# milos-agathon/vulkan-forge

Measured on AMD Instinct MI355X. Metric: Mpix/s terrain shade (grid=4096, 4096x4096), higher is better.
Workload: dtype f32

## Files before the change

include/vf_hip.h:

```cpp
#ifndef VF_HIP_H
#define VF_HIP_H

#include <stddef.h>
#include <stdint.h>

#ifdef __cplusplus
extern "C" {
#endif

#define VF_OK 0
#define VF_ERR_NO_DEVICE (-1)
#define VF_ERR_HIP (-2)
#define VF_ERR_INVALID (-3)
#define VF_ERR_NOMEM (-4)

typedef struct vf_ctx vf_ctx;
typedef struct vf_terrain vf_terrain;

typedef struct vf_device_info {
    char name[256];
    char arch[64];
    int32_t device_ordinal;
    int32_t compute_units;
    int32_t wavefront_size;
// ... 25 lines not shown
int vf_ctx_stream(const vf_ctx *ctx, void **stream);

int vf_terrain_create(vf_ctx *ctx, uint32_t width, uint32_t height, uint32_t grid,
                      const uint8_t lut_rgba8[1024], int lut_is_srgb, vf_terrain **out);
void vf_terrain_destroy(vf_terrain *t);

int vf_terrain_set_uniforms(vf_terrain *t, const float uniforms[44]);

int vf_terrain_set_height(vf_terrain *t, const float *host_height, uint32_t tw, uint32_t th);
int vf_terrain_set_height_device(vf_terrain *t, const float *dev_height, uint32_t tw, uint32_t th);

#define VF_SHADE_REFERENCE 0
#define VF_SHADE_SPEC_T32 1
int vf_terrain_set_shade_mode(vf_terrain *t, int mode);
#define VF_PRECISION_EXACT 0
#define VF_PRECISION_FAST 1
int vf_terrain_set_shade_precision(vf_terrain *t, int precision);
int vf_terrain_set_raster_groups(vf_terrain *t, int mode);
int vf_terrain_raster_groups(const vf_terrain *t, int *in_use, float ms[2]);

int vf_terrain_set_shard(vf_terrain *t, uint32_t rank, uint32_t nranks, uint32_t band_h);
int vf_terrain_local_rows(const vf_terrain *t, uint32_t *rows);

#define VF_TILE_LAYOUT(skew, stripe_log2) ((uint32_t)(skew) | ((uint32_t)(stripe_log2) << 16))
int vf_terrain_set_tile_shard(vf_terrain *t, uint32_t rank, uint32_t nranks, uint32_t layout);
int vf_terrain_tile_times(vf_terrain *t, float *ms, uint32_t capacity, uint32_t *count);
int vf_balance_stripes(const float *stripe_ms, uint32_t nstripes, uint32_t nranks, uint8_t *stripe_owner);
int vf_tile_layout_register_map(const uint8_t *stripe_owner, uint32_t nstripes, uint32_t stripe_log2, uint32_t nranks, uint32_t *layout);
int vf_terrain_local_tiles(const vf_terrain *t, uint32_t *tiles);
int vf_terrain_read_tiles(vf_terrain *t, uint8_t *dst, uint32_t first, uint32_t count);
int vf_tile_layout(uint32_t width, uint32_t height, uint32_t rank, uint32_t nranks, uint32_t layout, uint32_t *tiles,
                   uint32_t capacity, uint32_t *count);

int vf_terrain_set_output_device(vf_terrain *t, void *dev_rgba);
int vf_terrain_rgba_device(const vf_terrain *t, void **dev_rgba);

int vf_terrain_render(vf_terrain *t, void *stream);
int vf_terrain_render_batch(vf_terrain *t, const float *uniforms, uint32_t n, void *const *dev_rgba, void *stream);
int vf_terrain_render_batch_host(vf_terrain *t, const float *uniforms, uint32_t n, uint8_t *const *host_rgba);
int vf_terrain_sync(vf_terrain *t);

#define VF_SHAPE_CIRCLE 0
#define VF_SHAPE_SQUARE 1
#define VF_CAP_BUTT 0
#define VF_CAP_SQUARE 1
#define VF_CAP_ROUND 2
int vf_terrain_add_points(vf_terrain *t, const float *xyz, uint32_t n, const float *size_px, const uint8_t *rgba, float default_size,
                          const uint8_t default_rgba[4], int shape, int drape, uint32_t *layer_id);
int vf_terrain_add_lines(vf_terrain *t, const float *xyz, const uint32_t *path_offsets, uint32_t npaths, float width_px,
                         const uint8_t rgba[4], int cap, int drape, uint32_t *layer_id);
int vf_terrain_clear_overlays(vf_terrain *t);
int vf_terrain_add_polygons(vf_terrain *t, const float *xyz, const uint32_t *ring_offsets, uint32_t nrings, const uint32_t *feature_offsets,
                            uint32_t nfeatures, const uint8_t *fill_rgba, const uint8_t default_fill[4], const uint8_t line_rgba[4],
                            float line_width_px, int drape, uint32_t *layer_id);
#define VF_OCCLUSION_DEPTH_BIAS 1e-2f
int vf_terrain_set_layer_occlusion(vf_terrain *t, uint32_t layer_id, int occlude, float depth_bias);
#define VF_JOIN_ROUND 0
#define VF_JOIN_NONE 1
int vf_terrain_add_contours(vf_terrain *t, const float *levels, uint32_t nlevels, float width_px, const uint8_t rgba[4], float lift, int join,
                            int occlude, float depth_bias, uint32_t *layer_id, uint32_t *nsegments);
int vf_terrain_height_bounds(vf_terrain *t, float *lo, float *hi);
int vf_terrain_layer_primitive_count(vf_terrain *t, uint32_t layer_id, uint32_t *count);

int vf_terrain_read_rgba(vf_terrain *t, uint8_t *dst, uint32_t y0, uint32_t rows);
int vf_host_alloc(size_t bytes, void **host);
void vf_host_free(void *host);
int vf_terrain_read_png_scanlines(vf_terrain *t, const uint8_t **host_scanlines, size_t *nbytes);
int vf_terrain_read_visibility(vf_terrain *t, uint32_t *dst);

int vf_terrain_enable_timing(vf_terrain *t, int enable);
int vf_terrain_timings(vf_terrain *t, vf_timings *out);
int vf_terrain_frame_times(vf_terrain *t, float *tile_ms, float *period_ms, uint32_t max_frames, uint32_t *count);
int vf_terrain_debug_item_stats(vf_terrain *t, uint32_t *dst, uint32_t max_items, uint32_t *count);
#define VF_BAND_SLOTS 8u
int vf_terrain_debug_band_masks(vf_terrain *t, uint32_t *recs, uint64_t *masks, int32_t *xy, uint32_t max_blocks, uint32_t *count);
int vf_terrain_debug_set_plan_feedback(vf_terrain *t, const uint32_t *tile_ticks, const uint8_t *strips_log2, const uint32_t *piece_ticks,
                                       uint32_t ntiles);
#define VF_PLAN_FIRST        1u
#define VF_PLAN_FRESH        2u
#define VF_PLAN_MOTION_MAP   4u
#define VF_PLAN_DILATE       8u
#define VF_PLAN_QUEUED_AHEAD 16u
#define VF_PLAN_GEOMETRY_REUSED 32u
int vf_terrain_debug_plan_mode(const vf_terrain *t, uint32_t *mode);
int vf_terrain_debug_phase_cycles(vf_terrain *t, uint64_t *dst, uint32_t n);

int vf_grid_generate(vf_ctx *ctx, uint32_t nx, uint32_t nz, float dx, float dy,
                     float *xy, float *uv, uint32_t *idx);
int vf_grid_generate_device(vf_ctx *ctx, uint32_t nx, uint32_t nz, float dx, float dy,
                            float *dev_xy, float *dev_uv, uint32_t *dev_idx, void *stream);

int vf_triangle_render(vf_ctx *ctx, uint32_t width, uint32_t height, uint8_t *rgba_host);

typedef struct vf_dem vf_dem;
int vf_dem_create(vf_ctx *ctx, vf_dem **out);
void vf_dem_destroy(vf_dem *d);
int vf_dem_set_heights_f32(vf_dem *d, const float *host, uint32_t w, uint32_t h, float exaggeration);
int vf_dem_set_heights_f64(vf_dem *d, const double *host, uint32_t w, uint32_t h, float exaggeration);
int vf_dem_stats(vf_dem *d, float out[4]);
int vf_dem_percentile_range(vf_dem *d, float *p1, float *p99);
int vf_dem_normalize(vf_dem *d, int mode, float lo, float hi, float eps);
int vf_dem_upload_height(vf_dem *d);
int vf_dem_texture_size(const vf_dem *d, uint32_t *w, uint32_t *h);
int vf_dem_read_patch(vf_dem *d, uint32_t x, uint32_t y, uint32_t w, uint32_t h, float *dst);

int vf_stitch_bands_device(vf_ctx *ctx, const void *dev_gathered, void *dev_image, uint32_t width,
                           uint32_t height, uint32_t nranks, uint32_t band_h, void *stream);
int vf_stitch_tiles_device(vf_ctx *ctx, const void *dev_gathered, void *dev_image, uint32_t width, uint32_t height,
                           uint32_t nranks, uint32_t layout, uint32_t stride_tiles, void *stream);

#define VF_DIST_UNIQUE_ID_BYTES 128
int vf_dist_available(void);
int vf_dist_version(int *version);
int vf_dist_unique_id(uint8_t id[VF_DIST_UNIQUE_ID_BYTES]);
int vf_dist_comm_init(vf_ctx *ctx, const uint8_t id[VF_DIST_UNIQUE_ID_BYTES], int rank, int nranks, void **comm);
void vf_dist_comm_destroy(void *comm);
int vf_dist_gather_tiles(vf_terrain *t, void *rccl_comm, int root, void *dev_gathered, uint32_t stride_tiles, void *stream);
int vf_dist_gather_bands(vf_terrain *t, void *rccl_comm, int root, void *dev_image, void *stream);
int vf_dist_exchange_bands(vf_terrain *t, void *rccl_comm, int root, void *dev_image, void *stream);

typedef struct vf_fragment_timing {
    float resolve_ms;
    uint32_t covered_pixels;
    uint32_t repeats;
    uint32_t equal_to_frame;
} vf_fragment_timing;
int vf_terrain_debug_fragment_stage(vf_terrain *t, uint32_t repeats, vf_fragment_timing *out);

int vf_terrain_gbuffer_device(vf_terrain *t, float *dev_depth, float *dev_position, float *dev_normal, uint32_t *dev_primitive, void *stream);
int vf_terrain_read_gbuffer(vf_terrain *t, float *depth, float *position, float *normal, uint32_t *primitive);
int vf_terrain_pick(vf_terrain *t, const int32_t *pixels_xy, uint32_t n, float *out8);
#define VF_GBUFFER_DEPTH 1u
#define VF_GBUFFER_POSITION 2u
#define VF_GBUFFER_NORMAL 4u
#define VF_GBUFFER_PRIMITIVE 8u
int vf_terrain_debug_gbuffer_stage(vf_terrain *t, uint32_t planes, uint32_t repeats, float *ms);

#define VF_SHADOW_STRENGTH 0.7f
#define VF_SHADOW_SOFTNESS 0.02f
#define VF_SHADOW_BIAS 0.002f
int vf_terrain_set_shadows(vf_terrain *t, int enable, float strength, float softness, float bias);
int vf_terrain_read_shadow_field(vf_terrain *t, float *lit);
int vf_terrain_shadow_field_device(vf_terrain *t, float *dev_lit, void *stream);
int vf_terrain_debug_shadow_stage(vf_terrain *t, uint32_t repeats, float ms[2]);
int vf_terrain_debug_shadow_scans(vf_terrain *t, uint32_t *count);

#define VF_AMBIENT_STRENGTH 0.6f
#define VF_AMBIENT_REACH 64.0f
#define VF_AMBIENT_DIRECTIONS 16
#define VF_AMBIENT_REACH_MAX 1024
#define VF_AMBIENT_DIRECTIONS_MAX 64
int vf_terrain_set_ambient(vf_terrain *t, int enable, float strength, float reach, uint32_t ndirs, const float *dirs_xz);
int vf_terrain_read_sky_view_field(vf_terrain *t, float *sky);
int vf_terrain_sky_view_field_device(vf_terrain *t, float *dev_sky, void *stream);
int vf_terrain_debug_ambient_stage(vf_terrain *t, uint32_t repeats, float ms[2]);
int vf_terrain_debug_ambient_scans(vf_terrain *t, uint32_t *count);

#define VF_DRAPE_SIZE_MAX 16384
#define VF_DRAPE_NEAREST 0
#define VF_DRAPE_LINEAR 1
int vf_terrain_set_drape(vf_terrain *t, const uint8_t *rgba, uint32_t iw, uint32_t ih, uint32_t channels ,
                         const float extent[4], float opacity, int filter);
int vf_terrain_set_drape_device(vf_terrain *t, const void *dev_rgba , uint32_t iw, uint32_t ih,
                                const float extent[4], float opacity, int filter, void *stream);
int vf_terrain_clear_drape(vf_terrain *t);
int vf_terrain_drape_info(const vf_terrain *t, uint32_t *iw, uint32_t *ih, float extent[4], float *opacity, int *filter);
int vf_terrain_debug_drape_stage(vf_terrain *t, uint32_t repeats, float *ms);
// ... 56 lines not shown
```

vulkan_forge_amd/cabi.py:

```python
from __future__ import annotations

import ctypes as C
import os

import numpy as np

_HERE = os.path.dirname(os.path.abspath(__file__))
DEFAULT_LIB = os.environ.get("VF_HIP_LIB") or os.path.join(_HERE, "libvf_hip.so")

VF_OK, VF_ERR_NO_DEVICE, VF_ERR_HIP, VF_ERR_INVALID, VF_ERR_NOMEM = 0, -1, -2, -3, -4
VF_DRAPE_SIZE_MAX, VF_DRAPE_NEAREST, VF_DRAPE_LINEAR = 16384, 0, 1
VF_DRAPE_MIP_BIAS_MAX, VF_DRAPE_MIP_LEVELS_MAX = 16.0, 15
VF_PLAN_FIRST, VF_PLAN_FRESH, VF_PLAN_MOTION_MAP, VF_PLAN_DILATE, VF_PLAN_QUEUED_AHEAD = 1, 2, 4, 8, 16
VF_PLAN_GEOMETRY_REUSED = 32

SYMBOLS = [
    "vf_last_error", "vf_device_count", "vf_device_query", "vf_ctx_create", "vf_ctx_destroy", "vf_ctx_device_info", "vf_ctx_stream",
    "vf_terrain_create", "vf_terrain_destroy", "vf_terrain_set_uniforms", "vf_terrain_set_height",
    "vf_terrain_set_height_device", "vf_terrain_set_shade_mode", "vf_terrain_set_shade_precision", "vf_terrain_set_raster_groups", "vf_terrain_raster_groups", "vf_terrain_set_shard", "vf_terrain_local_rows", "vf_terrain_set_tile_shard",
    "vf_terrain_local_tiles", "vf_terrain_read_tiles", "vf_tile_layout", "vf_terrain_tile_times", "vf_balance_stripes", "vf_tile_layout_register_map", "vf_terrain_set_output_device",
    "vf_terrain_rgba_device", "vf_terrain_render", "vf_terrain_render_batch", "vf_terrain_render_batch_host", "vf_terrain_sync",
    "vf_terrain_add_points", "vf_terrain_add_lines", "vf_terrain_add_polygons", "vf_terrain_set_layer_occlusion", "vf_terrain_add_contours", "vf_terrain_height_bounds", "vf_terrain_layer_primitive_count", "vf_terrain_clear_overlays", "vf_terrain_read_rgba", "vf_terrain_read_png_scanlines", "vf_terrain_read_visibility",
    "vf_terrain_enable_timing", "vf_terrain_timings", "vf_terrain_frame_times", "vf_terrain_debug_item_stats", "vf_terrain_debug_band_masks", "vf_terrain_debug_set_plan_feedback", "vf_terrain_debug_plan_mode", "vf_terrain_debug_phase_cycles", "vf_grid_generate", "vf_grid_generate_device", "vf_triangle_render",
    "vf_stitch_bands_device", "vf_stitch_tiles_device",
    "vf_dist_available", "vf_dist_version", "vf_dist_unique_id", "vf_dist_comm_init", "vf_dist_comm_destroy", "vf_dist_gather_tiles", "vf_dist_gather_bands", "vf_dist_exchange_bands",
    "vf_terrain_debug_fragment_stage", "vf_host_alloc", "vf_host_free",
    "vf_terrain_gbuffer_device", "vf_terrain_read_gbuffer", "vf_terrain_pick", "vf_terrain_debug_gbuffer_stage",
    "vf_terrain_set_shadows", "vf_terrain_read_shadow_field", "vf_terrain_shadow_field_device", "vf_terrain_debug_shadow_stage",
    "vf_terrain_debug_shadow_scans",
    "vf_terrain_set_ambient", "vf_terrain_read_sky_view_field", "vf_terrain_sky_view_field_device", "vf_terrain_debug_ambient_stage",
    "vf_terrain_debug_ambient_scans",
    "vf_terrain_set_drape", "vf_terrain_set_drape_device", "vf_terrain_clear_drape", "vf_terrain_drape_info", "vf_terrain_debug_drape_stage",
    "vf_terrain_set_drape_mips", "vf_terrain_drape_mip_info", "vf_terrain_read_drape_level", "vf_terrain_debug_drape_mip_build",
    "vf_terrain_set_viewshed", "vf_terrain_read_viewshed_field", "vf_terrain_viewshed_field_device", "vf_terrain_viewshed_info",
    "vf_terrain_debug_viewshed_stage", "vf_terrain_debug_viewshed_scans",
    "vf_terrain_set_cumulative_viewshed", "vf_terrain_read_cumulative_viewshed_field", "vf_terrain_cumulative_viewshed_field_device",
    "vf_terrain_cumulative_viewshed_info", "vf_terrain_read_cumulative_viewshed_vertices", "vf_terrain_debug_cumulative_viewshed_batch",
    "vf_terrain_debug_cumulative_viewshed_scans", "vf_terrain_debug_cumulative_viewshed_stage",
    "vf_dem_create", "vf_dem_destroy", "vf_dem_set_heights_f32", "vf_dem_set_heights_f64", "vf_dem_stats",
    "vf_dem_percentile_range", "vf_dem_normalize", "vf_dem_upload_height", "vf_dem_texture_size", "vf_dem_read_patch",
]


class DeviceInfo(C.Structure):
    _fields_ = [("name", C.c_char * 256), ("arch", C.c_char * 64), ("device_ordinal", C.c_int32), ("compute_units", C.c_int32),
                ("wavefront_size", C.c_int32), ("clock_khz", C.c_int32), ("total_mem_bytes", C.c_uint64),
                ("lds_bytes_per_cu", C.c_uint64), ("pci_bus_id", C.c_int32), ("pci_device_id", C.c_int32)]


class Timings(C.Structure):
    _fields_ = [("ranges_ms", C.c_float), ("plan_ms", C.c_float), ("tile_ms", C.c_float), ("total_ms", C.c_float),
                ("blocks_rasterised", C.c_uint32), ("tiles", C.c_uint32), ("frames", C.c_uint32), ("blocks_distinct", C.c_uint32)]


class FragmentTiming(C.Structure):
    _fields_ = [("resolve_ms", C.c_float), ("covered_pixels", C.c_uint32), ("repeats", C.c_uint32), ("equal_to_frame", C.c_uint32)]


class ViewshedInfo(C.Structure):
    _fields_ = [("enabled", C.c_int32), ("has_observer", C.c_int32), ("vertex", C.c_uint32 * 2), ("observer_xyz", C.c_float * 3), ("eye_y", C.c_float),
                ("eye_height", C.c_float), ("target_height", C.c_float), ("radius", C.c_float), ("softness", C.c_float), ("bias", C.c_float),
                ("visible_rgba", C.c_uint8 * 4), ("hidden_rgba", C.c_uint8 * 4)]


class CumulativeViewshedInfo(C.Structure):
    _fields_ = [("enabled", C.c_int32), ("count", C.c_uint32), ("batch", C.c_uint32), ("eye_height", C.c_float), ("target_height", C.c_float),
                ("radius", C.c_float), ("softness", C.c_float), ("bias", C.c_float), ("high_rgba", C.c_uint8 * 4), ("low_rgba", C.c_uint8 * 4)]


DIST_UNIQUE_ID_BYTES = 128
_vp, _u32, _f, _i = C.c_void_p, C.c_uint32, C.c_float, C.c_int
_PROTOS = {
    "vf_last_error": (C.c_char_p, []),
    "vf_device_count": (_i, [C.POINTER(_i)]),
    "vf_device_query": (_i, [_i, C.POINTER(DeviceInfo)]),
    "vf_ctx_create": (_i, [_i, C.POINTER(_vp)]),
    "vf_ctx_destroy": (None, [_vp]),
    "vf_ctx_device_info": (_i, [_vp, C.POINTER(DeviceInfo)]),
    "vf_ctx_stream": (_i, [_vp, C.POINTER(_vp)]),
    "vf_terrain_create": (_i, [_vp, _u32, _u32, _u32, _vp, _i, C.POINTER(_vp)]),
    "vf_terrain_destroy": (None, [_vp]),
    "vf_terrain_set_uniforms": (_i, [_vp, _vp]),
    "vf_terrain_set_height": (_i, [_vp, _vp, _u32, _u32]),
    "vf_terrain_set_height_device": (_i, [_vp, _vp, _u32, _u32]),
    "vf_terrain_set_shade_mode": (_i, [_vp, _i]),
    "vf_terrain_set_shade_precision": (_i, [_vp, _i]),
    "vf_terrain_set_raster_groups": (_i, [_vp, _i]),
    "vf_terrain_raster_groups": (_i, [_vp, C.POINTER(_i), _vp]),
    "vf_terrain_set_shard": (_i, [_vp, _u32, _u32, _u32]),
    "vf_terrain_local_rows": (_i, [_vp, C.POINTER(_u32)]),
    "vf_terrain_set_tile_shard": (_i, [_vp, _u32, _u32, _u32]),
    "vf_terrain_add_points": (_i, [_vp, _vp, _u32, _vp, _vp, _f, _vp, _i, _i, C.POINTER(_u32)]),
    "vf_terrain_add_lines": (_i, [_vp, _vp, _vp, _u32, _f, _vp, _i, _i, C.POINTER(_u32)]),
    "vf_terrain_add_polygons": (_i, [_vp, _vp, _vp, _u32, _vp, _u32, _vp, _vp, _vp, _f, _i, C.POINTER(_u32)]),
    "vf_terrain_set_layer_occlusion": (_i, [_vp, _u32, _i, _f]),
    "vf_terrain_add_contours": (_i, [_vp, _vp, _u32, _f, _vp, _f, _i, _i, _f, C.POINTER(_u32), C.POINTER(_u32)]),
    "vf_terrain_height_bounds": (_i, [_vp, C.POINTER(_f), C.POINTER(_f)]),
    "vf_terrain_layer_primitive_count": (_i, [_vp, _u32, C.POINTER(_u32)]),
    "vf_terrain_clear_overlays": (_i, [_vp]),
    "vf_terrain_local_tiles": (_i, [_vp, C.POINTER(_u32)]),
    "vf_terrain_read_tiles": (_i, [_vp, _vp, _u32, _u32]),
    "vf_tile_layout": (_i, [_u32, _u32, _u32, _u32, _u32, _vp, _u32, C.POINTER(_u32)]),
    "vf_terrain_set_output_device": (_i, [_vp, _vp]),
    "vf_terrain_rgba_device": (_i, [_vp, C.POINTER(_vp)]),
    "vf_terrain_render": (_i, [_vp, _vp]),
    "vf_terrain_render_batch": (_i, [_vp, _vp, _u32, _vp, _vp]),
    "vf_terrain_render_batch_host": (_i, [_vp, _vp, _u32, _vp]),
    "vf_terrain_sync": (_i, [_vp]),
    "vf_terrain_read_rgba": (_i, [_vp, _vp, _u32, _u32]),
    "vf_terrain_read_png_scanlines": (_i, [_vp, C.POINTER(_vp), C.POINTER(C.c_size_t)]),
    "vf_terrain_read_visibility": (_i, [_vp, _vp]),
    "vf_terrain_enable_timing": (_i, [_vp, _i]),
    "vf_terrain_timings": (_i, [_vp, C.POINTER(Timings)]),
    "vf_terrain_frame_times": (_i, [_vp, _vp, _vp, _u32, C.POINTER(_u32)]),
    "vf_terrain_debug_item_stats": (_i, [_vp, _vp, _u32, C.POINTER(_u32)]),
    "vf_terrain_debug_band_masks": (_i, [_vp, _vp, _vp, _vp, _u32, C.POINTER(_u32)]),
    "vf_terrain_debug_set_plan_feedback": (_i, [_vp, _vp, _vp, _vp, _u32]),
    "vf_terrain_debug_plan_mode": (_i, [_vp, C.POINTER(_u32)]),
    "vf_terrain_debug_phase_cycles": (_i, [_vp, _vp, _u32]),
    "vf_terrain_tile_times": (_i, [_vp, _vp, _u32, C.POINTER(_u32)]),
    "vf_balance_stripes": (_i, [_vp, _u32, _u32, _vp]),
    "vf_tile_layout_register_map": (_i, [_vp, _u32, _u32, _u32, C.POINTER(_u32)]),
    "vf_host_alloc": (_i, [C.c_size_t, C.POINTER(_vp)]),
    "vf_host_free": (None, [_vp]),
    "vf_grid_generate": (_i, [_vp, _u32, _u32, _f, _f, _vp, _vp, _vp]),
    "vf_grid_generate_device": (_i, [_vp, _u32, _u32, _f, _f, _vp, _vp, _vp, _vp]),
    "vf_triangle_render": (_i, [_vp, _u32, _u32, _vp]),
    "vf_stitch_bands_device": (_i, [_vp, _vp, _vp, _u32, _u32, _u32, _u32, _vp]),
    "vf_stitch_tiles_device": (_i, [_vp, _vp, _vp, _u32, _u32, _u32, _u32, _u32, _vp]),
    "vf_dist_available": (_i, []),
    "vf_dist_version": (_i, [C.POINTER(_i)]),
    "vf_dist_unique_id": (_i, [_vp]),
    "vf_dist_comm_init": (_i, [_vp, _vp, _i, _i, C.POINTER(_vp)]),
    "vf_dist_comm_destroy": (None, [_vp]),
    "vf_dist_gather_tiles": (_i, [_vp, _vp, _i, _vp, _u32, _vp]),
    "vf_dist_gather_bands": (_i, [_vp, _vp, _i, _vp, _vp]),
    "vf_dist_exchange_bands": (_i, [_vp, _vp, _i, _vp, _vp]),
    "vf_terrain_debug_fragment_stage": (_i, [_vp, _u32, C.POINTER(FragmentTiming)]),
    "vf_terrain_gbuffer_device": (_i, [_vp, _vp, _vp, _vp, _vp, _vp]),
    "vf_terrain_read_gbuffer": (_i, [_vp, _vp, _vp, _vp, _vp]),
    "vf_terrain_pick": (_i, [_vp, _vp, _u32, _vp]),
    "vf_terrain_debug_gbuffer_stage": (_i, [_vp, _u32, _u32, C.POINTER(_f)]),
    "vf_terrain_set_shadows": (_i, [_vp, _i, _f, _f, _f]),
    "vf_terrain_read_shadow_field": (_i, [_vp, _vp]),
    "vf_terrain_shadow_field_device": (_i, [_vp, _vp, _vp]),
    "vf_terrain_debug_shadow_stage": (_i, [_vp, _u32, C.POINTER(_f)]),
    "vf_terrain_debug_shadow_scans": (_i, [_vp, C.POINTER(_u32)]),
    "vf_terrain_set_ambient": (_i, [_vp, _i, _f, _f, _u32, _vp]),
    "vf_terrain_read_sky_view_field": (_i, [_vp, _vp]),
    "vf_terrain_sky_view_field_device": (_i, [_vp, _vp, _vp]),
    "vf_terrain_debug_ambient_stage": (_i, [_vp, _u32, C.POINTER(_f)]),
    "vf_terrain_debug_ambient_scans": (_i, [_vp, C.POINTER(_u32)]),
    "vf_terrain_set_drape": (_i, [_vp, _vp, _u32, _u32, _u32, C.POINTER(_f), _f, _i]),
    "vf_terrain_set_drape_device": (_i, [_vp, _vp, _u32, _u32, C.POINTER(_f), _f, _i, _vp]),
    "vf_terrain_clear_drape": (_i, [_vp]),
    "vf_terrain_drape_info": (_i, [_vp, C.POINTER(_u32), C.POINTER(_u32), C.POINTER(_f), C.POINTER(_f), C.POINTER(_i)]),
    "vf_terrain_debug_drape_stage": (_i, [_vp, _u32, C.POINTER(_f)]),
    "vf_terrain_set_drape_mips": (_i, [_vp, _i, _f]),
    "vf_terrain_drape_mip_info": (_i, [_vp, C.POINTER(_i), C.POINTER(_u32), C.POINTER(_f), C.POINTER(C.c_uint64), C.POINTER(_u32)]),
    "vf_terrain_read_drape_level": (_i, [_vp, _u32, _vp, C.POINTER(_u32), C.POINTER(_u32)]),
    "vf_terrain_debug_drape_mip_build": (_i, [_vp, _u32, C.POINTER(_f)]),
    "vf_terrain_set_viewshed": (_i, [_vp, _i, C.POINTER(_f), _f, _f, _f, C.POINTER(C.c_uint8), C.POINTER(C.c_uint8), _f, _f]),
    "vf_terrain_read_viewshed_field": (_i, [_vp, _vp]),
    "vf_terrain_viewshed_field_device": (_i, [_vp, _vp, _vp]),
    "vf_terrain_viewshed_info": (_i, [_vp, C.POINTER(ViewshedInfo)]),
    "vf_terrain_debug_viewshed_stage": (_i, [_vp, _u32, C.POINTER(_f)]),
    "vf_terrain_debug_viewshed_scans": (_i, [_vp, C.POINTER(_u32)]),
    "vf_terrain_set_cumulative_viewshed": (_i, [_vp, _i, _vp, _u32, _f, _f, _f, C.POINTER(C.c_uint8), C.POINTER(C.c_uint8), _f, _f]),
    "vf_terrain_read_cumulative_viewshed_field": (_i, [_vp, _vp]),
    "vf_terrain_cumulative_viewshed_field_device": (_i, [_vp, _vp, _vp]),
    "vf_terrain_cumulative_viewshed_info": (_i, [_vp, C.POINTER(CumulativeViewshedInfo)]),
    "vf_terrain_read_cumulative_viewshed_vertices": (_i, [_vp, _vp]),
    "vf_terrain_debug_cumulative_viewshed_batch": (_i, [_vp, _u32]),
    "vf_terrain_debug_cumulative_viewshed_scans": (_i, [_vp, C.POINTER(_u32)]),
    "vf_terrain_debug_cumulative_viewshed_stage": (_i, [_vp, _u32, C.POINTER(_f)]),
    "vf_dem_create": (_i, [_vp, C.POINTER(_vp)]),
    "vf_dem_destroy": (None, [_vp]),
    "vf_dem_set_heights_f32": (_i, [_vp, _vp, _u32, _u32, _f]),
    "vf_dem_set_heights_f64": (_i, [_vp, _vp, _u32, _u32, _f]),
    "vf_dem_stats": (_i, [_vp, _vp]),
    "vf_dem_percentile_range": (_i, [_vp, C.POINTER(_f), C.POINTER(_f)]),
    "vf_dem_normalize": (_i, [_vp, _i, _f, _f, _f]),
    "vf_dem_upload_height": (_i, [_vp]),
    "vf_dem_texture_size": (_i, [_vp, C.POINTER(_u32), C.POINTER(_u32)]),
    "vf_dem_read_patch": (_i, [_vp, _u32, _u32, _u32, _u32, _vp]),
}


def load(path: str = DEFAULT_LIB) -> C.CDLL:
    lib = C.CDLL(path)
    for name, (res, args) in _PROTOS.items():
        fn = getattr(lib, name)
        fn.restype, fn.argtypes = res, args
    return lib


class VfError(RuntimeError):
    pass


def tile_layout(width, height, rank, nranks, skew=3, lib=None):
# ... 422 lines not shown
        from ._drape import drape_args
        img, iw, ih, ch, ext, opacity, code = drape_args(image, extent, opacity, filter)
        self._check(self.lib.vf_terrain_set_drape(self.t, img.ctypes.data, iw, ih, ch, ext.ctypes.data_as(C.POINTER(_f)), opacity, code))

    def set_drape_device(self, dev_rgba, width, height, *, extent=None, opacity=1.0, filter="linear", stream=None):
        from ._drape import drape_params, drape_size
        iw, ih = drape_size(width, height)
        ext, opacity, code = drape_params(extent, opacity, filter)
        self._check(self.lib.vf_terrain_set_drape_device(self.t, dev_rgba, iw, ih, ext.ctypes.data_as(C.POINTER(_f)), opacity, code, stream))

    def clear_drape(self):
        self._check(self.lib.vf_terrain_clear_drape(self.t))

    def drape_info(self):
        from ._drape import drape_info
        iw, ih, op, code, ext = _u32(), _u32(), _f(), _i(), (_f * 4)()
        self._check(self.lib.vf_terrain_drape_info(self.t, C.byref(iw), C.byref(ih), ext, C.byref(op), C.byref(code)))
        return drape_info(iw.value, ih.value, tuple(ext), op.value, code.value)

    def drape_stage(self, repeats=20):
        ms = _f()
        self._check(self.lib.vf_terrain_debug_drape_stage(self.t, int(repeats), C.byref(ms)))
        return ms.value

    def set_drape_mipmaps(self, enabled=True, *, bias=0.0):
        from ._drape import mip_params
        on, bias = mip_params(enabled, bias)
        self._check(self.lib.vf_terrain_set_drape_mips(self.t, on, bias))

    def drape_mip_info(self):
        from ._drape import mip_info
        on, levels, bias, nbytes, builds, iw, ih = _i(), _u32(), _f(), C.c_uint64(), _u32(), _u32(), _u32()
        self._check(self.lib.vf_terrain_drape_mip_info(self.t, C.byref(on), C.byref(levels), C.byref(bias), C.byref(nbytes), C.byref(builds)))
        self._check(self.lib.vf_terrain_drape_info(self.t, C.byref(iw), C.byref(ih), None, None, None))
        return mip_info(on.value != 0, levels.value, bias.value, nbytes.value, builds.value, iw.value, ih.value)

    def read_drape_level(self, level):
        from ._drape import mip_level
        levels, w, h = _u32(), _u32(), _u32()
        self._check(self.lib.vf_terrain_drape_mip_info(self.t, None, C.byref(levels), None, None, None))
        k = mip_level(level, levels.value)
        self._check(self.lib.vf_terrain_read_drape_level(self.t, k, None, C.byref(w), C.byref(h)))
        out = np.empty((h.value, w.value, 4), np.float16)
        self._check(self.lib.vf_terrain_read_drape_level(self.t, k, out.ctypes.data, None, None))
        return out

    def drape_mip_build_stage(self, repeats=20):
        ms = _f()
        self._check(self.lib.vf_terrain_debug_drape_mip_build(self.t, int(repeats), C.byref(ms)))
        return ms.value

    def enable_timing(self, on=True, stats=True, sampled=False):
        self._check(self.lib.vf_terrain_enable_timing(self.t, (1 if stats else (3 if sampled else 2)) if on else 0))

    def item_stats(self):
        cap = self.timings()["tiles"] + 2048
        out = np.zeros((cap, 4), np.uint32)
        n = _u32()
        self._check(self.lib.vf_terrain_debug_item_stats(self.t, out.ctypes.data, cap, C.byref(n)))
        return out[:n.value]

    def band_masks(self):
        nb = (self.grid - 1 + 7) // 8
        n = nb * nb
        recs, masks, xy = np.zeros((n, 8), np.uint32), np.zeros((n, 8, 2), np.uint64), np.zeros((n, 81, 2), np.int32)
        got = _u32()
        self._check(self.lib.vf_terrain_debug_band_masks(self.t, recs.ctypes.data, masks.ctypes.data, xy.ctypes.data, n, C.byref(got)))
        assert got.value == n
        wide = recs[:, 4:8].copy().view(np.uint64)
        return dict(box=recs[:, 0:2].copy().view(np.int16), flags=recs[:, 2].copy(), count=recs[:, 3].copy(),
                    alive_even=wide[:, 0].copy(), alive_odd=wide[:, 1].copy(), masks=masks, xy=xy)

    def set_plan_feedback(self, tile_ticks, strips_log2=None, piece_ticks=None):
        ticks = np.ascontiguousarray(tile_ticks, dtype=np.uint32).reshape(-1)
        n = len(ticks)
        lg = np.zeros(n, np.uint8) if strips_log2 is None else np.ascontiguousarray(strips_log2, dtype=np.uint8).reshape(n)
        pieces = None if piece_ticks is None else np.ascontiguousarray(piece_ticks, dtype=np.uint32).reshape(n, 64)
        self._check(self.lib.vf_terrain_debug_set_plan_feedback(self.t, ticks.ctypes.data, lg.ctypes.data,
                                                                None if pieces is None else pieces.ctypes.data, n))

    def plan_mode(self, geometry=False):
        m = _u32()
        self._check(self.lib.vf_terrain_debug_plan_mode(self.t, C.byref(m)))
        return m.value if geometry else m.value & ~VF_PLAN_GEOMETRY_REUSED

    def geometry_reused(self):
        return bool(self.plan_mode(geometry=True) & VF_PLAN_GEOMETRY_REUSED)

    def tile_stats(self):
        it = self.item_stats()
        out = np.zeros((self.timings()["tiles"], 3), np.uint32)
        tile = it[:, 0] & 0xFFFFF
        np.add.at(out[:, 0], tile, it[:, 1])
        np.maximum.at(out[:, 1], tile, it[:, 2])
        np.maximum.at(out[:, 2], tile, it[:, 3])
        return out

    def phase_cycles(self):
        out = np.zeros(40, np.uint64)
        self._check(self.lib.vf_terrain_debug_phase_cycles(self.t, out.ctypes.data, 40))
        return out

    def frame_times(self):
        tile, period, n = np.zeros(64, np.float32), np.zeros(64, np.float32), _u32(0)
        self._check(self.lib.vf_terrain_frame_times(self.t, tile.ctypes.data, period.ctypes.data, 64, C.byref(n)))
        return tile[:n.value].copy(), period[:n.value].copy()

    def timings(self):
        tm = Timings()
        self._check(self.lib.vf_terrain_timings(self.t, C.byref(tm)))
        return {k: getattr(tm, k) for k, _ in Timings._fields_}


class Dem:

    def __init__(self, device=0, lib=None):
        self.lib = lib or load()
        self.ctx, self.d = _vp(), _vp()
        self._check(self.lib.vf_ctx_create(int(device), C.byref(self.ctx)))
        self._check(self.lib.vf_dem_create(self.ctx, C.byref(self.d)))

    def _check(self, rc):
        if rc != VF_OK:
            msg = self.lib.vf_last_error().decode()
            raise VfError("No suitable GPU adapter" if rc == VF_ERR_NO_DEVICE else msg)

    def close(self):
        if self.d:
            self.lib.vf_dem_destroy(self.d)
            self.d = _vp()
        if self.ctx:
            self.lib.vf_ctx_destroy(self.ctx)
            self.ctx = _vp()

    def __del__(self):
        try:
            self.close()
        except Exception:
            pass

    def set_heights(self, heights, exaggeration=1.0):
        a = np.asarray(heights)
        if a.ndim != 2 or a.dtype not in (np.float32, np.float64) or not a.flags.c_contiguous:
            raise TypeError("heights must be a C-contiguous 2-D array of float32 or float64")
        fn = self.lib.vf_dem_set_heights_f32 if a.dtype == np.float32 else self.lib.vf_dem_set_heights_f64
        self._check(fn(self.d, a.ctypes.data, a.shape[1], a.shape[0], float(exaggeration)))

    def stats(self):
        out = np.zeros(4, np.float32)
        self._check(self.lib.vf_dem_stats(self.d, out.ctypes.data))
        return tuple(out)

    def percentile_range(self):
        p1, p99 = _f(), _f()
        self._check(self.lib.vf_dem_percentile_range(self.d, C.byref(p1), C.byref(p99)))
        return np.float32(p1.value), np.float32(p99.value)

    def normalize(self, mode, lo=0.0, hi=1.0, eps=1e-8):
        self._check(self.lib.vf_dem_normalize(self.d, {"minmax": 0, "zscore": 1}[mode], float(lo), float(hi), float(eps)))

    def upload(self):
        self._check(self.lib.vf_dem_upload_height(self.d))

    def texture_size(self):
        w, h = _u32(), _u32()
        self._check(self.lib.vf_dem_texture_size(self.d, C.byref(w), C.byref(h)))
        return w.value, h.value
# ... 11 lines not shown
```

vulkan_forge_amd/csrc/vf_hip.hip:

```cpp
#include "../../include/vf_hip.h"
#include "vf_kernels.h"
#include "vf_overlay.h"
#include "vf_gbuffer.h"
#include "vf_shadow.h"
#include "vf_ambient.h"
#include "vf_drape.h"
#include "vf_relight.h"
#include "vf_viewshed.h"
#include "vf_cumulative_viewshed.h"
#include "vf_line_loop.h"

#include <algorithm>
#include <cmath>
#include <vector>
#include <cstddef>
#include <cstdio>
#include <cstring>
#include <cstdlib>
#include <functional>
#include <new>
#include <string>
#include <atomic>
#include <memory>
#include <mutex>
// ... 79 lines not shown
    while ((1u << s) < v) ++s;
    return s;
}

}

struct PinnedRegistry {
    std::mutex mu;
    std::vector<void *> registered;
    static PinnedRegistry &get() { static PinnedRegistry *r = new PinnedRegistry; return *r; }
};
static hipError_t pinned_alloc(void **out, size_t n)
{
    constexpr size_t kHuge = (size_t)2 << 20;
    *out = nullptr;
    if (n >= 2 * kHuge) {
        void *p = nullptr;
        const size_t r = (n + kHuge - 1) & ~(kHuge - 1);
        if (posix_memalign(&p, kHuge, r) == 0) {
            (void)madvise(p, r, MADV_HUGEPAGE);
            if (hipHostRegister(p, r, hipHostRegisterDefault) == hipSuccess) {
                std::lock_guard<std::mutex> lk(PinnedRegistry::get().mu);
                PinnedRegistry::get().registered.push_back(p);
                *out = p;
                return hipSuccess;
            }
            (void)hipGetLastError();
            std::free(p);
        }
    }
    return hipHostMalloc(out, n, hipHostMallocDefault);
}
static void pinned_free(void *p)
{
    if (!p) return;
    bool ours = false;
    {
        PinnedRegistry &R = PinnedRegistry::get();
        std::lock_guard<std::mutex> lk(R.mu);
        auto it = std::find(R.registered.begin(), R.registered.end(), p);
        if (it != R.registered.end()) { R.registered.erase(it); ours = true; }
    }
    if (ours) { (void)hipHostUnregister(p); std::free(p); }
    else (void)hipHostFree(p);
}

struct vf_ctx {
    int device = 0;
    hipStream_t stream = nullptr;
    hipDeviceProp_t prop;
    float *d_decode = nullptr;
    float *d_thresh = nullptr;
    hipStream_t side = nullptr, side2 = nullptr, copy = nullptr;
    uint8_t *d_maps = nullptr;
    uint64_t maps_uploaded = 0;
    std::mutex lazy_mu;
};

static hipError_t ctx_side_streams(vf_ctx *c, hipStream_t *side, hipStream_t *side2)
{
    std::lock_guard<std::mutex> lk(c->lazy_mu);
    hipError_t e = hipSuccess;
    if (!c->side) e = hipStreamCreateWithFlags(&c->side, hipStreamNonBlocking);
    if (e == hipSuccess && !c->side2) e = hipStreamCreateWithFlags(&c->side2, hipStreamNonBlocking);
    *side = c->side; *side2 = c->side2;
    return e;
}
static hipError_t ctx_copy_stream(vf_ctx *c, hipStream_t *copy)
{
    std::lock_guard<std::mutex> lk(c->lazy_mu);
    hipError_t e = hipSuccess;
    if (!c->copy) e = hipStreamCreateWithFlags(&c->copy, hipStreamNonBlocking);
    *copy = c->copy;
    return e;
}

struct FramePlan {
    FrameParams P;
    uint32_t set = 0, ntiles = 0;
    uint32_t mode = 0;
    bool motion_starts = false;
    bool sampled = true;
    uint32_t *rc_lo = nullptr, *rc_hi = nullptr, *seg_count = nullptr;
};

template <typename T> struct DevBuf {
    T *p = nullptr;
    size_t cap = 0;
    hipError_t reserve(size_t need, size_t new_cap, size_t keep = 0, bool zero = false)
    {
        if (need <= cap) return hipSuccess;
        T *q = nullptr;
        hipError_t e = hipMalloc(&q, new_cap * sizeof(T));
        if (e == hipSuccess && zero) e = hipMemset(q, 0, new_cap * sizeof(T));
        if (e == hipSuccess && keep) e = hipMemcpy(q, p, keep * sizeof(T), hipMemcpyDeviceToDevice);
        if (e != hipSuccess) {
            if (q) (void)hipFree(q);
            return e;
        }
        release();
        p = q; cap = new_cap;
        return hipSuccess;
    }
    void release()
    {
        if (p) (void)hipFree(p);
        p = nullptr; cap = 0;
    }
};

struct VertexField {
    DevBuf<float> d;
    bool valid = false;
    uint64_t height_gen = 0;
    std::vector<uint32_t> key;
    uint32_t scans = 0;
    int prepare(const vf_terrain *t, const std::vector<uint32_t> &k, bool force, const char *nomem, bool *current);
    void computed(const vf_terrain *t, std::vector<uint32_t> &k);
    void release() { d.release(); valid = false; }
};
static uint32_t key_bits(float f) { uint32_t w; std::memcpy(&w, &f, sizeof w); return w; }
static std::vector<uint32_t> key_of(std::initializer_list<float> fs)
{
    std::vector<uint32_t> k;
    for (float f : fs) k.push_back(key_bits(f));
    return k;
}

template <typename F> static hipError_t time_launches(hipStream_t s, uint32_t repeats, float &ms, F &&launch)
{
    hipEvent_t e0 = nullptr, e1 = nullptr;
    hipError_t err = hipEventCreate(&e0);
    if (err == hipSuccess) err = hipEventCreate(&e1);
    if (err == hipSuccess) err = launch(true);
    if (err == hipSuccess) err = hipEventRecord(e0, s);
    for (uint32_t k = 0; k < repeats && err == hipSuccess; ++k) err = launch(false);
    if (err == hipSuccess) err = hipEventRecord(e1, s);
    if (err == hipSuccess) err = hipEventSynchronize(e1);
    float total = 0.0f;
    if (err == hipSuccess) err = hipEventElapsedTime(&total, e0, e1);
    if (e0) (void)hipEventDestroy(e0);
    if (e1) (void)hipEventDestroy(e1);
    ms = total / (float)repeats;
    return err;
}

struct PlanCursor {
    uint32_t cur_set = 0;
    uint32_t frame_no = 0;
    uint32_t frames_since_reset = 0;
    bool have_drawn = false, camera_moving = false, was_moving = false;
    float u_drawn[32] = {};
};

struct FrameInputs {
    float u[44] = {};
    uint32_t shade_mode = 0;
    uint32_t precision = VF_PRECISION_FAST;
};

struct LineLoop {
    int mode = -1;
    struct Probe { hipEvent_t a = nullptr, b = nullptr; int variant = 0; uint32_t epoch = 0; bool pending = false; } probes[16];
    uint32_t head = 0, epoch_id = 0;
    float ms[2] = { 0.0f, 0.0f };
    uint32_t n[2] = { 0u, 0u };
// ... 86 lines not shown
        DevBuf<float> d_cmax;
    } sh;
    struct Ambient {
        bool enabled = false;
        float strength = VF_AMBIENT_STRENGTH, reach = VF_AMBIENT_REACH;
        uint32_t ndirs = VF_AMBIENT_DIRECTIONS;
        bool default_dirs = true;
        std::vector<float> dirs;
        VertexField sky;
    } am;
    struct Drape {
        uint32_t iw = 0, ih = 0;
        float extent[4] = { -1.5f, -1.5f, 1.5f, 1.5f }, opacity = 1.0f;
        int filter = VF_DRAPE_LINEAR;
        DevBuf<uint32_t> d_img;
        hipEvent_t copied = nullptr;
    } dr;
    struct DrapeMipState {
        bool enabled = false;
        float bias = 0.0f;
        DevBuf<uint2> d_pyr;
        bool stale = true;
        uint32_t builds = 0;
    } dm;
    struct Viewshed {
        bool enabled = false, have_observer = false;
        float ox = 0.0f, oz = 0.0f;
        float eye_height = VF_VIEWSHED_EYE_HEIGHT, target_height = VF_VIEWSHED_TARGET_HEIGHT, radius = 0.0f;
        float softness = VF_VIEWSHED_SOFTNESS, bias = VF_VIEWSHED_BIAS;
        uint32_t visible_rgba = VF_VIEWSHED_VISIBLE_RGBA, hidden_rgba = VF_VIEWSHED_HIDDEN_RGBA;
        bool tinted = false;
        VertexField seen;
        DevBuf<float> d_cmax;
    } vs;
    struct CumulativeViewshed {
        bool enabled = false;
        std::vector<float> xz;
        float eye_height = VF_VIEWSHED_EYE_HEIGHT, target_height = VF_VIEWSHED_TARGET_HEIGHT, radius = 0.0f;
        float softness = VF_VIEWSHED_SOFTNESS, bias = VF_VIEWSHED_BIAS;
        uint32_t high_rgba = VF_CUMULATIVE_VIEWSHED_HIGH_RGBA, low_rgba = VF_CUMULATIVE_VIEWSHED_LOW_RGBA;
        uint32_t forced_batch = 0;
        DevBuf<uint32_t> d_sum;
        VertexField count;
        DevBuf<float> d_frac;
        DevBuf<float> d_cmax;
        DevBuf<ViewshedPlan> d_plans;
        std::vector<ViewshedPlan> plans;
        uint32_t batch = 0;
    } cv;
    uint64_t height_gen = 1;
    static constexpr uint32_t kBatchRing = 3;
    uint32_t *d_batch[kBatchRing] = { nullptr, nullptr, nullptr };
    hipEvent_t batch_drawn[kBatchRing] = { nullptr, nullptr, nullptr }, batch_copied[kBatchRing] = { nullptr, nullptr, nullptr };
    hipStream_t copy_stream = nullptr;
    uint8_t *d_png = nullptr, *h_png = nullptr;
    uint8_t *h_stage = nullptr;
    hipEvent_t stage_ev[4] = { nullptr, nullptr, nullptr, nullptr };
    static constexpr uint32_t kPlanStates = 2;
    struct PlanState {
        PixelBox *ranges = nullptr;
        VertexRec *vtx = nullptr;
        BlockRec *recs = nullptr;
        ulonglong2 *gen = nullptr;
        ulonglong2 *band = nullptr;
        uint32_t *seg_list = nullptr;
        PixelBox *row_ranges = nullptr;
        float4 *cap_seg = nullptr;
        float *cap_rad = nullptr;
        uint32_t *rc = nullptr;
        uint2 *work = nullptr;
        uint2 *work_sorted = nullptr;
        uint32_t *work_count = nullptr;
        uint32_t *redo = nullptr;
        uint32_t *background = nullptr;
        uint32_t *flags_new = nullptr;
        uint32_t *feedback = nullptr;
        hipEvent_t planned = nullptr, drawn = nullptr, boxed = nullptr, set_up = nullptr;
        hipEvent_t pev[3] = { nullptr, nullptr, nullptr };
        bool pev_valid = false;
        uint8_t *slab = nullptr;
        float u_used[32] = {};
        bool have_u_used = false;
        uint64_t geom_stamp = 0, height_stamp = 0;
    } ps[kPlanStates];
    PlanCursor cursor;
    uint32_t last_set = 0;
    uint32_t last_plan_mode = 0;
    hipStream_t side = nullptr;
    hipStream_t side2 = nullptr;
    hipEvent_t entry = nullptr;
    hipEvent_t cached = nullptr;
    hipStream_t cached_on = nullptr;
    hipStream_t last_stream = nullptr;
    bool rendered = false;
    uint64_t inputs_gen = 1;
    uint64_t geom_gen = 1;
    struct PrePlan {
        bool valid = false;
        FramePlan K;
        uint64_t gen = 0, geom = 0;
        PlanCursor before;
    } pre;
    uint64_t last_drawn_geom = 0;
    bool replan_fresh = false;
    bool preplan_pending = false;
    uint32_t tight_calls = 0;
    bool want_plan_streams = false;
    hipEvent_t copied = nullptr;
    static constexpr int kTimingRing = 64;
    bool timing = false;
    bool stats_on = false;
    uint32_t timing_every = 1;
    struct FrameEvents { hipEvent_t begin = nullptr, end = nullptr; } ev[kTimingRing];
    uint32_t timed_frames = 0;
    LineLoop loop;
    uint8_t *d_xrecv = nullptr, *d_xband = nullptr;
    size_t xrecv_bytes = 0, xband_bytes = 0;
    struct Overlays {
        uint32_t nprims = 0, features = 0;
        DevBuf<OvIn> in;
        DevBuf<OvPrim> prim;
        DevBuf<uint2> box;
        uint32_t *d_cnt = nullptr;
        uint32_t *d_start = nullptr;
        DevBuf<uint32_t> list;
        uint32_t *h_total = nullptr;
        hipEvent_t counted = nullptr;
        uint32_t nfill = 0;
        uint32_t pg_lo = 0, pg_hi = 0;
        DevBuf<uint32_t> pg_hdr;
        DevBuf<uint4> pg_fbox;
        DevBuf<uint4> pg_fbin;
        DevBuf<unsigned long long> pg_total;
        DevBuf<uint32_t> mask;
        struct Layer { uint32_t lo, hi; bool polygon, occlude; };
        std::vector<Layer> layer;
        uint32_t occluding = 0;
        DevBuf<float4> dep;
    } ov;
    struct Contours {
        DevBuf<float> levels;
        DevBuf<uint32_t> count;
        DevBuf<unsigned long long> total;
        DevBuf<float2> bounds;
    } ct;
};

struct StatsLayout { size_t phases, block_bits, words; };
static StatsLayout stats_layout(const vf_terrain *t)
{
    const size_t phases = 4 + 4 * ((size_t)t->ntx * t->nty + kSplitBudget), block_bits = phases + 2 * kPhaseSlots;
    return { phases, block_bits, block_bits + (t->nblocks + 31) / 32 };
}
static size_t feedback_words(const vf_terrain *t) { return (size_t)t->ntx * t->nty * 65 + 1; }
static uint32_t grid_segments(const vf_terrain *t) { return t->nb * ((t->nb + kSegBlocks - 1) / kSegBlocks); }
static float grid_step(const vf_terrain *t) { return (2.0f * 1.5f) / ((float)t->n - 1.0f); }
static float spacing_of(const float *u) { return std::fmax(u[36], 1e-8f); }

int VertexField::prepare(const vf_terrain *t, const std::vector<uint32_t> &k, bool force, const char *nomem, bool *current)
{
    if (!d.p) {
        const size_t nv = (size_t)t->n * t->n;
        if (d.reserve(nv, nv) != hipSuccess) { (void)hipGetLastError(); return fail(VF_ERR_NOMEM, nomem); }
        valid = false;
    }
    *current = !force && valid && height_gen == t->height_gen && key == k;
    if (!*current) valid = false;
// ... 112 lines not shown
}

static AxisTables axis(const vf_terrain *t)
{
    AxisTables A;
    A.xs = t->d_xs; A.sinx = t->d_sinx; A.cosz = t->d_cosz; A.txi = t->d_txi; A.tyj = t->d_tyj;
    return A;
}

namespace {
struct Carver {
    struct Item { void **p; size_t bytes; };
    std::vector<Item> zeroed, plain;
    void add(void **p, size_t bytes, bool zero = false) { (zero ? zeroed : plain).push_back({ p, (bytes + 255u) & ~(size_t)255u }); }
    hipError_t commit(uint8_t **base, hipStream_t s)
    {
        size_t zero_bytes = 0, total = 0;
        for (const Item &i : zeroed) zero_bytes += i.bytes;
        total = zero_bytes;
        for (const Item &i : plain) total += i.bytes;
        hipError_t e = hipMalloc((void **)base, total);
        if (e != hipSuccess) return e;
        size_t off = 0;
        for (const Item &i : zeroed) { *i.p = *base + off; off += i.bytes; }
        for (const Item &i : plain) { *i.p = *base + off; off += i.bytes; }
        return zero_bytes ? hipMemsetAsync(*base, 0, zero_bytes, s) : hipSuccess;
    }
};
}

static hipError_t sync_sides(const vf_terrain *t)
{
    hipError_t e = t->side ? hipStreamSynchronize(t->side) : hipSuccess;
    if (e == hipSuccess && t->side2) e = hipStreamSynchronize(t->side2);
    return e;
}

static hipError_t wait_frame(const vf_terrain *t)
{
    const hipError_t e = hipSetDevice(t->ctx->device);
    return e != hipSuccess ? e : hipStreamSynchronize(t->last_stream ? t->last_stream : t->ctx->stream);
}

static hipError_t drop_preplan(vf_terrain *t, hipStream_t next_plan_on = nullptr)
{
    t->preplan_pending = false;
    if (!t->pre.valid) return hipSuccess;
    const vf_terrain::PrePlan &R = t->pre;
    t->pre.valid = false;
    t->cursor = R.before;
    t->replan_fresh = true;
    hipStream_t on = t->side ? t->side : (next_plan_on ? next_plan_on : (t->last_stream ? t->last_stream : t->ctx->stream));
    hipError_t e = hipStreamWaitEvent(on, t->ps[R.K.set].set_up, 0);
    if (e == hipSuccess) e = hipStreamWaitEvent(on, t->ps[R.K.set].planned, 0);
    if (e == hipSuccess) e = hipMemsetAsync(R.K.seg_count, 0, sizeof(uint32_t), on);
    return e;
}

static hipError_t ensure_plan_state(vf_terrain *t, uint32_t k, hipStream_t zero_on)
{
    vf_terrain::PlanState &S = t->ps[k];
    if (S.slab) return hipSuccess;
    const size_t all_tiles = (size_t)t->ntx * t->nty;
    Carver C;
    C.add((void **)&S.seg_list, ((size_t)grid_segments(t) + 1) * sizeof(uint32_t), true);
    C.add((void **)&S.feedback, feedback_words(t) * sizeof(uint32_t), true);
    C.add((void **)&S.background, all_tiles * sizeof(uint32_t), true);
    C.add((void **)&S.ranges, t->nblocks * sizeof(PixelBox));
    C.add((void **)&S.vtx, (size_t)t->nblocks * kBlockStride * sizeof(VertexRec));
    C.add((void **)&S.recs, (size_t)t->nblocks * sizeof(BlockRec));
    C.add((void **)&S.band, (size_t)t->nblocks * kBandSlots * sizeof(ulonglong2));
    C.add((void **)&S.gen, (size_t)t->nblocks * sizeof(ulonglong2));
    C.add((void **)&S.row_ranges, t->nb * sizeof(PixelBox));
    C.add((void **)&S.cap_seg, t->nblocks * sizeof(float4));
    C.add((void **)&S.cap_rad, t->nblocks * sizeof(float));
    C.add((void **)&S.rc, 2 * (size_t)t->nb * t->ntx * sizeof(uint32_t));
    C.add((void **)&S.work, 2 * (all_tiles + kSplitBudget + 16) * sizeof(uint2));
    C.add((void **)&S.work_count, 4 * sizeof(uint32_t));
    C.add((void **)&S.redo, (all_tiles + kSplitBudget) * sizeof(uint32_t));
    C.add((void **)&S.flags_new, all_tiles * sizeof(uint32_t));
    hipError_t err = C.commit(&S.slab, zero_on);
    if (err != hipSuccess) { S.slab = nullptr; return err; }
    S.geom_stamp = S.height_stamp = 0;
    S.work_sorted = S.work + (all_tiles + kSplitBudget + 16);
    if (err == hipSuccess) err = hipEventCreateWithFlags(&S.planned, hipEventDisableTiming);
    if (err == hipSuccess) err = hipEventCreateWithFlags(&S.drawn, hipEventDisableTiming);
    if (err == hipSuccess) err = hipEventCreateWithFlags(&S.boxed, hipEventDisableTiming);
    if (err == hipSuccess) err = hipEventCreateWithFlags(&S.set_up, hipEventDisableTiming);
    return err;
}

static int refresh_tables(vf_terrain *t, hipStream_t s)
{
    hipLaunchKernelGGL(k_axis_tables, dim3((t->n + 255) / 256), dim3(256), 0, s, t->n, t->tw, t->th, t->d_xs, t->d_sinx,
                       t->d_cosz, t->d_txi, t->d_tyj);
    VF_HIP_TRY(hipGetLastError());
    t->bounds_dirty = true;
    return VF_OK;
}

static void ov_release(vf_terrain *t)
{
    vf_terrain::Overlays &O = t->ov;
    void *ptrs[] = { O.d_cnt, O.d_start };
    for (void *p : ptrs) if (p) (void)hipFree(p);
    O.in.release(); O.prim.release(); O.box.release(); O.list.release(); O.dep.release();
    O.pg_hdr.release(); O.pg_fbox.release(); O.pg_fbin.release(); O.pg_total.release(); O.mask.release();
    if (O.h_total) (void)hipHostFree(O.h_total);
    if (O.counted) (void)hipEventDestroy(O.counted);
    O = vf_terrain::Overlays();
    t->ct.levels.release(); t->ct.count.release(); t->ct.total.release(); t->ct.bounds.release();
}

static void drape_release(vf_terrain *t)
{
    vf_terrain::Drape &D = t->dr;
    D.d_img.release();
    if (D.copied) (void)hipEventDestroy(D.copied);
    D = vf_terrain::Drape();
    t->dm.d_pyr.release(); t->dm.stale = true;
}

static void shadow_release(vf_terrain *t) { t->sh.lit.release(); t->sh.d_cmax.release(); }
static void ambient_release(vf_terrain *t) { t->am.sky.release(); }

static void viewshed_release(vf_terrain *t)
{
    vf_terrain::Viewshed &H = t->vs;
    H.seen.release(); H.d_cmax.release();
    const uint32_t scans = H.seen.scans;
    H = vf_terrain::Viewshed();
    H.seen.scans = scans;
}

static void cumulative_release(vf_terrain *t)
{
    vf_terrain::CumulativeViewshed &H = t->cv;
    H.d_sum.release(); H.count.release(); H.d_frac.release(); H.d_cmax.release(); H.d_plans.release();
    const uint32_t scans = H.count.scans, forced = H.forced_batch;
    H = vf_terrain::CumulativeViewshed();
    H.count.scans = scans; H.forced_batch = forced;
}

int vf_terrain_create(vf_ctx *ctx, uint32_t width, uint32_t height, uint32_t grid, const uint8_t lut_rgba8[1024],
                      int lut_is_srgb, vf_terrain **out)
{
    if (!ctx || !out || !lut_rgba8) return fail(VF_ERR_INVALID, "NULL argument");
    *out = nullptr;
    if (width == 0 || height == 0 || width > 16384 || height > 16384) return fail(VF_ERR_INVALID, "width/height must be in 1..16384");
    uint32_t n = grid < 2 ? 2 : grid;
    if (n > 8192) return fail(VF_ERR_INVALID, "grid must be <= 8192");
    VF_HIP_TRY(hipSetDevice(ctx->device));
    vf_terrain *t = new (std::nothrow) vf_terrain;
    if (!t) return fail(VF_ERR_NOMEM, "out of host memory");
    t->ctx = ctx; t->W = width; t->H = height; t->n = n;
    t->nb = (n - 1 + kBlockCells - 1) / kBlockCells;
    t->nblocks = t->nb * t->nb;
    t->ntx = (width + kTileW - 1) / kTileW;
    t->nty = (height + kTileH - 1) / kTileH;
    t->local_rows = height;
    t->local_tiles = t->ntx * t->nty;

    float lut[kLutFloats];
    for (int i = 0; i <= 256; ++i) {
        const int k = i < 256 ? i : 255;
        for (int ch = 0; ch < 3; ++ch)
            lut[kLutStride * i + ch] = lut_is_srgb ? tables().decode[lut_rgba8[4 * k + ch]] : (float)lut_rgba8[4 * k + ch] / 255.0f;
        lut[kLutStride * i + 3] = 0.0f;
    }
    hipError_t err = hipSuccess;
    const size_t all_tiles = (size_t)t->ntx * t->nty;
    Carver C;
    C.add((void **)&t->d_height_dummy, sizeof(float), true);
    C.add((void **)&t->d_stats, stats_layout(t).words * sizeof(uint32_t), true);
    C.add((void **)&t->d_xs, n * sizeof(float));
    C.add((void **)&t->d_sinx, n * sizeof(float));
    C.add((void **)&t->d_cosz, n * sizeof(float));
    C.add((void **)&t->d_txi, n * sizeof(int32_t));
    C.add((void **)&t->d_tyj, n * sizeof(int32_t));
    C.add((void **)&t->d_bounds, t->nblocks * sizeof(float2));
    C.add((void **)&t->d_hblk, (size_t)t->nblocks * kBlockStride * sizeof(float));
    C.add((void **)&t->d_lut, sizeof lut);
    C.add((void **)&t->d_rgba_own, all_tiles * kTileW * kTileH * sizeof(uint32_t));
    C.add((void **)&t->d_tile_map, all_tiles * sizeof(uint32_t));
    C.add((void **)&t->d_stripe_owner, kMaxStripes);
    err = C.commit(&t->slab, ctx->stream);
    if (err == hipSuccess) err = hipMemcpyAsync(t->d_lut, lut, sizeof lut, hipMemcpyHostToDevice, ctx->stream);
    if (err == hipSuccess) err = hipEventCreateWithFlags(&t->entry, hipEventDisableTiming);
    if (err == hipSuccess) err = hipEventCreateWithFlags(&t->cached, hipEventDisableTiming);
    for (uint32_t k = 0; k < vf_terrain::kPlanStates && err == hipSuccess; ++k) err = ensure_plan_state(t, k, ctx->stream);
    if (err != hipSuccess) {
        std::string m = std::string("terrain allocation failed: ") + hipGetErrorString(err);
        vf_terrain_destroy(t);
        return fail(err == hipErrorOutOfMemory ? VF_ERR_NOMEM : VF_ERR_HIP, m);
    }
    t->d_rgba = t->d_rgba_own;
    t->d_height = t->d_height_dummy; t->tw = 1; t->th = 1;
    int rc = refresh_tables(t, ctx->stream);
    if (rc == VF_OK && hipStreamSynchronize(ctx->stream) != hipSuccess) rc = fail(VF_ERR_HIP, "table setup failed");
    if (rc != VF_OK) { std::string keep = g_err; vf_terrain_destroy(t); g_err = keep; return rc; }
    *out = t;
    return VF_OK;
}

void vf_terrain_destroy(vf_terrain *t)
{
    if (!t) return;
    (void)hipSetDevice(t->ctx->device);
    (void)hipDeviceSynchronize();
    void *ptrs[] = { t->slab, t->d_height_own, t->d_vis, t->d_rgba_scratch, t->d_diag, t->d_xrecv, t->d_xband, t->d_batch[0], t->d_batch[1], t->d_batch[2] };
    for (void *p : ptrs) if (p) (void)hipFree(p);
    t->d_gb.release(); t->d_pick.release();
    shadow_release(t); ambient_release(t); viewshed_release(t); cumulative_release(t);
    drape_release(t);
    for (auto &e : t->batch_drawn) if (e) (void)hipEventDestroy(e);
    for (auto &e : t->batch_copied) if (e) (void)hipEventDestroy(e);

    for (auto &S : t->ps) {
        if (S.slab) (void)hipFree(S.slab);
        if (S.planned) (void)hipEventDestroy(S.planned);
        if (S.drawn) (void)hipEventDestroy(S.drawn);
        if (S.boxed) (void)hipEventDestroy(S.boxed);
        if (S.set_up) (void)hipEventDestroy(S.set_up);
        for (auto &e : S.pev) if (e) (void)hipEventDestroy(e);
    }
    pinned_free(t->h_stage);
    for (auto &e : t->stage_ev) if (e) (void)hipEventDestroy(e);
    if (t->d_png) (void)hipFree(t->d_png);
    pinned_free(t->h_png);
    for (auto &f : t->ev) { if (f.begin) (void)hipEventDestroy(f.begin); if (f.end) (void)hipEventDestroy(f.end); }
    if (t->entry) (void)hipEventDestroy(t->entry);
    if (t->cached) (void)hipEventDestroy(t->cached);
    if (t->copied) (void)hipEventDestroy(t->copied);
    for (auto &g : t->loop.probes) { if (g.a) (void)hipEventDestroy(g.a); if (g.b) (void)hipEventDestroy(g.b); }
    ov_release(t);
    delete t;
}

static bool same_geometry(const float *a, const float *b)
{
    return std::memcmp(a, b, 32 * sizeof(float)) == 0 && std::memcmp(a + 36, b + 36, sizeof(float)) == 0 && std::memcmp(a + 38, b + 38, sizeof(float)) == 0;
}

static void take_uniforms(vf_terrain *t, const float *uniforms)
{
    if (!t->have_uniforms || std::memcmp(t->inputs.u, uniforms, sizeof t->inputs.u) != 0) t->inputs_gen++;
    if (!t->have_uniforms || !same_geometry(t->inputs.u, uniforms)) t->geom_gen++;
    std::memcpy(t->inputs.u, uniforms, sizeof t->inputs.u);
    t->have_uniforms = true;
}

int vf_terrain_set_uniforms(vf_terrain *t, const float uniforms[44])
{
    if (!t || !uniforms) return fail(VF_ERR_INVALID, "NULL argument");
    take_uniforms(t, uniforms);
    return VF_OK;
}

static int set_height_common(vf_terrain *t, uint32_t tw, uint32_t th)
{
    t->inputs_gen++;
    t->geom_gen++;
    t->height_gen++;
    VF_HIP_TRY(drop_preplan(t));
    t->loop.reset();
    bool resized = tw != t->tw || th != t->th;
    t->tw = tw; t->th = th;
    if (resized) return refresh_tables(t, t->ctx->stream);
    t->bounds_dirty = true;
    return VF_OK;
}

int vf_terrain_set_height(vf_terrain *t, const float *host_height, uint32_t tw, uint32_t th)
{
    if (!t || !host_height) return fail(VF_ERR_INVALID, "NULL argument");
    if (tw == 0 || th == 0 || tw > 32768 || th > 32768) return fail(VF_ERR_INVALID, "height texture size must be in 1..32768");
    VF_HIP_TRY(wait_frame(t));
    VF_HIP_TRY(sync_sides(t));
    size_t bytes = (size_t)tw * th * sizeof(float);
    if ((size_t)t->tw * t->th != (size_t)tw * th || t->d_height != t->d_height_own) {
        float *fresh = nullptr;
        hipError_t e = hipMalloc(&fresh, bytes);
        if (e != hipSuccess) return fail(e == hipErrorOutOfMemory ? VF_ERR_NOMEM : VF_ERR_HIP, std::string("height texture allocation failed: ") + hipGetErrorString(e));
        if (t->d_height_own) (void)hipFree(t->d_height_own);
        t->d_height_own = fresh;
    }
    t->d_height = t->d_height_own;
    VF_HIP_TRY(hipMemcpyAsync(t->d_height_own, host_height, bytes, hipMemcpyHostToDevice, t->ctx->stream));
    int rc = set_height_common(t, tw, th);
    if (rc == VF_OK) {
        hipLaunchKernelGGL(k_height_blocks, dim3(t->nblocks), dim3(64), 0, t->ctx->stream, t->n, t->nb, t->tw, axis(t), t->d_height, t->d_hblk, t->d_bounds);
        const hipError_t le = hipGetLastError();
        if (le != hipSuccess) rc = fail(VF_ERR_HIP, std::string("k_height_blocks: ") + hipGetErrorString(le));
        else t->bounds_dirty = false;
    }
    VF_HIP_TRY(hipStreamSynchronize(t->ctx->stream));
    return rc;
}

int vf_terrain_set_height_device(vf_terrain *t, const float *dev_height, uint32_t tw, uint32_t th)
{
    if (!t || !dev_height) return fail(VF_ERR_INVALID, "NULL argument");
    if (tw == 0 || th == 0 || tw > 32768 || th > 32768) return fail(VF_ERR_INVALID, "height texture size must be in 1..32768");
    VF_HIP_TRY(wait_frame(t));
    VF_HIP_TRY(sync_sides(t));
    t->d_height = dev_height;
    int rc = set_height_common(t, tw, th);
    if (rc != VF_OK) return rc;
    VF_HIP_TRY(hipStreamSynchronize(t->ctx->stream));
    return VF_OK;
}

int vf_terrain_set_shade_mode(vf_terrain *t, int mode)
{
    if (!t) return fail(VF_ERR_INVALID, "NULL argument");
    if (mode != VF_SHADE_REFERENCE && mode != VF_SHADE_SPEC_T32) return fail(VF_ERR_INVALID, "unknown shade mode");
    if (t->inputs.shade_mode != (uint32_t)mode) t->inputs_gen++;
    t->inputs.shade_mode = (uint32_t)mode;
    return VF_OK;
}

int vf_terrain_set_shade_precision(vf_terrain *t, int precision)
{
    if (!t) return fail(VF_ERR_INVALID, "NULL argument");
    if (precision != VF_PRECISION_EXACT && precision != VF_PRECISION_FAST) return fail(VF_ERR_INVALID, "unknown shade precision");
    if (t->inputs.precision != (uint32_t)precision) t->inputs_gen++;
    t->inputs.precision = (uint32_t)precision;
    return VF_OK;
}

int vf_terrain_set_raster_groups(vf_terrain *t, int mode)
{
    if (!t) return fail(VF_ERR_INVALID, "NULL argument");
    if (mode < -1 || mode > 1) return fail(VF_ERR_INVALID, "mode must be -1 (measure and choose), 0 or 1");
    t->loop.mode = mode;
    t->loop.reset();
    return VF_OK;
}

int vf_terrain_raster_groups(const vf_terrain *t, int *in_use, float ms[2])
{
    if (!t || !in_use) return fail(VF_ERR_INVALID, "NULL argument");
    *in_use = t->loop.now;
    if (ms) { ms[0] = t->loop.n[0] ? t->loop.ms[0] : 0.0f; ms[1] = t->loop.n[1] ? t->loop.ms[1] : 0.0f; }
    return VF_OK;
}

static int reset_layout_feedback(vf_terrain *t)
{
    t->rendered = false; t->have_frame = false;
    t->cursor.frames_since_reset = 0;
    VF_HIP_TRY(sync_sides(t));
    for (auto &S : t->ps) {
        if (!S.slab) continue;
        VF_HIP_TRY(hipMemset(S.feedback, 0, feedback_words(t) * sizeof(uint32_t)));
        VF_HIP_TRY(hipMemset(S.background, 0, (size_t)t->ntx * t->nty * sizeof(uint32_t)));
        S.have_u_used = false;
    }
    for (auto &S : t->ps) S.geom_stamp = S.height_stamp = 0;
    return VF_OK;
}

int vf_terrain_set_shard(vf_terrain *t, uint32_t rank, uint32_t nranks, uint32_t band_h)
{
    if (!t) return fail(VF_ERR_INVALID, "NULL argument");
    if (nranks == 0 || rank >= nranks) return fail(VF_ERR_INVALID, "rank must be < nranks");
    if (!is_pow2(band_h) || band_h < (uint32_t)kTileH) return fail(VF_ERR_INVALID, "band_h must be a power of two >= 64 (the tile height)");
    if (!t->ov.layer.empty()) return fail(VF_ERR_INVALID, "the handle has overlays: sharded compositing is not supported (vf_terrain_clear_overlays first)");
    if (t->sh.enabled && nranks != 1) return fail(VF_ERR_INVALID, "the handle has shadows enabled: shadows need a whole-frame handle");
    if (t->am.enabled && nranks != 1) return fail(VF_ERR_INVALID, "the handle has ambient occlusion enabled: it needs a whole-frame handle");
    if (t->dr.iw && nranks != 1) return fail(VF_ERR_INVALID, "the handle holds a draped image: it needs a whole-frame handle");
    if (t->vs.enabled && nranks != 1) return fail(VF_ERR_INVALID, "the handle has a viewshed enabled: it needs a whole-frame handle");
    if (t->cv.enabled && nranks != 1) return fail(VF_ERR_INVALID, "the handle has a cumulative viewshed enabled: it needs a whole-frame handle");
    VF_HIP_TRY(wait_frame(t));
    t->inputs_gen++;
    t->geom_gen++;
    VF_HIP_TRY(drop_preplan(t));
    t->rank = rank; t->nranks = nranks; t->band_h = band_h;
    t->shard_tiles = false; t->use_map = false;
    t->local_rows = compute_local_rows(t->H, rank, nranks, band_h);
    t->local_tiles = t->ntx * ((t->local_rows + kTileH - 1) / kTileH);
    return reset_layout_feedback(t);
}

int vf_tile_layout(uint32_t width, uint32_t height, uint32_t rank, uint32_t nranks, uint32_t skew, uint32_t *tiles, uint32_t capacity,
                   uint32_t *count)
{
    if (!count) return fail(VF_ERR_INVALID, "NULL argument");
    if (width == 0 || height == 0 || nranks == 0 || rank >= nranks) return fail(VF_ERR_INVALID, "empty frame or rank >= nranks");
    if (!layout_valid(skew)) return fail(VF_ERR_INVALID, "layout word is neither VF_TILE_LAYOUT(skew < 65536, stripe_log2 <= 15) nor a registered stripe map");
    const uint32_t ntx = (width + kTileW - 1) / kTileW, nty = (height + kTileH - 1) / kTileH;
    if (ntx > 0xFFFFu || nty > 0xFFFFu) return fail(VF_ERR_INVALID, "frame too large");
    const StripeMap *m = layout_map(skew);
    if (m && (m->nranks != nranks || ((ntx - 1u) >> m->shift) >= m->owner.size()))
        return fail(VF_ERR_INVALID, "the registered stripe map was made for another number of ranks or a narrower frame");
    uint32_t n = 0;
    for (uint32_t ty = 0; ty < nty; ++ty)
        for (uint32_t tx = 0; tx < ntx; ++tx)
            if (layout_owner(skew, m, tx, ty, nranks) == rank) {
                if (tiles && n < capacity) tiles[n] = tx | (ty << 16);
                ++n;
            }
    *count = n;
    return VF_OK;
}

int vf_tile_layout_register_map(const uint8_t *stripe_owner, uint32_t nstripes, uint32_t stripe_log2, uint32_t nranks, uint32_t *layout)
{
    if (!stripe_owner || !layout) return fail(VF_ERR_INVALID, "NULL argument");
    if (nstripes == 0 || nstripes > kMaxStripes || stripe_log2 > 15u || nranks == 0 || nranks > 255u) return fail(VF_ERR_INVALID, "1..256 stripes, stripe_log2 <= 15, 1..255 ranks");
    for (uint32_t k = 0; k < nstripes; ++k) if (stripe_owner[k] >= nranks) return fail(VF_ERR_INVALID, "a stripe's owner is not a rank");
    std::lock_guard<std::mutex> lk(g_maps_mu);
    g_maps.reserve(kMaxStripeMaps);
    for (uint32_t id = 0; id < g_maps.size(); ++id)
        if (g_maps[id].shift == stripe_log2 && g_maps[id].nranks == nranks && g_maps[id].owner.size() == nstripes &&
            std::memcmp(g_maps[id].owner.data(), stripe_owner, nstripes) == 0) { *layout = kLayoutMapBit | (id << 21) | (stripe_log2 << 16); return VF_OK; }
    if (g_maps.size() >= kMaxStripeMaps) return fail(VF_ERR_INVALID, "too many registered stripe maps (64 per process)");
    StripeMap m;
    m.owner.assign(stripe_owner, stripe_owner + nstripes); m.shift = stripe_log2; m.nranks = nranks;
    g_maps.push_back(std::move(m));
    *layout = kLayoutMapBit | ((uint32_t)(g_maps.size() - 1u) << 21) | (stripe_log2 << 16);
    return VF_OK;
}

int vf_balance_stripes(const float *stripe_ms, uint32_t nstripes, uint32_t nranks, uint8_t *stripe_owner)
{
    if (!stripe_ms || !stripe_owner) return fail(VF_ERR_INVALID, "NULL argument");
    if (nranks == 0 || nranks > 255u || nstripes == 0 || nstripes > kMaxStripes || nstripes % nranks) return fail(VF_ERR_INVALID, "the stripes must divide evenly among 1..255 ranks");
    std::vector<uint32_t> order(nstripes);
    for (uint32_t k = 0; k < nstripes; ++k) order[k] = k;
    auto cost = [&](uint32_t k) { const float v = stripe_ms[k]; return std::isfinite(v) && v > 0.0f ? (double)v : 0.0; };
    std::stable_sort(order.begin(), order.end(), [&](uint32_t a, uint32_t b) { return cost(a) > cost(b); });
    std::vector<double> load(nranks, 0.0);
    std::vector<uint32_t> have(nranks, 0u);
    std::vector<uint8_t> own(nstripes, 0);
    const uint32_t room = nstripes / nranks;
    for (uint32_t k : order) {
        uint32_t best = nranks;
        for (uint32_t r = 0; r < nranks; ++r)
            if (have[r] < room && (best == nranks || load[r] < load[best])) best = r;
        own[k] = (uint8_t)best; load[best] += cost(k); have[best]++;
    }
// ... 128 lines not shown
    P.hw = 0.5f * (float)t->W; P.hh = 0.5f * (float)t->H;
    P.step = grid_step(t);
    P.n = t->n; P.nm1 = t->n - 1; P.nb = t->nb;
    P.W = t->W; P.H = t->H; P.ntx = t->ntx; P.nty = t->nty; P.tw = t->tw; P.th = t->th;
    P.rank = t->rank; P.nranks = t->nranks; P.band_h = t->band_h; P.band_shift = ilog2(t->band_h);
    P.local_rows = t->local_rows;
    P.shard_tiles = t->shard_tiles ? 1u : 0u; P.tile_map = t->d_tile_map; P.skew = layout_skew(t->skew); P.stripe_shift = layout_shift(t->skew);
    P.stripe_owner = t->shard_tiles && t->use_map ? t->d_stripe_owner : nullptr;
    P.shade_mode = in.shade_mode; P.tex = t->d_height;
    P.inv2hr = 1.0f / (2.0f * P.h_range);
    {
        const uint32_t d = P.nm1;
        if (d <= 1u) { P.div_m = 0u; P.div_s = 0u; }
        else {
            const uint32_t L = ilog2(d);
            P.div_s = L - 1u;
            P.div_m = (uint32_t)((((uint64_t)1 << (31u + L)) + d - 1u) / d);
        }
    }
    const SrgbTables &T = tables();
    P.clear_rgba = T.encode(0.02f) | (T.encode(0.02f) << 8) | (T.encode(0.03f) << 16) | 0xFF000000u;
}

static float camera_shift_px(const vf_terrain *t, const float *a, const float *b)
{
    const float ext = 1.5f * spacing_of(t->inputs.u);
    float worst = 0.0f;
    for (int c = 0; c < 4; ++c) {
        const float p[4] = { (c & 1) ? ext : -ext, 0.0f, (c & 2) ? ext : -ext, 1.0f };
        float xy[2][2];
        for (int k = 0; k < 2; ++k) {
            const float *u = k ? b : a;
            float v[4], q[4];
            for (int r = 0; r < 4; ++r) v[r] = u[r] * p[0] + u[4 + r] * p[1] + u[8 + r] * p[2] + u[12 + r] * p[3];
            for (int r = 0; r < 4; ++r) q[r] = u[16 + r] * v[0] + u[20 + r] * v[1] + u[24 + r] * v[2] + u[28 + r] * v[3];
            if (!(q[3] > 1e-6f)) return 1e9f;
            xy[k][0] = q[0] / q[3] * 0.5f * (float)t->W; xy[k][1] = q[1] / q[3] * 0.5f * (float)t->H;
        }
        worst = std::fmax(worst, std::fmax(std::fabs(xy[0][0] - xy[1][0]), std::fabs(xy[0][1] - xy[1][1])));
    }
    return worst;
}
static bool motion_map(const vf_terrain *t, const float *then, const float *now, MotionMap &M)
{
    const double hw = 0.5 * t->W, hh = 0.5 * t->H;
    auto plane = [&](const float *u, double g[9]) {
        double vp[16];
        for (int c = 0; c < 4; ++c)
            for (int r = 0; r < 4; ++r) {
                double a = 0.0;
                for (int k = 0; k < 4; ++k) a += (double)u[16 + 4 * k + r] * (double)u[4 * c + k];
                vp[4 * c + r] = a;
            }
        const int cols[3] = { 0, 2, 3 };
        for (int j = 0; j < 3; ++j) {
            const double cx = vp[4 * cols[j] + 0], cy = vp[4 * cols[j] + 1], cw = vp[4 * cols[j] + 3];
            g[0 + j] = hw * cx + hw * cw; g[3 + j] = -hh * cy + hh * cw; g[6 + j] = cw;
        }
    };
    double a[9], b[9];
    plane(then, a); plane(now, b);
    const double det = b[0] * (b[4] * b[8] - b[5] * b[7]) - b[1] * (b[3] * b[8] - b[5] * b[6]) + b[2] * (b[3] * b[7] - b[4] * b[6]);
    double scale = 0.0;
    for (double v : b) scale = std::fmax(scale, std::fabs(v));
    if (!(std::fabs(det) > 1e-12 * scale * scale * scale)) return false;
    const double inv[9] = { (b[4] * b[8] - b[5] * b[7]) / det, (b[2] * b[7] - b[1] * b[8]) / det, (b[1] * b[5] - b[2] * b[4]) / det,
                            (b[5] * b[6] - b[3] * b[8]) / det, (b[0] * b[8] - b[2] * b[6]) / det, (b[2] * b[3] - b[0] * b[5]) / det,
                            (b[3] * b[7] - b[4] * b[6]) / det, (b[1] * b[6] - b[0] * b[7]) / det, (b[0] * b[4] - b[1] * b[3]) / det };
    double m[9], big = 0.0;
    for (int r = 0; r < 3; ++r)
        for (int c = 0; c < 3; ++c) { m[3 * r + c] = a[3 * r] * inv[c] + a[3 * r + 1] * inv[3 + c] + a[3 * r + 2] * inv[6 + c]; big = std::fmax(big, std::fabs(m[3 * r + c])); }
    if (!(big > 0.0) || !std::isfinite(big)) return false;
    for (int k = 0; k < 9; ++k) M.m[k] = (float)(m[k] / big);
    M.on = 1u;
    return true;
}
constexpr float kFreshFeedbackPx = 24.0f;

#ifndef VF_GROUPS_MAX_RANKS
#define VF_GROUPS_MAX_RANKS 8
#endif
static bool fast_shading(const FrameInputs &in) { return in.precision == VF_PRECISION_FAST && in.shade_mode == VF_SHADE_REFERENCE; }

static int plan_frame(vf_terrain *t, hipStream_t s, FramePlan &K, bool streaming = false)
{
    FrameParams &P = K.P;
    PlanCursor &C = t->cursor;
    const float *u = t->inputs.u;
    build_params(t, t->inputs, P);
    AxisTables A = axis(t);
    const uint32_t ntiles = t->local_tiles;
    const uint32_t set = C.cur_set;
    C.cur_set = (set + 1u) % vf_terrain::kPlanStates;
    C.frame_no++;
    if (!t->side && C.frame_no > 1u) {
        bool have = false;
        { std::lock_guard<std::mutex> lk(t->ctx->lazy_mu); have = t->ctx->side && t->ctx->side2; }
        if (have || streaming || t->want_plan_streams) VF_HIP_TRY(ctx_side_streams(t->ctx, &t->side, &t->side2));
    }
    const bool solo = !t->side;
    VF_HIP_TRY(ensure_plan_state(t, set, solo ? s : t->side));
    vf_terrain::PlanState &S = t->ps[set], &O = t->ps[t->last_set];
    float shift = 0.0f;
    if (C.have_drawn) {
        shift = camera_shift_px(t, C.u_drawn, u);
        if (shift > kFreshFeedbackPx) C.camera_moving = true;
        else if (shift < 0.5f * kFreshFeedbackPx) C.camera_moving = false;
    }
    const bool young = C.frames_since_reset >= 1 && C.frames_since_reset < vf_terrain::kPlanStates;
    MotionMap M;
    std::memset(&M, 0, sizeof M);
    if ((C.camera_moving || C.was_moving) && !young && C.frames_since_reset >= vf_terrain::kPlanStates && S.have_u_used && t->nranks == 1u && !t->shard_tiles &&
        camera_shift_px(t, S.u_used, u) < 0.4f * (float)std::max(t->W, t->H))
        (void)motion_map(t, S.u_used, u, M);
    const bool after_drop = t->replan_fresh && C.frames_since_reset >= vf_terrain::kPlanStates;
    t->replan_fresh = false;
    if (after_drop) M.on = 0u;
    const bool fresh = young || after_drop || ((C.camera_moving || C.was_moving) && !M.on);
    const bool first = C.frames_since_reset == 0;
    C.frames_since_reset++;
    const bool motion_starts = C.camera_moving && !C.was_moving;
    C.was_moving = C.camera_moving;
    const bool dilate = fresh || shift > 0.5f * kFreshFeedbackPx;
    std::memcpy(C.u_drawn, u, sizeof C.u_drawn);
    C.have_drawn = true;
    hipStream_t side = solo ? s : t->side, side2 = solo ? s : t->side2;
    K.sampled = t->timing_every <= 1u || C.frame_no % t->timing_every == 0u;
    const bool timed = t->timing && t->timing_every <= 1u && S.pev[0] != nullptr;
    hipEvent_t *ev = S.pev;
    S.pev_valid = timed;
    VF_HIP_TRY(hipStreamWaitEvent(side, S.drawn, 0));
    if (t->bounds_dirty) {
        VF_HIP_TRY(hipEventRecord(t->entry, s));
        VF_HIP_TRY(hipStreamWaitEvent(side, t->entry, 0));
        hipLaunchKernelGGL(k_height_blocks, dim3(t->nblocks), dim3(64), 0, side, t->n, t->nb, t->tw, A, t->d_height, t->d_hblk, t->d_bounds);
        VF_HIP_TRY(hipGetLastError());
        VF_HIP_TRY(hipEventRecord(t->cached, side));
        t->cached_on = side;
        t->bounds_dirty = false;
        for (auto &X : t->ps) X.geom_stamp = X.height_stamp = 0;
    }
    if (t->cached_on && t->cached_on != side) {
        VF_HIP_TRY(hipStreamWaitEvent(side, t->cached, 0));
        t->cached_on = side;
    }
    const bool reuse = S.geom_stamp != 0 && S.geom_stamp == t->geom_gen && S.height_stamp == t->height_gen;
    if (timed) VF_HIP_TRY(hipEventRecord(ev[0], side));
    const size_t rc_n = (size_t)t->nb * t->ntx;
    uint32_t *rc_lo = S.rc, *rc_hi = S.rc + rc_n;
    uint32_t *quantum = S.feedback + (size_t)t->ntx * t->nty;
    const uint32_t nsegs_all = grid_segments(t);
    uint32_t *seg_count = S.seg_list + nsegs_all;
    const uint32_t *const quantum_from = fresh || first ? (const uint32_t *)nullptr : S.feedback;
    if (reuse) {
        hipLaunchKernelGGL(k_plan_begin, dim3(1), dim3(512), 0, side, quantum_from, t->ntx * t->nty, quantum, S.work_count);
    } else {
        S.geom_stamp = S.height_stamp = 0;
        hipLaunchKernelGGL(k_block_boxes, dim3(t->nb + 1), dim3(t->nb > 256 ? 512 : 256), 0, side, P, t->d_bounds, S.ranges, S.row_ranges, S.cap_seg, S.cap_rad, rc_lo, rc_hi,
                           quantum_from, t->ntx * t->nty, quantum, S.work_count, S.recs, S.seg_list, seg_count);
        VF_HIP_TRY(hipEventRecord(S.boxed, side));
        VF_HIP_TRY(hipStreamWaitEvent(side2, S.boxed, 0));
        hipLaunchKernelGGL(k_block_setup, dim3(nsegs_all), dim3(kSetupThreads), 0, side2,
                           P, t->d_hblk, S.ranges, S.vtx, S.recs, S.gen, S.seg_list, seg_count, S.band);
        VF_HIP_TRY(hipEventRecord(S.set_up, side2));
        VF_HIP_TRY(hipGetLastError());
        S.geom_stamp = t->geom_gen; S.height_stamp = t->height_gen;
    }
    if (timed) VF_HIP_TRY(hipEventRecord(ev[1], side));
    if (ntiles) {
        if (fresh) {
            VF_HIP_TRY(hipStreamWaitEvent(side, O.drawn, 0));
            hipLaunchKernelGGL(k_quantum, dim3(1), dim3(512), 0, side, O.feedback, t->ntx * t->nty, quantum);
        } else if (first) {
            VF_HIP_TRY(hipStreamWaitEvent(side, S.set_up, 0));
            hipLaunchKernelGGL(k_plan_estimate, dim3(ntiles), dim3(256), 0, side, P, S.row_ranges, S.recs, S.cap_seg, S.cap_rad, rc_lo, rc_hi, S.feedback);
            hipLaunchKernelGGL(k_quantum, dim3(1), dim3(512), 0, side, S.feedback, t->ntx * t->nty, quantum);
        }
        const vf_terrain::PlanState &F = fresh ? O : S;
        hipLaunchKernelGGL(k_plan, dim3(ntiles), dim3(256), 0, side, P, S.row_ranges, S.flags_new, S.work, S.work_count,
                           F.feedback, quantum, S.work_count + 1, rc_lo, rc_hi, dilate ? 1u : 0u, F.background, M);
        hipLaunchKernelGGL(k_plan_sort, dim3(1), dim3(256), 0, side, S.work, S.work_sorted, S.work_count, S.feedback, t->ntx * t->nty,
                           S.flags_new, S.background, ntiles);
    }
    VF_HIP_TRY(hipGetLastError());
    if (timed) VF_HIP_TRY(hipEventRecord(ev[2], side));
    VF_HIP_TRY(hipEventRecord(S.planned, side));
    K.mode = (first ? VF_PLAN_FIRST : 0u) | (fresh ? VF_PLAN_FRESH : 0u) | (M.on ? VF_PLAN_MOTION_MAP : 0u) | (dilate ? VF_PLAN_DILATE : 0u) |
             (reuse ? VF_PLAN_GEOMETRY_REUSED : 0u);
    K.set = set; K.ntiles = ntiles; K.motion_starts = motion_starts; K.rc_lo = rc_lo; K.rc_hi = rc_hi; K.seg_count = seg_count;
    return VF_OK;
}

static int overlay_pass(vf_terrain *t, hipStream_t s, const FrameParams &P, const SetupView &V)
{
    vf_terrain::Overlays &O = t->ov;
    const uint32_t nbx = (t->W + kOvBin - 1u) / kOvBin, nby = (t->H + kOvBin - 1u) / kOvBin, nbins = nbx * nby;
    const dim3 per_prim((O.nprims + 255u) / 256u), threads(256);
    const bool occlude = O.occluding != 0u;
    hipLaunchKernelGGL(k_ov_setup, per_prim, threads, 0, s, P, axis(t), O.nprims, O.in.p, O.prim.p, O.box.p, O.d_cnt, nbx,
                       occlude ? O.dep.p : nullptr);
    const dim3 per_slot((O.pg_hi - O.pg_lo + 255u) / 256u);
    if (O.nfill) {
        hipLaunchKernelGGL(k_pg_setup, per_slot, threads, 0, s, P, axis(t), O.pg_lo, O.pg_hi, O.in.p, O.prim.p, O.box.p, O.d_cnt, nbx, O.pg_fbox.p);
        hipLaunchKernelGGL(k_pg_header, dim3((O.nfill + 255u) / 256u), threads, 0, s, P, O.nfill, O.pg_hdr.p, O.in.p, O.pg_fbox.p, O.pg_fbin.p,
                           O.prim.p, O.box.p, O.d_cnt, nbx, O.pg_total.p);
    }
    hipLaunchKernelGGL(k_ov_scan, dim3(1), dim3(1024), 0, s, nbins, O.d_cnt, O.d_start);
    VF_HIP_TRY(hipGetLastError());
    VF_HIP_TRY(hipMemcpyAsync(O.h_total, O.d_start + nbins, sizeof(uint32_t), hipMemcpyDeviceToHost, s));
    if (O.nfill) {
        VF_HIP_TRY(hipMemcpyAsync(O.h_total + 2, O.pg_total.p, sizeof(unsigned long long), hipMemcpyDeviceToHost, s));
        VF_HIP_TRY(hipMemsetAsync(O.pg_total.p, 0, sizeof(unsigned long long), s));
    }
    VF_HIP_TRY(hipEventRecord(O.counted, s));
    VF_HIP_TRY(hipEventSynchronize(O.counted));
    const uint32_t total = *O.h_total;
    unsigned long long words = 0;
    if (O.nfill) std::memcpy(&words, O.h_total + 2, sizeof words);
    if (total == 0u) return VF_OK;
    if (total == 0xFFFFFFFFu) return fail(VF_ERR_NOMEM, "overlays: more than 2^32 - 2 (primitive, screen bin) pairs in one frame");
    if (words > 0xFFFFFFFFull) return fail(VF_ERR_NOMEM, "overlays: polygon fills reach more than 2^32 - 1 (feature, screen bin) pairs in one frame");
    hipError_t e = O.mask.reserve(words, words + words / 2u + 4096u);
    if (e != hipSuccess) return fail(VF_ERR_NOMEM, std::string("polygon mask allocation failed: ") + hipGetErrorString(e));
    if (words) {
        VF_HIP_TRY(hipMemsetAsync(O.mask.p, 0, (size_t)words * sizeof(uint32_t), s));
        hipLaunchKernelGGL(k_pg_backdrop, per_slot, threads, 0, s, t->H, O.pg_lo, O.pg_hi, O.in.p, O.prim.p, O.pg_fbin.p, O.mask.p);
        hipLaunchKernelGGL(k_pg_prefix, dim3((O.nfill + 3u) / 4u), threads, 0, s, O.nfill, O.pg_fbin.p, O.mask.p);
    }
    e = O.list.reserve(total, (size_t)total + total / 2u + 4096u);
    if (e != hipSuccess) return fail(VF_ERR_NOMEM, std::string("overlay pair list allocation failed: ") + hipGetErrorString(e));
    hipLaunchKernelGGL(k_ov_scatter, per_prim, threads, 0, s, O.nprims, O.box.p, nbx, O.d_start, O.d_cnt, O.list.p);
    if (occlude)
        hipLaunchKernelGGL(k_ov_composite_occlude, dim3(nbins), threads, 0, s, t->W, t->H, nbx, O.prim.p, O.d_cnt, O.d_start, O.list.p, t->ctx->d_decode,
                           t->ctx->d_thresh, O.mask.p, t->d_rgba, P, V, t->d_vis, O.dep.p);
    else
        hipLaunchKernelGGL(k_ov_composite, dim3(nbins), threads, 0, s, t->W, t->H, nbx, O.prim.p, O.d_cnt, O.d_start, O.list.p, t->ctx->d_decode,
                           t->ctx->d_thresh, O.mask.p, t->d_rgba);
    VF_HIP_TRY(hipGetLastError());
    return VF_OK;
}

static int relight_pass(vf_terrain *t, hipStream_t s, const FrameParams &P, const SetupView &V, const uint32_t *redo, uint32_t *rgba, Relight pass,
                        bool shadows, bool ambient);

static int viewshed_pass(vf_terrain *t, hipStream_t s, const FrameParams &P, const SetupView &V, const uint32_t *redo, uint32_t *rgba);
static int cumulative_pass(vf_terrain *t, hipStream_t s, const FrameParams &P, const SetupView &V, const uint32_t *redo, uint32_t *rgba);

static int draw_frame(vf_terrain *t, hipStream_t s, const FramePlan &K, bool diag)
{
    const FrameParams &P = K.P;
    const bool shadows = t->sh.enabled && !diag;
    const bool ambient = t->am.enabled && !diag;
    const bool drape = t->dr.iw != 0u && !diag;
    const Relight drape_pass = t->dm.enabled ? kDrapeMip : kDrape;
    const bool viewshed = t->vs.enabled && !diag;
    const bool cumulative = t->cv.enabled && !diag;
    const bool write_vis = diag || (t->ov.occluding && t->ov.nprims) || shadows || ambient || drape || viewshed || cumulative;
    vf_terrain::PlanState &S = t->ps[K.set];
    const uint32_t ntiles = K.ntiles, set = K.set;
    uint32_t *const rc_lo = K.rc_lo, *const rc_hi = K.rc_hi, *const seg_count = K.seg_count;
    vf_terrain::FrameEvents &ev = t->ev[t->timed_frames % (uint32_t)vf_terrain::kTimingRing];
    const bool timing_now = t->timing && K.sampled;
    const SetupView V = { S.vtx, t->d_hblk, S.recs, S.gen };
    uint32_t *stats = t->timing && t->stats_on ? t->d_stats : nullptr;
    const uint32_t nstats = (uint32_t)stats_layout(t).words;
    VF_HIP_TRY(hipStreamWaitEvent(s, S.planned, 0));
    VF_HIP_TRY(hipStreamWaitEvent(s, S.set_up, 0));
    if (t->last_stream && t->last_stream != s && t->rendered)
        VF_HIP_TRY(hipStreamWaitEvent(s, t->ps[t->last_set].drawn, 0));
    if (timing_now) VF_HIP_TRY(hipEventRecord(ev.begin, s));
    const int guess = t->nranks < (uint32_t)VF_GROUPS_MAX_RANKS ? 1 : 0;
    const LoopPick pick = t->loop.choose(guess, t->cursor.frames_since_reset <= 1 || K.motion_starts, ntiles != 0u);
    const bool groups = pick.variant != 0;
    LineLoop::Probe *gp = pick.probe ? t->loop.arm(s) : nullptr;
    if (ntiles) {
        uint32_t *vis = write_vis ? t->d_vis : nullptr;
        hipLaunchKernelGGL(k_clear, dim3(ntiles), dim3(256), 0, s, P, S.background, t->d_rgba, vis, stats, nstats, seg_count);
        const dim3 per_cu(std::min<uint32_t>((uint32_t)std::max(1, t->ctx->prop.multiProcessorCount) * (1024u / (uint32_t)kTileThreads), ntiles + kSplitBudget)),
                   few(std::min<uint32_t>(64u, ntiles + kSplitBudget)), threads(kTileThreads);
#define VF_TILE_ARGS P, V, S.row_ranges, S.cap_seg, S.cap_rad, t->d_lut, t->ctx->d_thresh, S.work_sorted, S.work_count, \
                     rc_lo, rc_hi, t->d_rgba, vis, stats, S.feedback, S.redo, S.band
        const bool fast = fast_shading(t->inputs);
#define VF_TILE_LAUNCH(WV, FS)                                                                                         \
        do {                                                                                                           \
            if (groups) hipLaunchKernelGGL((k_tile<WV, false, FS, true>), per_cu, threads, 0, s, VF_TILE_ARGS);        \
            else hipLaunchKernelGGL((k_tile<WV, false, FS, false>), per_cu, threads, 0, s, VF_TILE_ARGS);              \
            hipLaunchKernelGGL((k_tile<WV, true, FS, false>), few, threads, 0, s, VF_TILE_ARGS);                       \
        } while (0)
        if (write_vis && fast) VF_TILE_LAUNCH(true, true);
        else if (write_vis) VF_TILE_LAUNCH(true, false);
        else if (fast) VF_TILE_LAUNCH(false, true);
        else VF_TILE_LAUNCH(false, false);
#undef VF_TILE_LAUNCH
#undef VF_TILE_ARGS
        if (gp) t->loop.close(gp, s);
    }
    else VF_HIP_TRY(hipMemsetAsync(seg_count, 0, sizeof(uint32_t), s));
    if (timing_now) { VF_HIP_TRY(hipEventRecord(ev.end, s)); t->timed_frames++; }
    if ((shadows || ambient) && ntiles) {
        const int src = relight_pass(t, s, P, V, S.work_count + 3, t->d_rgba, ambient ? kAmbient : kShadow, shadows, ambient);
        if (src != VF_OK) return src;
    }
    if (drape && ntiles) {
        const int drc = relight_pass(t, s, P, V, S.work_count + 3, t->d_rgba, drape_pass, shadows, ambient);
        if (drc != VF_OK) return drc;
    }
    if (cumulative && ntiles) {
        const int crc = cumulative_pass(t, s, P, V, S.work_count + 3, t->d_rgba);
        if (crc != VF_OK) return crc;
    }
    if (viewshed && ntiles) {
        const int vrc = viewshed_pass(t, s, P, V, S.work_count + 3, t->d_rgba);
        if (vrc != VF_OK) return vrc;
    }
    if (t->ov.nprims && !diag) {
        const int orc = overlay_pass(t, s, P, V);
        if (orc != VF_OK) return orc;
    }
    VF_HIP_TRY(hipEventRecord(S.drawn, s));
    VF_HIP_TRY(hipGetLastError());
    std::memcpy(S.u_used, t->inputs.u, sizeof S.u_used);
    S.have_u_used = true;
    t->last_stream = s;
    t->last_set = set;
    t->rendered = true;
    return VF_OK;
}

static void plan_ahead(vf_terrain *t, hipStream_t s)
{
    vf_terrain::PrePlan &R = t->pre;
    R.before = t->cursor;
    if (plan_frame(t, s, R.K) == VF_OK) { R.valid = true; R.gen = t->inputs_gen; R.geom = t->geom_gen; }
    else {
        t->cursor = R.before;
        (void)hipGetLastError();
    }
}

static void flush_preplan(vf_terrain *t, hipStream_t s)
{
    if (!t->preplan_pending) return;
    t->preplan_pending = false;
    if (t->pre.valid || t->side || t->last_drawn_geom != t->geom_gen || t->bounds_dirty || s != t->last_stream) return;
    plan_ahead(t, s);
}

static hipError_t finish_readback(vf_terrain *t, hipStream_t s)
{
    if (!t->preplan_pending) return hipStreamSynchronize(s);
    hipError_t e = t->copied ? hipSuccess : hipEventCreateWithFlags(&t->copied, hipEventDisableTiming);
    if (e != hipSuccess) { t->preplan_pending = false; return hipStreamSynchronize(s); }
    e = hipEventRecord(t->copied, s);
    if (e != hipSuccess) return e;
    flush_preplan(t, s);
    return hipEventSynchronize(t->copied);
}

static int render_impl(vf_terrain *t, hipStream_t s, bool write_vis)
{
    FramePlan K;
    bool planned = false;
    const bool idle_at_entry = t->rendered && hipEventQuery(t->ps[t->last_set].drawn) == hipSuccess;
    (void)hipGetLastError();
    const bool streaming = t->rendered && !idle_at_entry;
    t->preplan_pending = false;
    if (t->pre.valid) {
        t->pre.valid = false;
        if (t->pre.geom == t->geom_gen && !write_vis) {
            K = t->pre.K; planned = true;
            if (t->pre.gen != t->inputs_gen) build_params(t, t->inputs, K.P);
            if (!t->side) {
                const bool ready = hipEventQuery(t->ps[K.set].planned) == hipSuccess;
                (void)hipGetLastError();
                t->tight_calls = ready ? 0u : t->tight_calls + 1u;
                if (t->tight_calls >= 3u) t->want_plan_streams = true;
            }
        }
        else { t->pre.valid = true; VF_HIP_TRY(drop_preplan(t, s)); }
    }
    if (!planned) { const int rc = plan_frame(t, s, K, streaming); if (rc != VF_OK) return rc; }
    const bool again = t->last_drawn_geom == t->geom_gen;
    const int rc = draw_frame(t, s, K, write_vis);
    if (rc != VF_OK) return rc;
    t->last_plan_mode = K.mode | (planned ? VF_PLAN_QUEUED_AHEAD : 0u);
    t->last_drawn_geom = t->geom_gen;
    if (again && (idle_at_entry || t->side) && !write_vis && !t->bounds_dirty && !t->cursor.camera_moving && !t->cursor.was_moving && t->cursor.frames_since_reset > vf_terrain::kPlanStates && !(t->timing && t->stats_on)) {
        if (t->side) plan_ahead(t, s);
        else t->preplan_pending = true;
    }
    return VF_OK;
}

static int render_recorded(vf_terrain *t, hipStream_t s)
{
    t->drawn_inputs = t->inputs;
    t->have_frame = true;
    return render_impl(t, s, false);
}

int vf_terrain_render(vf_terrain *t, void *stream)
{
    if (!t) return fail(VF_ERR_INVALID, "NULL argument");
    if (!t->have_uniforms) return fail(VF_ERR_INVALID, "uniforms not set");
    VF_HIP_TRY(hipSetDevice(t->ctx->device));
    return render_recorded(t, stream ? (hipStream_t)stream : t->ctx->stream);
}

int vf_terrain_render_batch(vf_terrain *t, const float *uniforms, uint32_t n, void *const *dev_rgba, void *stream)
{
    if (!t || (!uniforms && n)) return fail(VF_ERR_INVALID, "NULL argument");
    if (t->sh.enabled) return fail(VF_ERR_INVALID, "render_batch on a handle with shadows enabled is not supported: a sun per pose would need a shadow field per pose");
    if (t->am.enabled) return fail(VF_ERR_INVALID, "render_batch on a handle with ambient occlusion enabled is not supported");
    if (t->dr.iw) return fail(VF_ERR_INVALID, "render_batch on a handle that holds a draped image is not supported");
    if (t->vs.enabled) return fail(VF_ERR_INVALID, "render_batch on a handle with a viewshed enabled is not supported");
    if (t->cv.enabled) return fail(VF_ERR_INVALID, "render_batch on a handle with a cumulative viewshed enabled is not supported");
    VF_HIP_TRY(hipSetDevice(t->ctx->device));
    hipStream_t s = stream ? (hipStream_t)stream : t->ctx->stream;
    for (uint32_t k = 0; k < n; ++k) {
        if (dev_rgba && !dev_rgba[k]) return fail(VF_ERR_INVALID, "dev_rgba holds a NULL output buffer");
        take_uniforms(t, uniforms + 44u * k);
        if (dev_rgba) t->d_rgba = (uint32_t *)dev_rgba[k];
        const int rc = render_recorded(t, s);
        if (rc != VF_OK) return rc;
    }
    return VF_OK;
}

int vf_terrain_render_batch_host(vf_terrain *t, const float *uniforms, uint32_t n, uint8_t *const *host_rgba)
{
    if (!t || !uniforms || !host_rgba) return fail(VF_ERR_INVALID, "NULL argument");
    if (t->shard_tiles || t->local_rows != t->H) return fail(VF_ERR_INVALID, "batch read-back needs the whole frame on one handle (pose-parallel ranks are replicas)");
    if (t->sh.enabled) return fail(VF_ERR_INVALID, "render_batch on a handle with shadows enabled is not supported: a sun per pose would need a shadow field per pose");
    if (t->am.enabled) return fail(VF_ERR_INVALID, "render_batch on a handle with ambient occlusion enabled is not supported");
    if (t->dr.iw) return fail(VF_ERR_INVALID, "render_batch on a handle that holds a draped image is not supported");
    if (t->vs.enabled) return fail(VF_ERR_INVALID, "render_batch on a handle with a viewshed enabled is not supported");
    if (t->cv.enabled) return fail(VF_ERR_INVALID, "render_batch on a handle with a cumulative viewshed enabled is not supported");
    for (uint32_t k = 0; k < n; ++k) if (!host_rgba[k]) return fail(VF_ERR_INVALID, "host_rgba holds a NULL destination");
    VF_HIP_TRY(hipSetDevice(t->ctx->device));
    constexpr uint32_t R = vf_terrain::kBatchRing;
    const size_t frame_bytes = (size_t)t->W * t->H * 4, slot_bytes = (size_t)t->ntx * t->nty * kTileW * kTileH * 4;
    VF_HIP_TRY(ctx_copy_stream(t->ctx, &t->copy_stream));
    for (uint32_t r = 0; r < R && r < n; ++r) {
        if (!t->d_batch[r]) VF_HIP_TRY(hipMalloc(&t->d_batch[r], slot_bytes));
        if (!t->batch_drawn[r]) VF_HIP_TRY(hipEventCreateWithFlags(&t->batch_drawn[r], hipEventDisableTiming));
        if (!t->batch_copied[r]) VF_HIP_TRY(hipEventCreateWithFlags(&t->batch_copied[r], hipEventDisableTiming));
    }
    hipStream_t s = t->ctx->stream;
    uint32_t *const out_before = t->d_rgba;
    int rc = VF_OK;
    hipError_t err = hipSuccess;
    for (uint32_t k = 0; k < n && rc == VF_OK && err == hipSuccess; ++k) {
        const uint32_t r = k % R;
        if (k >= R) err = hipStreamWaitEvent(s, t->batch_copied[r], 0);
        if (err != hipSuccess) break;
        rc = vf_terrain_render_batch(t, uniforms + 44u * k, 1, (void *const *)&t->d_batch[r], s);
        if (rc != VF_OK) break;
        err = hipEventRecord(t->batch_drawn[r], s);
        if (err == hipSuccess) err = hipStreamWaitEvent(t->copy_stream, t->batch_drawn[r], 0);
        if (err == hipSuccess) err = hipMemcpyAsync(host_rgba[k], t->d_batch[r], frame_bytes, hipMemcpyDeviceToHost, t->copy_stream);
        if (err == hipSuccess) err = hipEventRecord(t->batch_copied[r], t->copy_stream);
    }
    const hipError_t e2 = hipStreamSynchronize(t->copy_stream);
    const hipError_t e3 = hipStreamSynchronize(s);
    t->d_rgba = out_before;
    t->rendered = false;
    if (rc != VF_OK) return rc;
    if (err != hipSuccess) return fail(VF_ERR_HIP, std::string("batch read-back: ") + hipGetErrorString(err));
    if (e2 != hipSuccess || e3 != hipSuccess) return fail(VF_ERR_HIP, std::string("batch read-back: ") + hipGetErrorString(e2 != hipSuccess ? e2 : e3));
// ... 369 lines not shown
        VF_HIP_TRY(hipGetLastError());
        VF_HIP_TRY(hipStreamSynchronize(s));
        return VF_OK;
    }, {}, 0, false, t->ov.features + 1u, layer_id, occlude != 0);
    if (rc == VF_OK && nsegments) *nsegments = (uint32_t)nseg;
    return rc;
}

int vf_terrain_clear_overlays(vf_terrain *t)
{
    if (!t) return fail(VF_ERR_INVALID, "NULL argument");
    VF_HIP_TRY(wait_frame(t));
    ov_release(t);
    return VF_OK;
}

constexpr size_t kStageChunk = 8u << 20;
constexpr size_t kStageSlots = 4;
static unsigned copy_threads()
{
    if (const char *e = std::getenv("VF_COPY_THREADS")) { const int v = std::atoi(e); if (v >= 1) return (unsigned)std::min(v, 16); }
    const unsigned hw = std::thread::hardware_concurrency();
    return std::max(1u, std::min(4u, hw > 1 ? hw - 1 : 1u));
}
static bool is_pinned_host(const void *p)
{
    hipPointerAttribute_t a;
    if (hipPointerGetAttributes(&a, p) != hipSuccess) { (void)hipGetLastError(); return false; }
    return a.type == hipMemoryTypeHost;
}
static hipError_t copy_to_pinned(void *host, const void *dev, size_t n, hipStream_t s)
{
    void *view = nullptr;
    if (n >= 4096 && hipHostGetDevicePointer(&view, host, 0) == hipSuccess && view && (((uintptr_t)view | (uintptr_t)dev) & 15u) == 0) {
        const size_t n16 = n / 16;
        const unsigned grid = (unsigned)std::min<size_t>(1024, (n16 + 255) / 256);
        hipLaunchKernelGGL(k_copy_to_host, dim3(grid), dim3(256), 0, s, (const uint4 *)dev, (uint4 *)view, n16, n);
        return hipGetLastError();
    }
    (void)hipGetLastError();
    return hipMemcpyAsync(host, dev, n, hipMemcpyDeviceToHost, s);
}
static int copy_to_host_staged(vf_terrain *t, uint8_t *dst, const uint8_t *src, size_t n, hipStream_t s)
{
    if (is_pinned_host(dst)) { VF_HIP_TRY(copy_to_pinned(dst, src, n, s)); VF_HIP_TRY(finish_readback(t, s)); return VF_OK; }
    if (n < kStageChunk) { VF_HIP_TRY(hipMemcpyAsync(dst, src, n, hipMemcpyDeviceToHost, s)); VF_HIP_TRY(finish_readback(t, s)); return VF_OK; }
    if (!t->h_stage) VF_HIP_TRY(pinned_alloc((void **)&t->h_stage, kStageSlots * kStageChunk));
    for (auto &e : t->stage_ev) if (!e) VF_HIP_TRY(hipEventCreateWithFlags(&e, hipEventDisableTiming));
    const size_t nchunks = (n + kStageChunk - 1) / kStageChunk;
    const unsigned nthreads = copy_threads();
    auto chunk_len = [&](size_t k) { return k + 1 == nchunks ? n - k * kStageChunk : kStageChunk; };
    std::atomic<size_t> enqueued{0};
    std::unique_ptr<std::atomic<uint32_t>[]> done(new std::atomic<uint32_t>[nchunks]);
    for (size_t k = 0; k < nchunks; ++k) done[k].store(0, std::memory_order_relaxed);
    std::atomic<int> failed{0};
    const int device = t->ctx->device;
    auto worker = [&](unsigned w) {
        (void)hipSetDevice(device);
        for (size_t k = 0; k < nchunks; ++k) {
            while (enqueued.load(std::memory_order_acquire) <= k) {
                if (failed.load(std::memory_order_relaxed)) return;
                std::this_thread::yield();
            }
            if (hipEventSynchronize(t->stage_ev[k % kStageSlots]) != hipSuccess) failed.store(1);
            else {
                const size_t len = chunk_len(k);
                const size_t lo = (len * w / nthreads) & ~(size_t)4095, hi = w + 1 == nthreads ? len : (len * (w + 1) / nthreads) & ~(size_t)4095;
                if (hi > lo) std::memcpy(dst + k * kStageChunk + lo, t->h_stage + (k % kStageSlots) * kStageChunk + lo, hi - lo);
            }
            done[k].fetch_add(1, std::memory_order_release);
        }
    };
    std::vector<std::thread> pool;
    pool.reserve(nthreads);
    for (unsigned w = 0; w < nthreads; ++w) pool.emplace_back(worker, w);
    hipError_t err = hipSuccess;
    for (size_t i = 0; i < nchunks && err == hipSuccess && !failed.load(); ++i) {
        if (i >= kStageSlots)
            while (done[i - kStageSlots].load(std::memory_order_acquire) < nthreads) std::this_thread::yield();
        err = copy_to_pinned(t->h_stage + (i % kStageSlots) * kStageChunk, src + i * kStageChunk, chunk_len(i), s);
        if (err == hipSuccess) err = hipEventRecord(t->stage_ev[i % kStageSlots], s);
        if (err == hipSuccess) enqueued.store(i + 1, std::memory_order_release);
    }
    if (err == hipSuccess) flush_preplan(t, s);
    if (err != hipSuccess) failed.store(1);
    for (auto &th : pool) th.join();
    if (err != hipSuccess) return fail(VF_ERR_HIP, hipGetErrorString(err));
    if (failed.load()) return fail(VF_ERR_HIP, "device -> host copy failed");
    return VF_OK;
}

int vf_terrain_read_rgba(vf_terrain *t, uint8_t *dst, uint32_t y0, uint32_t rows)
{
    if (!t || !dst) return fail(VF_ERR_INVALID, "NULL argument");
    if (!t->rendered) return fail(VF_ERR_INVALID, "nothing rendered yet");
    if (t->shard_tiles) return fail(VF_ERR_INVALID, "tile-sharded handle: read with vf_terrain_read_tiles");
    if ((uint64_t)y0 + rows > t->local_rows) return fail(VF_ERR_INVALID, "row range outside the local rows");
    int rc = vf_terrain_sync(t);
    if (rc != VF_OK) return rc;
    return copy_to_host_staged(t, dst, (const uint8_t *)(t->d_rgba + (size_t)y0 * t->W), (size_t)rows * t->W * 4,
                               t->last_stream ? t->last_stream : t->ctx->stream);
}

int vf_host_alloc(size_t bytes, void **host)
{
    if (!host || bytes == 0) return fail(VF_ERR_INVALID, "NULL argument or zero size");
    *host = nullptr;
    hipError_t e = pinned_alloc(host, bytes);
    if (e != hipSuccess) { *host = nullptr; return fail(e == hipErrorOutOfMemory ? VF_ERR_NOMEM : VF_ERR_HIP, std::string("page-locked allocation: ") + hipGetErrorString(e)); }
    return VF_OK;
}
void vf_host_free(void *host) { pinned_free(host); }

int vf_terrain_read_png_scanlines(vf_terrain *t, const uint8_t **host_scanlines, size_t *nbytes)
{
    if (!t || !host_scanlines || !nbytes) return fail(VF_ERR_INVALID, "NULL argument");
    if (!t->rendered) return fail(VF_ERR_INVALID, "nothing rendered yet");
    if (t->shard_tiles || t->local_rows != t->H) return fail(VF_ERR_INVALID, "PNG read-back needs the whole frame on one handle");
    VF_HIP_TRY(hipSetDevice(t->ctx->device));
    const size_t n = ((size_t)t->W * 4 + 1) * t->H;
    if (!t->d_png) VF_HIP_TRY(hipMalloc(&t->d_png, n));
    hipStream_t s = t->last_stream ? t->last_stream : t->ctx->stream;
    hipLaunchKernelGGL(k_png_filter, dim3(t->H), dim3(256), 0, s, (const uint32_t *)t->d_rgba, t->W, t->d_png);
    VF_HIP_TRY(hipGetLastError());
    if (!t->h_png) VF_HIP_TRY(pinned_alloc((void **)&t->h_png, n));
    uint8_t *host = t->h_png;
    VF_HIP_TRY(copy_to_pinned(host, t->d_png, n, s));
    VF_HIP_TRY(finish_readback(t, s));
    *host_scanlines = host;
    *nbytes = n;
    return VF_OK;
}

int vf_terrain_read_visibility(vf_terrain *t, uint32_t *dst)
{
    if (!t || !dst) return fail(VF_ERR_INVALID, "NULL argument");
    if (!t->have_uniforms) return fail(VF_ERR_INVALID, "uniforms not set");
    if (t->shard_tiles) return fail(VF_ERR_INVALID, "visibility read-back needs a row-oriented handle (vf_terrain_set_shard)");
    VF_HIP_TRY(hipSetDevice(t->ctx->device));
    int rc = render_visibility(t);
    if (rc != VF_OK) return rc;
    VF_HIP_TRY(hipMemcpy(dst, t->d_vis, (size_t)t->local_rows * t->W * sizeof(uint32_t), hipMemcpyDeviceToHost));
    return VF_OK;
}

static dim3 region_grid(const vf_terrain *t, uint32_t regions, const char *env, uint32_t per_cu)
{
    if (const char *v = std::getenv(env)) per_cu = (uint32_t)std::max(1, std::atoi(v));
    const uint32_t cus = (uint32_t)std::max(8, t->ctx->prop.multiProcessorCount) / 8u * 8u;
    return dim3(std::min<uint32_t>((regions + 7u) / 8u * 8u, cus * per_cu));
}

int vf_terrain_debug_fragment_stage(vf_terrain *t, uint32_t repeats, vf_fragment_timing *out)
{
    if (!t || !out) return fail(VF_ERR_INVALID, "NULL argument");
    if (!t->have_uniforms) return fail(VF_ERR_INVALID, "uniforms not set");
    if (t->shard_tiles || t->nranks != 1) return fail(VF_ERR_INVALID, "fragment-stage diagnostics need a whole-frame handle");
    if (repeats == 0) repeats = 1;
    VF_HIP_TRY(hipSetDevice(t->ctx->device));
    int rc = render_visibility(t);
    if (rc != VF_OK) return rc;
    const size_t npx = (size_t)t->W * t->H;
    uint32_t *d_out = nullptr;
    VF_HIP_TRY(hipMalloc(&d_out, npx * sizeof(uint32_t)));
    if (!t->d_diag) { hipError_t e = hipMalloc(&t->d_diag, 4 * sizeof(uint32_t)); if (e != hipSuccess) { (void)hipFree(d_out); return fail(VF_ERR_NOMEM, "diagnostics allocation failed"); } }
    uint32_t redo = 0;
    hipError_t err = hipMemcpy(&redo, t->ps[t->last_set].work_count + 3, sizeof redo, hipMemcpyDeviceToHost);
// ... 1071 lines not shown
    held.hold(t);
    int rc = VF_OK;
    float a = 0.0f;
    const hipError_t err = time_launches(s, repeats, a, [&](bool) { rc = cumulative_field(t, t->inputs.u, s, true); return rc == VF_OK ? hipSuccess : hipErrorUnknown; });
    if (rc != VF_OK) return rc;
    if (err != hipSuccess) return fail(VF_ERR_HIP, std::string("cumulative viewshed diagnostics: ") + hipGetErrorString(err));
    *ms = a;
    return VF_OK;
}

int vf_terrain_debug_item_stats(vf_terrain *t, uint32_t *dst, uint32_t max_items, uint32_t *count)
{
    if (!t || !dst || !count) return fail(VF_ERR_INVALID, "NULL argument");
    if (!t->timing || !t->stats_on || !t->rendered) return fail(VF_ERR_INVALID, "statistics not enabled or nothing rendered");
    int rc = vf_terrain_sync(t);
    if (rc != VF_OK) return rc;
    uint32_t n = 0;
    VF_HIP_TRY(hipMemcpy(&n, t->ps[t->last_set].work_count, sizeof n, hipMemcpyDeviceToHost));
    if (n > max_items) n = max_items;
    if (n) VF_HIP_TRY(hipMemcpy(dst, t->d_stats + 4, 4 * (size_t)n * sizeof(uint32_t), hipMemcpyDeviceToHost));
    *count = n;
    return VF_OK;
}

int vf_terrain_debug_band_masks(vf_terrain *t, uint32_t *recs, uint64_t *masks, int32_t *xy, uint32_t max_blocks, uint32_t *count)
{
    static_assert(VF_BAND_SLOTS == (uint32_t)kBandSlots, "the header's slot count is the kernels'");
    if (!t || !count) return fail(VF_ERR_INVALID, "NULL argument");
    if (!t->rendered) return fail(VF_ERR_INVALID, "nothing rendered");
    if (max_blocks < t->nblocks) return fail(VF_ERR_INVALID, "max_blocks is smaller than the grid's blocks");
    const vf_terrain::PlanState &S = t->ps[t->last_set];
    if (!S.slab) return fail(VF_ERR_INVALID, "nothing rendered");
    VF_HIP_TRY(wait_frame(t));
    VF_HIP_TRY(sync_sides(t));
    const size_t nb = t->nblocks;
    if (recs) VF_HIP_TRY(hipMemcpy(recs, S.recs, nb * sizeof(BlockRec), hipMemcpyDeviceToHost));
    if (masks) VF_HIP_TRY(hipMemcpy(masks, S.band, nb * kBandSlots * sizeof(ulonglong2), hipMemcpyDeviceToHost));
    if (xy) {
        std::vector<VertexRec> v(nb * kBlockStride);
        VF_HIP_TRY(hipMemcpy(v.data(), S.vtx, v.size() * sizeof(VertexRec), hipMemcpyDeviceToHost));
        for (size_t k = 0; k < v.size(); ++k) { xy[2 * k] = v[k].X; xy[2 * k + 1] = v[k].Y; }
    }
    *count = (uint32_t)nb;
    return VF_OK;
}

int vf_terrain_debug_set_plan_feedback(vf_terrain *t, const uint32_t *tile_ticks, const uint8_t *strips_log2, const uint32_t *piece_ticks,
                                       uint32_t ntiles)
{
    if (!t || !tile_ticks || !strips_log2) return fail(VF_ERR_INVALID, "NULL argument");
    if (ntiles != t->local_tiles) return fail(VF_ERR_INVALID, "ntiles must be the handle's local tiles");
    for (uint32_t k = 0; k < ntiles; ++k) if (strips_log2[k] > 4u) return fail(VF_ERR_INVALID, "strips_log2 must be 0 .. 4");
    if (t->cursor.frames_since_reset < vf_terrain::kPlanStates)
        return fail(VF_ERR_INVALID, "the handle's first frames are planned from the static estimate: render two frames first");
    for (const auto &S : t->ps) if (!S.slab) return fail(VF_ERR_INVALID, "a plan state has not been used yet: render two frames first");
    VF_HIP_TRY(hipSetDevice(t->ctx->device));
    VF_HIP_TRY(wait_frame(t));
    VF_HIP_TRY(sync_sides(t));
    VF_HIP_TRY(drop_preplan(t));
    VF_HIP_TRY(wait_frame(t));
    VF_HIP_TRY(sync_sides(t));
    if (!ntiles) return VF_OK;
    const size_t all_tiles = (size_t)t->ntx * t->nty;
    std::vector<uint32_t> pieces((size_t)ntiles * 64u, 0u), flags(ntiles);
    if (piece_ticks) std::memcpy(pieces.data(), piece_ticks, pieces.size() * sizeof(uint32_t));
    for (auto &S : t->ps) {
        VF_HIP_TRY(hipMemcpy(S.feedback, tile_ticks, (size_t)ntiles * sizeof(uint32_t), hipMemcpyHostToDevice));
        VF_HIP_TRY(hipMemcpy(S.feedback + all_tiles + 1u, pieces.data(), pieces.size() * sizeof(uint32_t), hipMemcpyHostToDevice));
        VF_HIP_TRY(hipMemcpy(flags.data(), S.background, (size_t)ntiles * sizeof(uint32_t), hipMemcpyDeviceToHost));
        for (uint32_t k = 0; k < ntiles; ++k) flags[k] = (flags[k] & 0xFFu) | ((uint32_t)strips_log2[k] << 8);
        VF_HIP_TRY(hipMemcpy(S.background, flags.data(), (size_t)ntiles * sizeof(uint32_t), hipMemcpyHostToDevice));
    }
    return VF_OK;
}

int vf_terrain_debug_plan_mode(const vf_terrain *t, uint32_t *mode)
{
    if (!t || !mode) return fail(VF_ERR_INVALID, "NULL argument");
    if (!t->rendered) return fail(VF_ERR_INVALID, "nothing rendered yet");
    *mode = t->last_plan_mode;
    return VF_OK;
}

int vf_terrain_debug_phase_cycles(vf_terrain *t, uint64_t *dst, uint32_t n)
{
    if (!t || !dst) return fail(VF_ERR_INVALID, "NULL argument");
#ifndef VF_PHASE_PROF
    (void)n;
    return fail(VF_ERR_INVALID, "library built without -DVF_PHASE_PROF");
#else
    if (!t->timing || !t->stats_on || !t->rendered) return fail(VF_ERR_INVALID, "statistics not enabled or nothing rendered");
    int rc = vf_terrain_sync(t);
    if (rc != VF_OK) return rc;
    if (n > kPhaseSlots) n = kPhaseSlots;
    VF_HIP_TRY(hipMemcpy(dst, t->d_stats + stats_layout(t).phases, n * sizeof(uint64_t), hipMemcpyDeviceToHost));
    return VF_OK;
#endif
}

int vf_terrain_enable_timing(vf_terrain *t, int enable)
{
    if (!t) return fail(VF_ERR_INVALID, "NULL argument");
    if (enable != 0 && !t->ev[0].begin) {
        VF_HIP_TRY(hipSetDevice(t->ctx->device));
        for (auto &f : t->ev) { VF_HIP_TRY(hipEventCreate(&f.begin)); VF_HIP_TRY(hipEventCreate(&f.end)); }
    }
    if (enable != 0) for (auto &S : t->ps) for (auto &e : S.pev) if (!e) VF_HIP_TRY(hipEventCreate(&e));
    if (enable < 0 || enable > 3) return fail(VF_ERR_INVALID, "enable must be 0 .. 3");
    t->timing = enable != 0;
    t->stats_on = enable == 1;
    t->timing_every = enable == 3 ? 4u : 1u;
    t->timed_frames = 0;
    return VF_OK;
}

int vf_terrain_timings(vf_terrain *t, vf_timings *out)
{
    if (!t || !out) return fail(VF_ERR_INVALID, "NULL argument");
    if (!t->timing || !t->rendered || t->timed_frames == 0) return fail(VF_ERR_INVALID, "timing not enabled or nothing rendered");
    int rc = vf_terrain_sync(t);
    if (rc != VF_OK) return rc;
    const uint32_t nf = t->timed_frames < (uint32_t)vf_terrain::kTimingRing ? t->timed_frames : (uint32_t)vf_terrain::kTimingRing;
    double ranges = 0, plan = 0, tile = 0, total = 0;
    uint32_t nplan = 0;
    for (uint32_t f = 0; f < nf; ++f) {
        float c = 0;
        VF_HIP_TRY(hipEventSynchronize(t->ev[f].end));
        VF_HIP_TRY(hipEventElapsedTime(&c, t->ev[f].begin, t->ev[f].end));
        tile += c; total += c;
    }
    VF_HIP_TRY(sync_sides(t));
    for (auto &S : t->ps) {
        if (!S.pev_valid || !S.pev[2]) continue;
        float a = 0, b = 0;
        if (hipEventSynchronize(S.pev[2]) != hipSuccess || hipEventElapsedTime(&a, S.pev[0], S.pev[1]) != hipSuccess ||
            hipEventElapsedTime(&b, S.pev[1], S.pev[2]) != hipSuccess) { (void)hipGetLastError(); continue; }
        ranges += a; plan += b; ++nplan;
    }
    if (nf == 1u && t->ps[t->last_set].pev_valid) {
        float d = 0;
        if (hipEventElapsedTime(&d, t->ps[t->last_set].pev[0], t->ev[0].end) == hipSuccess && d > 0.0f) total = d;
        else (void)hipGetLastError();
    }
    out->ranges_ms = nplan ? (float)(ranges / nplan) : 0.0f; out->plan_ms = nplan ? (float)(plan / nplan) : 0.0f; out->tile_ms = (float)(tile / nf);
    out->total_ms = (float)(total / nf);
    if (nf >= 2 && t->timed_frames <= (uint32_t)vf_terrain::kTimingRing) {
        float span = 0;
        VF_HIP_TRY(hipEventElapsedTime(&span, t->ev[0].end, t->ev[nf - 1].end));
        out->total_ms = span / (float)((nf - 1) * t->timing_every);
    }
    out->frames = nf;
    out->blocks_rasterised = 0; out->blocks_distinct = 0;
    out->tiles = t->local_tiles;
    if (t->stats_on) {
        uint32_t c[4];
        VF_HIP_TRY(hipMemcpy(c, t->d_stats, sizeof c, hipMemcpyDeviceToHost));
        out->blocks_rasterised = c[0];
        std::vector<uint32_t> bits((t->nblocks + 31) / 32);
        VF_HIP_TRY(hipMemcpy(bits.data(), t->d_stats + stats_layout(t).block_bits, bits.size() * sizeof(uint32_t), hipMemcpyDeviceToHost));
        uint32_t n = 0;
        for (uint32_t w : bits) n += (uint32_t)__builtin_popcount(w);
        out->blocks_distinct = n;
    }
    return VF_OK;
}

// ... 615 lines not shown
```

vulkan_forge_amd/csrc/vf_kernels.h:

```cpp
#pragma once
#include "vf_device.h"
#include "vf_raster.h"

namespace vf {

__global__ void k_axis_tables(uint32_t n, uint32_t tw, uint32_t th, float *xs, float *sinx, float *cosz,
                              int32_t *txi, int32_t *tyj)
{
    uint32_t i = blockIdx.x * blockDim.x + threadIdx.x;
    if (i >= n) return;
    const float scale = 1.5f;
    const float nm1f = (float)n - 1.0f;
    const float step = (2.0f * scale) / nm1f;
    float x = -scale + (float)i * step;
    float uvc = (float)i / nm1f;
    xs[i] = x;
    sinx[i] = det_sin(x * 1.3f);
    cosz[i] = det_cos(x * 1.1f);
    int tx = (int)floorf(uvc * (float)tw), ty = (int)floorf(uvc * (float)th);
    txi[i] = min(max(tx, 0), (int)tw - 1);
    tyj[i] = min(max(ty, 0), (int)th - 1);
}

__global__ __launch_bounds__(64) void k_height_blocks(uint32_t n, uint32_t nb, uint32_t tw, AxisTables A,
// ... 918 lines not shown
__device__ __forceinline__ uint32_t work_tile(uint32_t code) { return code & 0xFFFFFu; }
__device__ __forceinline__ uint32_t work_part(uint32_t code) { return (code >> 20) & 15u; }
__device__ __forceinline__ uint32_t work_slice(uint32_t code) { return (code >> 27) & 3u; }
__device__ __forceinline__ uint32_t work_lg_slices(uint32_t code) { return (code >> 29) & 3u; }
__device__ __forceinline__ void work_strip(uint32_t code, int32_t &px_lo, int32_t &px_hi)
{
    const uint32_t lg = (code >> 24) & 7u, part = (code >> 20) & 15u;
    const int32_t w = kTileW >> lg;
    const int32_t lo = px_lo + (int32_t)part * w;
    px_hi = min(px_hi, lo + w - 1);
    px_lo = lo;
}


__device__ __forceinline__ uint32_t tile_reach(const FrameParams &P, const PixelBox *__restrict__ row_boxes, const uint32_t *__restrict__ rc_lo,
                                               const uint32_t *__restrict__ rc_hi, uint32_t tcol, int32_t py_lo, int32_t py_hi,
                                               uint32_t *s_hits, uint32_t *s_est)
{
    if (threadIdx.x == 0) { *s_hits = 0; *s_est = 0; }
    __syncthreads();
    uint32_t hits = 0, est = 0;
    for (uint32_t r = threadIdx.x; r < P.nb; r += 256) {
        const PixelBox rr = row_boxes[r];
        const uint32_t lo = rc_lo[tcol * P.nb + r], hi = rc_hi[tcol * P.nb + r];
        if (lo < hi && rr.x0 <= rr.x1 && rr.y1 >= py_lo && rr.y0 <= py_hi) { ++hits; est += hi - lo; }
    }
    for (int o = 32; o > 0; o >>= 1) { hits += __shfl_xor(hits, o); est += __shfl_xor(est, o); }
    if ((threadIdx.x & 63u) == 0 && hits) { atomicAdd(s_hits, hits); atomicAdd(s_est, est); }
    __syncthreads();
    return *s_hits;
}
__device__ __forceinline__ uint32_t static_ticks(uint32_t blocks) { return max(blocks * 25u, 1u); }

__device__ __forceinline__ bool capsule_hits_rect(const float4 &seg, float rad, int32_t px_lo, int32_t px_hi, int32_t py_lo, int32_t py_hi);
__global__ __launch_bounds__(256) void k_plan_estimate(FrameParams P, const PixelBox *__restrict__ row_boxes, const BlockRec *__restrict__ recs,
                                                       const float4 *__restrict__ cap_seg, const float *__restrict__ cap_rad,
                                                       const uint32_t *__restrict__ rc_lo, const uint32_t *__restrict__ rc_hi,
                                                       uint32_t *__restrict__ feedback)
{
    constexpr uint32_t kEstDepth = 24;
    __shared__ uint32_t s_est, s_top[8], s_stop;
    int32_t px_lo, px_hi, py_lo, py_hi;
    const TilePlace tp = tile_rect(P, blockIdx.x, px_lo, px_hi, py_lo, py_hi);
    if (threadIdx.x < 8u) s_top[threadIdx.x] = 0u;
    if (threadIdx.x == 0) { s_est = 0; s_stop = 0; }
    __syncthreads();
    const uint32_t sub = threadIdx.x & 7u, rsub = threadIdx.x >> 3;
    uint32_t est = 0;
    for (uint32_t base = 0; base < P.nb; base += 32u) {
        const uint32_t k = base + rsub;
        if (k < P.nb) {
            const uint32_t r = P.nb - 1u - k;
            const PixelBox rr = row_boxes[r];
            const uint32_t lo = rc_lo[tp.tx * P.nb + r], hi = rc_hi[tp.tx * P.nb + r];
            if (lo < hi && rr.x0 <= rr.x1 && rr.y1 >= py_lo && rr.y0 <= py_hi)
                for (uint32_t bx = lo + sub; bx < hi; bx += 8u) {
                    const uint4 rw = *reinterpret_cast<const uint4 *>(recs + r * P.nb + bx);
                    const PixelBox b = PixelBox{ (int16_t)(rw.x & 0xFFFFu), (int16_t)(rw.x >> 16), (int16_t)(rw.y & 0xFFFFu), (int16_t)(rw.y >> 16) };
                    if (!(b.x0 <= b.x1 && b.x1 >= px_lo && b.x0 <= px_hi && b.y1 >= py_lo && b.y0 <= py_hi)) continue;
                    if (!capsule_hits_rect(cap_seg[r * P.nb + bx], cap_rad[r * P.nb + bx], px_lo, px_hi, py_lo, py_hi)) continue;
                    const float ov = (float)((min((int32_t)b.x1, px_hi) - max((int32_t)b.x0, px_lo) + 1) * (min((int32_t)b.y1, py_hi) - max((int32_t)b.y0, py_lo) + 1));
                    const float area = (float)(((int32_t)b.x1 - (int32_t)b.x0 + 1) * ((int32_t)b.y1 - (int32_t)b.y0 + 1));
                    est += 32u + (uint32_t)(29.0f * (float)rw.w * ov / area);
                    if ((int32_t)b.y0 <= py_lo && (int32_t)b.y1 >= py_lo + 7)
                        for (int32_t c = max(((int32_t)b.x0 - px_lo + 7) >> 3, 0); c <= min(((int32_t)b.x1 - px_lo - 7) >> 3, 7); ++c) atomicAdd(&s_top[c], 1u);
                }
        }
        __syncthreads();
        if (threadIdx.x == 0) {
            uint32_t least = s_top[0];
            for (int c = 1; c < 8; ++c) least = min(least, s_top[c]);
            s_stop = least >= kEstDepth ? 1u : 0u;
        }
        __syncthreads();
        if (s_stop) break;
    }
    for (int o = 32; o > 0; o >>= 1) est += __shfl_xor(est, o);
    if ((threadIdx.x & 63u) == 0 && est) atomicAdd(&s_est, est);
    __syncthreads();
    if (threadIdx.x == 0) {
        const uint32_t ticks = max(s_est / 16u, 1u);
        feedback[blockIdx.x] = ticks;
        feedback[(size_t)P.ntx * P.nty + 1u + (size_t)blockIdx.x * 64u] = ticks;
    }
}

__global__ __launch_bounds__(256) void k_plan(FrameParams P, const PixelBox *__restrict__ row_boxes, uint32_t *__restrict__ flags_out,
                                              uint2 *__restrict__ work, uint32_t *__restrict__ work_count,
                                              const uint32_t *__restrict__ last_blocks, const uint32_t *__restrict__ last_mean,
                                              uint32_t *__restrict__ split_budget, const uint32_t *__restrict__ rc_lo,
                                              const uint32_t *__restrict__ rc_hi, uint32_t moving, const uint32_t *last_flags, MotionMap M)
{
    __shared__ uint32_t s_hits, s_est;
    int32_t px_lo, px_hi, py_lo, py_hi;
    const TilePlace tp = tile_rect(P, blockIdx.x, px_lo, px_hi, py_lo, py_hi);
    const uint32_t total = tile_reach(P, row_boxes, rc_lo, rc_hi, tp.tx, py_lo, py_hi, &s_hits, &s_est);
    if (total) {
        if (threadIdx.x == 0) {
            const bool as_one = P.nranks == 1u && !P.shard_tiles;
            auto tile_time = [&](uint32_t idx) -> uint32_t {
                uint32_t t = last_blocks[idx];
                const uint32_t f = last_flags[idx];
                const uint32_t lg = (f >> 8) & 15u;
                const uint32_t lgp = lg + ((f >> 12) & 3u);
                if (t && lgp && lgp <= 6u) {
                    const uint32_t *pc = last_blocks + (size_t)P.ntx * P.nty + 1u + (size_t)idx * 64u;
                    uint32_t pk = 0;
                    for (uint32_t p = 0; p < (1u << lgp); ++p) pk = max(pk, pc[p]);
                    t = max(t, (uint32_t)min((unsigned long long)pk << lgp, 0xFFFFFFFFull));
                }
                return as_one ? (uint32_t)(((unsigned long long)t * 4ull) / (4ull + lg + ((f >> 12) & 3u))) : t;
            };
            uint32_t seen = tile_time(blockIdx.x);
            const uint32_t mean = *last_mean;
            bool own_time = true;
            if (M.on && as_one) {
                const float cx = 0.5f * (float)(px_lo + px_hi + 1), cy = 0.5f * (float)(py_lo + py_hi + 1);
                const float ox = fmaf(M.m[0], cx, fmaf(M.m[1], cy, M.m[2])), oy = fmaf(M.m[3], cx, fmaf(M.m[4], cy, M.m[5])), ow = fmaf(M.m[6], cx, fmaf(M.m[7], cy, M.m[8]));
                seen = 0u; own_time = false;
                if (ow > 1e-6f) {
                    const float fx = ox / ow, fy = oy / ow;
                    if (fx > -64.0f && fy > -64.0f && fx < (float)P.W + 64.0f && fy < (float)P.H + 64.0f) {
                        const int32_t tx = (int32_t)floorf(fx * (1.0f / kTileW)), ty = (int32_t)floorf(fy * (1.0f / kTileH));
                        for (int32_t dy = -1; dy <= 1; ++dy)
                            for (int32_t dx = -1; dx <= 1; ++dx) {
                                const int32_t x = tx + dx, y = ty + dy;
                                if (x >= 0 && y >= 0 && x < (int32_t)P.ntx && y < (int32_t)P.nty) seen = max(seen, tile_time((uint32_t)y * P.ntx + (uint32_t)x));
                            }
                    }
                }
                {
                    const int32_t tx = (int32_t)tp.tx, ty = (int32_t)(blockIdx.x / P.ntx);
                    for (int32_t dy = -1; dy <= 1; ++dy)
                        for (int32_t dx = -2; dx <= 2; ++dx) {
                            const int32_t x = tx + dx, y = ty + dy;
                            if (x >= 0 && y >= 0 && x < (int32_t)P.ntx && y < (int32_t)P.nty) seen = max(seen, tile_time((uint32_t)y * P.ntx + (uint32_t)x));
                        }
                }
            }
            else if ((seen == 0u || moving) && mean && P.nranks == 1u && !P.shard_tiles) {
                const int32_t tx = (int32_t)tp.tx, ty = (int32_t)(blockIdx.x / P.ntx);
                const int32_t reach = seen ? 1 : 2;
                for (int32_t dy = -reach; dy <= reach; ++dy)
                    for (int32_t dx = -reach; dx <= reach; ++dx) {
                        const int32_t x = tx + dx, y = ty + dy;
                        if (x >= 0 && y >= 0 && x < (int32_t)P.ntx && y < (int32_t)P.nty) seen = max(seen, tile_time((uint32_t)y * P.ntx + (uint32_t)x));
                    }
            }
            const uint32_t weight = seen ? seen : static_ticks(s_est);
            uint32_t lg = 0, lgs = 0;
            if (mean && px_hi - px_lo + 1 == kTileW) {
                const uint32_t q = seen / mean;
                lg = q >= 16u ? 4u : q >= 8u ? 3u : q >= 4u ? 2u : q >= 2u ? 1u : 0u;
                while (lg + lgs && atomicAdd(split_budget, (1u << (lg + lgs)) - 1u) + (1u << (lg + lgs)) - 1u > kSplitBudget) {
                    atomicSub(split_budget, (1u << (lg + lgs)) - 1u);
                    if (lgs) --lgs; else --lg;
                }
            }
            const uint32_t cut = lg | (lgs << 4);
            const bool same_cut = own_time && seen == tile_time(blockIdx.x) && seen != 0u && ((last_flags[blockIdx.x] >> 8) & 0x3Fu) == cut;
            const uint32_t *piece_time = last_blocks + (size_t)P.ntx * P.nty + 1u + (size_t)blockIdx.x * 64u;
            flags_out[blockIdx.x] = cut << 8;
            const uint32_t parts = 1u << lg, slices = 1u << lgs;
            const uint32_t at = atomicAdd(work_count, parts * slices);
            for (uint32_t p = 0; p < parts; ++p)
                for (uint32_t sl = 0; sl < slices; ++sl)
// ... 12 lines not shown
    if (blockIdx.x == 0 && threadIdx.x == 0) *seg_count = 0u;
    if (stats) for (uint32_t k = blockIdx.x * 256u + threadIdx.x; k < nstats; k += gridDim.x * 256u) stats[k] = 0u;
    if ((background[blockIdx.x] & 1u) == 0u) return;
    int32_t px_lo, px_hi, py_lo, py_hi;
    const TilePlace tp = tile_rect(P, blockIdx.x, px_lo, px_hi, py_lo, py_hi);
    const int32_t w = px_hi - px_lo + 1, h = py_hi - py_lo + 1;
    if (w == kTileW && (tp.out_stride & 3u) == 0u && (tp.out_base & 3u) == 0u && (reinterpret_cast<uintptr_t>(rgba) & 15u) == 0u &&
        (!vis_out || (reinterpret_cast<uintptr_t>(vis_out) & 15u) == 0u)) {
        const uint4 c4 = make_uint4(P.clear_rgba, P.clear_rgba, P.clear_rgba, P.clear_rgba), z4 = make_uint4(0u, 0u, 0u, 0u);
        for (int32_t k = threadIdx.x; k < (kTileW / 4) * h; k += 256) {
            const int32_t ly = k / (kTileW / 4), q = k - ly * (kTileW / 4);
            const size_t o = tp.out_base + (size_t)ly * tp.out_stride + 4u * (uint32_t)q;
            *reinterpret_cast<uint4 *>(rgba + o) = c4;
            if (vis_out) *reinterpret_cast<uint4 *>(vis_out + o) = z4;
        }
        return;
    }
    for (int32_t k = threadIdx.x; k < w * h; k += 256) {
        const int32_t ly = k / w, lx = k - ly * w;
        const size_t o = tp.out_base + (size_t)ly * tp.out_stride + (uint32_t)lx;
        rgba[o] = P.clear_rgba;
        if (vis_out) vis_out[o] = 0u;
    }
}

__global__ __launch_bounds__(256) void k_plan_sort(const uint2 *__restrict__ work, uint2 *__restrict__ sorted, const uint32_t *__restrict__ work_count,
                                                   uint32_t *__restrict__ last_blocks, uint32_t ntiles,
                                                   const uint32_t *__restrict__ flags_new, uint32_t *__restrict__ background, uint32_t nlocal)
{
    constexpr uint32_t kKeys = 1024, kT = 256;
    __shared__ uint32_t s_hist[kKeys];
    __shared__ uint32_t s_kr[4096];
    __shared__ uint32_t s_wsum[kT / 64];
    const uint32_t n = *work_count, tid = threadIdx.x, lane = tid & 63u, wave = tid >> 6;
    for (uint32_t k = tid; k < ntiles; k += kT) last_blocks[k] = 0u;
    for (uint32_t k = tid; k < nlocal; k += kT) background[k] = flags_new[k];
    for (uint32_t base = 0; base < n; base += 4096) {
        const uint32_t m = min(4096u, n - base);
        for (uint32_t k = tid; k < kKeys; k += kT) s_hist[k] = 0u;
        __syncthreads();
#pragma unroll 1
        for (uint32_t k = tid; k < m; k += kT) {
            const uint32_t f = (__float_as_uint((float)max(work[base + k].y, 1u)) >> 18) - (127u << 5);
            const uint32_t key = (kKeys - 1u) - min(f, kKeys - 1u);
            s_kr[k] = key | (atomicAdd(&s_hist[key], 1u) << 10);
        }
        __syncthreads();
        const uint32_t a0 = s_hist[4u * tid], a1 = s_hist[4u * tid + 1u], a2 = s_hist[4u * tid + 2u], a3 = s_hist[4u * tid + 3u];
        const uint32_t mine = a0 + a1 + a2 + a3;
        const uint32_t inc = wave_scan_add(mine);
        if (lane == 63u) s_wsum[wave] = inc;
        __syncthreads();
        uint32_t before = 0;
#pragma unroll
        for (uint32_t w = 0; w < kT / 64; ++w) before += w < wave ? s_wsum[w] : 0u;
        const uint32_t first = before + inc - mine;
        s_hist[4u * tid] = first; s_hist[4u * tid + 1u] = first + a0; s_hist[4u * tid + 2u] = first + a0 + a1; s_hist[4u * tid + 3u] = first + a0 + a1 + a2;
        __syncthreads();
#pragma unroll 1
        for (uint32_t k = tid; k < m; k += kT) {
            const uint32_t kr = s_kr[k];
            sorted[base + s_hist[kr & (kKeys - 1u)] + (kr >> 10)] = work[base + k];
        }
        __syncthreads();
    }
}

#ifdef VF_PHASE_PROF
struct PhaseClock {
    uint64_t acc[20], last;
    __device__ __forceinline__ void start() { for (int k = 0; k < 20; ++k) acc[k] = 0; last = __builtin_readcyclecounter(); }
    __device__ __forceinline__ void tick(int p) { const uint64_t now = __builtin_readcyclecounter(); acc[p] += now - last; last = now; }
};
#define VF_PH_INIT PhaseClock PH; PH.start();
#define VF_PH(p) PH.tick(p);
#define VF_PH_ARG , PhaseClock &PH
#define VF_PH_PASS , PH
#else
#define VF_PH_INIT
#define VF_PH(p)
#define VF_PH_ARG
#define VF_PH_PASS
#endif
namespace tile {
constexpr int kWaves = kTileThreads / 64;
constexpr int kNV = kBlockVerts * kBlockVerts;
constexpr uint32_t kChunk = 4096;
constexpr int kMaxSteps = 128;
constexpr int kHitWords = 16;
constexpr int kRescanEvery = 1;
constexpr int kBlockPrims = 2 * kBlockCells * kBlockCells;
constexpr uint32_t kWideLines = 28, kBalGain = 2;
struct WaveLds {
    int2 xy[kWaves][kNV];
    uint32_t surv[kWaves][kBlockPrims];
};
constexpr size_t kHitBytes = sizeof(unsigned long long) * kMaxSteps * kHitWords;
constexpr size_t kOverlayBytes = sizeof(WaveLds) > kHitBytes ? sizeof(WaveLds) : kHitBytes;
struct Lds {
    uint32_t *vis;
    unsigned long long (*hit)[kHitWords];
    int2 (*xy)[kNV]; uint32_t (*surv)[kBlockPrims];
    uint32_t *list;
    uint32_t *cnt;
    uint16_t *words;
    uint32_t *pending;
    uint32_t *firstid;
    uint16_t *allrows;
    uint32_t *rc;
    uint32_t *colfin, *rowfin, *colfin4, *rowfin4;
    uint32_t *part;
    unsigned long long *rows;
    uint32_t *next, *lock, *done, *frontier, *published, *blocks, *redo;
    const uint32_t *per;
};
__device__ __forceinline__ uint32_t lds_peek(const uint32_t *p) { return __hip_atomic_load(p, __ATOMIC_RELAXED, __HIP_MEMORY_SCOPE_WORKGROUP); }

__device__ __forceinline__ uint32_t list_block_rows(const FrameParams &P, const Lds &L, const TileCtx &T, const PixelBox *__restrict__ row_boxes,
                                                    const uint32_t *__restrict__ rc_lo, const uint32_t *__restrict__ rc_hi, uint32_t tcol,
                                                    uint32_t tid, uint32_t lane, uint32_t wave VF_PH_ARG)
{
    for (uint32_t base = 0; base < P.nb; base += kTileThreads) {
        const uint32_t r = base + tid;
        bool hit = false;
        if (r < P.nb) {
            const PixelBox rr = row_boxes[r];
            const uint32_t lo = rc_lo[tcol * P.nb + r], hi = rc_hi[tcol * P.nb + r];
            L.rc[r] = lo < hi ? lo | (hi << 16) : 1u;
            hit = lo < hi && rr.x0 <= rr.x1 && rr.x1 >= T.px_lo && rr.x0 <= T.px_hi && rr.y1 >= T.py_lo && rr.y0 <= T.py_hi;
        }
        const unsigned long long m = __ballot(hit);
        if (lane == 0 && m) L.rows[r >> 6] = m;
    }
    __syncthreads();
    VF_PH(14)

    uint32_t nrows_total = 0;
    {
        uint32_t cnt[16];
#pragma unroll
        for (uint32_t w = 0; w < 16u; ++w) { cnt[w] = (uint32_t)__popcll(L.rows[w]); nrows_total += cnt[w]; }
        for (uint32_t word = 15u - wave; word < 16u; word -= (uint32_t)kWaves) {
            uint32_t above = 0;
#pragma unroll
            for (uint32_t w = 0; w < 16u; ++w) above += w > word ? cnt[w] : 0u;
            const unsigned long long m = L.rows[word];
            const uint32_t b = 63u - lane;
            if ((m >> b) & 1ull) L.allrows[above + (uint32_t)__popcll(b == 63u ? 0ull : m >> (b + 1u))] = (uint16_t)(word * 64u + b);
        }
    }
    __syncthreads();

    return nrows_total;
}

template <bool GROUPS>
__device__ __forceinline__ void test_candidates_pairs(const FrameParams &P, const SetupView &V, const Lds &L, const TileCtx &T, const float4 *__restrict__ cap_seg,
                                                      const float *__restrict__ cap_rad, uint32_t cursor, uint32_t nrowsteps, uint32_t lane, uint32_t wave)
{
    const uint32_t rsub = lane >> 3, bsub = lane & 7u;
    uint32_t *const hit32 = reinterpret_cast<uint32_t *>(&L.hit[0][0]);
    for (uint32_t kbase = 0; kbase < nrowsteps; kbase += 8u * kWaves) {
        const uint32_t k = kbase + wave + rsub * kWaves;
        const bool valid = k < nrowsteps;
        uint32_t by = 0, lo = 1, hi = 0;
        if (valid) { by = L.allrows[cursor + k]; const uint32_t range = L.rc[by]; lo = range & 0xFFFFu; hi = range >> 16; }
// ... 31 lines not shown
            const bool valid = k < nrowsteps;
            by[r] = valid ? (uint32_t)__builtin_amdgcn_readfirstlane((int)L.allrows[cursor + k]) : 0u;
            const uint32_t range = valid ? (uint32_t)__builtin_amdgcn_readfirstlane((int)L.rc[by[r]]) : 1u;
            bx_lo[r] = range & 0xFFFFu;
            bx_hi[r] = range >> 16;
            cnt[r] = 0u;
        }
        uint32_t g_first = hit_words, g_last = 0;
#pragma unroll
        for (int r = 0; r < kRowsAtOnce; ++r)
            if (bx_lo[r] < bx_hi[r]) { g_first = min(g_first, bx_lo[r] >> 6); g_last = max(g_last, ((bx_hi[r] - 1u) >> 6) + 1u); }
        for (uint32_t g = g_first; g < g_last; ++g) {
            const uint32_t bx = g * 64u + lane;
            PixelBox box[kRowsAtOnce];
            float4 seg[kRowsAtOnce];
            float rad[kRowsAtOnce];
            bool in[kRowsAtOnce];
#pragma unroll
            for (int r = 0; r < kRowsAtOnce; ++r) {
                in[r] = bx >= bx_lo[r] && bx < bx_hi[r];
                box[r] = PixelBox{ 1, 1, 0, 0 }; seg[r] = make_float4(0.f, 0.f, 0.f, 0.f); rad[r] = 0.0f;
                if (in[r]) {
                    const uint32_t bidx = by[r] * P.nb + bx;
                    box[r] = V.recs[bidx].box; seg[r] = cap_seg[bidx]; rad[r] = cap_rad[bidx];
                }
            }
#pragma unroll
            for (int r = 0; r < kRowsAtOnce; ++r) {
                const uint32_t k = k0 + (uint32_t)r * kWaves;
                if (k >= nrowsteps) continue;
                const unsigned long long m = __ballot(in[r] && block_is_candidate<GROUPS>(box[r], seg[r], rad[r], T));
                if (lane == 0) L.hit[k][g] = m;
                cnt[r] += (uint32_t)__popcll(m);
            }
        }
#pragma unroll
        for (int r = 0; r < kRowsAtOnce; ++r) {
            const uint32_t k = k0 + (uint32_t)r * kWaves;
            if (lane == 0 && k < nrowsteps) { L.cnt[k] = cnt[r]; L.words[k] = (uint16_t)(g_first < g_last ? g_first | (g_last << 8) : 0u); L.firstid[k] = 2u * (by[r] * kBlockCells * P.nm1) + 1u; }
        }
    }
}

__device__ __forceinline__ void fill_work_list(const Lds &L, uint32_t cursor, uint32_t nrowsteps, uint32_t lane, uint32_t wave, uint32_t &nsteps, uint32_t &nlist)
{
    constexpr int kParts = kMaxSteps / 64;
    static_assert(kMaxSteps % 64 == 0 && kParts >= 1 && kParts <= 4, "the offset scan below works on 64-row parts");
    uint32_t c[kParts], inc[kParts];
    unsigned long long fm[kParts];
    asm volatile("" : "+v"(lane));
#pragma unroll
    for (int p = 0; p < kParts; ++p) {
        c[p] = lane + 64u * p < nrowsteps ? L.cnt[lane + 64u * p] : 0u;
        inc[p] = wave_scan_add(c[p]);
        if (p) inc[p] += (uint32_t)__builtin_amdgcn_readlane((int)inc[p - 1], 63);
        fm[p] = __ballot(lane + 64u * p < nrowsteps && inc[p] <= kChunk);
    }
    nsteps = 64u * kParts;
#pragma unroll
    for (int p = kParts - 1; p >= 0; --p) if (fm[p] != ~0ull) nsteps = 64u * p + (uint32_t)__builtin_ctzll(~fm[p]);
    auto row_value = [&](const uint32_t (&v)[kParts], uint32_t k) -> uint32_t {
        uint32_t r = (uint32_t)__builtin_amdgcn_readlane((int)v[0], (int)(k & 63u));
#pragma unroll
        for (int p = 1; p < kParts; ++p) if ((k >> 6) == (uint32_t)p) r = (uint32_t)__builtin_amdgcn_readlane((int)v[p], (int)(k & 63u));
        return r;
    };
    nlist = row_value(inc, nsteps - 1u);
    for (uint32_t k = wave; k < nsteps; k += kWaves) {
        const uint32_t by = (uint32_t)__builtin_amdgcn_readfirstlane((int)L.allrows[cursor + k]);
        uint32_t pos = row_value(inc, k) - row_value(c, k);
        uint32_t cnt = 0;
        const uint32_t words = (uint32_t)__builtin_amdgcn_readfirstlane((int)L.words[k]);
        for (uint32_t g = words & 0xFFu; g < (words >> 8); ++g) {
            const unsigned long long m = L.hit[k][g];
            if ((m >> lane) & 1ull) L.list[pos + (uint32_t)__popcll(m & ((1ull << lane) - 1ull))] = (g * 64u + lane) | (by << 10) | (k << 20);
            const uint32_t c = (uint32_t)__popcll(m);
            pos += c; cnt += c;
        }
        if (lane == 0) L.pending[k] = cnt;
    }
}

template <bool GROUPS>
__device__ __forceinline__ uint32_t publish_chunk_masks(const Lds &L, uint32_t nsteps, uint32_t lane, uint32_t wave)
{
    {
        constexpr int kRowsPerWave = kTileH / kWaves;
        uint32_t lane_here = lane;
        asm volatile("" : "+v"(lane_here));
        const uint32_t nfinal = rescan_final(L.vis, L.colfin, L.rowfin, lane_here, L.firstid[nsteps - 1], (int32_t)wave * kRowsPerWave,
                                             (int32_t)(wave + 1) * kRowsPerWave);
        if (lane == 0) L.part[wave] = nfinal;
    }
    __syncthreads();
    if constexpr (GROUPS)
        if (wave == 0) refresh_fin4(L.colfin, L.rowfin, L.colfin4, L.rowfin4, lane);
    uint32_t all = 0;
#pragma unroll
    for (int w = 0; w < kWaves; ++w) all += L.part[w];
    return all;
}

template <bool WRITE_VIS, bool COMPLETE, bool FAST>
__device__ __forceinline__ void shade_item(const FrameParams &P, const SetupView &V, const ShadeTables &S, const Lds &L, const TileCtx &T, const TilePlace &tp, int32_t tile_x0,
                                           uint32_t *__restrict__ rgba, uint32_t *__restrict__ vis_out, uint32_t tid)
{
    const int32_t item_w = T.px_hi - T.px_lo + 1;
    if (item_w > 32 || (item_w & (item_w - 1)) != 0) {
        for (int k = tid; k < kTileW * kTileH; k += kTileThreads) {
            const int32_t lx = k & (kTileW - 1), ly = k / kTileW;
            const int32_t px = T.px_lo + lx, py = T.py_lo + ly;
            if (px > T.px_hi || py > T.py_hi) continue;
            const uint32_t id = L.vis[vis_index(lx, ly)];
            const size_t o = tp.out_base + (size_t)ly * tp.out_stride + (uint32_t)(px - tile_x0);
            rgba[o] = id ? shade_pixel<COMPLETE, FAST>(P, V, S, id - 1u, px, py) : P.clear_rgba;
            if (WRITE_VIS) vis_out[o] = id;
        }
    } else {
        const int32_t w_shift = 31 - __builtin_clz(item_w);
        for (int k = tid; k < ((T.py_hi - T.py_lo + 1) << w_shift); k += kTileThreads) {
            const int32_t ly = k >> w_shift, lx = k - (ly << w_shift);
            const int32_t px = T.px_lo + lx, py = T.py_lo + ly;
            const uint32_t id = L.vis[vis_index(lx, ly)];
            const size_t o = tp.out_base + (size_t)ly * tp.out_stride + (uint32_t)(px - tile_x0);
            rgba[o] = id ? shade_pixel<COMPLETE, FAST>(P, V, S, id - 1u, px, py) : P.clear_rgba;
            if (WRITE_VIS) vis_out[o] = id;
        }
    }
}
}

template <bool WRITE_VIS, bool COMPLETE, bool FAST, bool GROUPS>
__global__ __launch_bounds__(kTileThreads, VF_TILE_MIN_WAVES) void k_tile(FrameParams P, SetupView V, const PixelBox *__restrict__ row_boxes,
                                                       const float4 *__restrict__ cap_seg, const float *__restrict__ cap_rad,
                                                       const float *__restrict__ lut_linear, const float *__restrict__ thresh,
                                                       const uint2 *__restrict__ work, uint32_t *__restrict__ work_count,
                                                       const uint32_t *__restrict__ rc_lo, const uint32_t *__restrict__ rc_hi,
                                                       uint32_t *__restrict__ rgba, uint32_t *__restrict__ vis_out, uint32_t *stats,
                                                       uint32_t *__restrict__ last_blocks, uint32_t *__restrict__ redo,
                                                       const ulonglong2 *__restrict__ band)
{
    using namespace tile;
    uint32_t *const redo_count = work_count + 3;
    __shared__ uint32_t s_vis[kTileW * kTileH];
    __shared__ __attribute__((aligned(16))) unsigned char s_overlay[kOverlayBytes];
    __shared__ uint32_t s_list[kChunk];
    __shared__ uint32_t s_cnt[kMaxSteps];
    __shared__ uint16_t s_words[kMaxSteps];
    __shared__ uint32_t s_pending[kMaxSteps];
    __shared__ uint32_t s_firstid[kMaxSteps];
    __shared__ uint16_t s_allrows[1024];
    __shared__ uint32_t s_rc[1024];
    __shared__ uint32_t s_colfin[kTileW * 2];
    __shared__ uint32_t s_rowfin[kTileH * 2];
    __shared__ uint32_t s_colfin4[kTileW / 4 * 2], s_rowfin4[kTileH / 4 * 2];
    __shared__ uint32_t s_part[kWaves];
    __shared__ unsigned long long s_rows[16];
    __shared__ uint32_t s_next, s_lock, s_done, s_frontier, s_published, s_blocks, s_redo, s_item;
    __shared__ __attribute__((aligned(16))) float s_lut[kLutFloats];
    __shared__ float s_thr[256];
    __shared__ uint32_t s_per[65];
    WaveLds &s_wave = *reinterpret_cast<WaveLds *>(s_overlay);
    int2 (&sXY)[kWaves][kNV] = s_wave.xy;
    uint32_t (&sS)[kWaves][kBlockPrims] = s_wave.surv;
    Lds L;
    L.vis = s_vis; L.hit = reinterpret_cast<unsigned long long (*)[kHitWords]>(s_overlay);
    L.xy = s_wave.xy; L.surv = s_wave.surv;
    L.list = s_list; L.cnt = s_cnt; L.words = s_words; L.pending = s_pending; L.firstid = s_firstid; L.allrows = s_allrows; L.rc = s_rc;
    L.colfin = s_colfin; L.rowfin = s_rowfin; L.colfin4 = s_colfin4; L.rowfin4 = s_rowfin4; L.part = s_part; L.rows = s_rows;
    L.next = &s_next; L.lock = &s_lock; L.done = &s_done; L.frontier = &s_frontier; L.published = &s_published; L.blocks = &s_blocks; L.redo = &s_redo;
    L.per = s_per;

    const uint32_t tid = threadIdx.x, lane = tid & 63u;
    const uint32_t wave = (uint32_t)__builtin_amdgcn_readfirstlane((int)(tid >> 6));
    VF_PH_INIT
    VF_RC(RasterCounts RC = {};)
    uint32_t redo_at = blockIdx.x;
    if (COMPLETE && redo_at >= *redo_count) return;
    for (int k = tid; k < kLutFloats; k += kTileThreads) s_lut[k] = lut_linear[k];
    for (int k = tid; k < 256; k += kTileThreads) s_thr[k] = thresh[k];
    if (tid <= 64u) { const uint32_t per = tid ? 64u / tid : 64u; s_per[tid] = per | (((65536u + per - 1u) / per) << 7) | ((64u / per) << 24); }
    const ShadeTables S = { s_lut, s_thr };
    const uint32_t nwork = *work_count;
    uint32_t pulled = 0;
    if (!COMPLETE) {
        if (tid == 0) s_item = atomicAdd(work_count + 2, 1u);
        __syncthreads();
        pulled = (uint32_t)__builtin_amdgcn_readfirstlane((int)s_item);
        if (pulled >= nwork) return;
    }
    for (;;) {
    VF_PH(12)
    const uint32_t item_idx = COMPLETE ? redo[redo_at] : pulled;
    const uint64_t t_start = __builtin_amdgcn_s_memrealtime();
    const uint32_t item = work[item_idx].x;
    const uint32_t tile = work_tile(item);
    TileCtx T;
    T.vis = s_vis; T.colfin = s_colfin; T.rowfin = s_rowfin; T.colfin4 = s_colfin4; T.rowfin4 = s_rowfin4;
    const TilePlace tp = tile_rect(P, tile, T.px_lo, T.px_hi, T.py_lo, T.py_hi);
    const uint32_t tcol = tp.tx;
    static_assert(kTileH == 64, "the set-up pass folds rows of 64 pixels");
    const uint32_t band_slot = (uint32_t)__builtin_amdgcn_readfirstlane((int)(((uint32_t)T.py_lo >> 6) & ((uint32_t)kBandSlots - 1u)));
    const int32_t tile_x0 = T.px_lo;
    work_strip(item, T.px_lo, T.px_hi);
    const uint32_t tile_pixels = (uint32_t)(T.px_hi - T.px_lo + 1) * (uint32_t)(T.py_hi - T.py_lo + 1);
    const uint64_t row_full = ~0ull >> (63 - (T.px_hi - T.px_lo));

    for (int k = tid; k < kTileW * kTileH; k += kTileThreads) s_vis[k] = 0u;
    for (int k = tid; k < kTileW * 2; k += kTileThreads) s_colfin[k] = 0u;
    for (int k = tid; k < kTileH * 2; k += kTileThreads) s_rowfin[k] = 0u;
    if (tid < kTileW / 4 * 2) { s_colfin4[tid] = 0u; s_rowfin4[tid] = 0u; }
    if (tid < 16) s_rows[tid] = 0ull;
    if (tid == 0) { s_done = 0; s_blocks = 0; s_redo = 0; }
    __syncthreads();
    VF_PH(13)
    const uint32_t nrows_total = list_block_rows(P, L, T, row_boxes, rc_lo, rc_hi, tcol, tid, lane, wave VF_PH_PASS);
    VF_PH(8)
    uint32_t dbg_loop = 0;
    const uint32_t hit_words = (P.nb + 63u) / 64u;
    for (uint32_t cursor = 0; cursor < nrows_total;) {
        const uint32_t nrowsteps = min((uint32_t)kMaxSteps, nrows_total - cursor);
        if (tid == 0) { s_next = 0; s_lock = 0; s_frontier = 0; s_published = 0; }
        if (!GROUPS) test_candidates_pairs<GROUPS>(P, V, L, T, cap_seg, cap_rad, cursor, nrowsteps, lane, wave);
        else test_candidates_rows<GROUPS>(P, V, L, T, cap_seg, cap_rad, cursor, nrowsteps, hit_words, lane, wave);
        VF_PH(9)
        __syncthreads();
        VF_PH(10)
        uint32_t nsteps, nlist;
        fill_work_list(L, cursor, nrowsteps, lane, wave, nsteps, nlist);
        cursor += nsteps;
        VF_PH(11)
        __syncthreads();
        VF_PH(0)

        uint32_t my_blocks = 0;
        const uint64_t dbg_t0 = kDiagItem == 1 ? __builtin_amdgcn_s_memrealtime() : 0ull;
        for (;;) {
            uint32_t idx = 0;
            if (lane == 0) idx = atomicAdd(&s_next, 1u);
            idx = (uint32_t)__builtin_amdgcn_readfirstlane((int)idx);
            if (idx >= nlist) break;
            const uint32_t entry = (uint32_t)__builtin_amdgcn_readfirstlane((int)s_list[idx]);
            const uint32_t bx = entry & 0x3FFu, by = (entry >> 10) & 0x3FFu, stepidx = entry >> 20;
            if (GROUPS) {
                const uint32_t fr_now = lds_peek(&s_frontier);
                if (stepidx <= fr_now) __builtin_amdgcn_s_setprio(2); else if (stepidx == fr_now + 1u) __builtin_amdgcn_s_setprio(1); else __builtin_amdgcn_s_setprio(0);
            }
            const uint32_t bidx = by * P.nb + bx;
            typedef uint32_t __attribute__((ext_vector_type(4))) rec_words;
            const rec_words rw = *(const __attribute__((address_space(4))) rec_words *)(uintptr_t)(V.recs + bidx);
            const rec_words bw = *(const __attribute__((address_space(4))) rec_words *)(uintptr_t)(band + (size_t)bidx * kBandSlots + band_slot);
            const uint4 r_lo = make_uint4(rw[0], rw[1], rw[2], rw[3]), r_hi = make_uint4(bw[0], bw[1], bw[2], bw[3]);
            const uint4 *vsrc = reinterpret_cast<const uint4 *>(V.vtx + (size_t)bidx * kBlockStride);
            const uint4 va4 = vsrc[lane];
            uint4 vb4 = make_uint4(0u, 0u, 0u, 0u);
            if (lane < (uint32_t)(kNV - 64)) vb4 = vsrc[64u + lane];
            const int2 xa = make_int2((int32_t)va4.x, (int32_t)va4.y), xb = make_int2((int32_t)vb4.x, (int32_t)vb4.y);
            bool live;
            {
                const int32_t bx0 = (int32_t)(int16_t)(r_lo.x & 0xFFFFu), by0 = (int32_t)(int16_t)(r_lo.x >> 16);
                const int32_t bx1 = (int32_t)(int16_t)(r_lo.y & 0xFFFFu), by1 = (int32_t)(int16_t)(r_lo.y >> 16);
                const int32_t x0 = max(bx0, T.px_lo) - T.px_lo, x1 = min(bx1, T.px_hi) - T.px_lo;
                const int32_t y0 = max(by0, T.py_lo) - T.py_lo, y1 = min(by1, T.py_hi) - T.py_lo;
                const bool in = (int32_t)lane >= x0 && (int32_t)lane <= x1;
                const uint64_t open = in ? (~load_mask(s_colfin, (int32_t)lane) & bit_range(y0, y1)) : 0ull;
                live = __ballot(open != 0ull) != 0ull;
            }
            VF_PH(1)
            if (live) {
                ++my_blocks;
#ifndef VF_PHASE_PROF
                if (stats && lane == 0)
                    atomicOr(&stats[4u + 4u * (P.ntx * P.nty + kSplitBudget) + 2u * kPhaseSlots + (bidx >> 5)], 1u << (bidx & 31u));
#endif
                const uint32_t i0 = bx * kBlockCells, j0 = by * kBlockCells;
                const unsigned long long alive_e = (unsigned long long)(uint32_t)__builtin_amdgcn_readfirstlane((int)r_hi.x) | ((unsigned long long)(uint32_t)__builtin_amdgcn_readfirstlane((int)r_hi.y) << 32);
                const unsigned long long alive_o = (unsigned long long)(uint32_t)__builtin_amdgcn_readfirstlane((int)r_hi.z) | ((unsigned long long)(uint32_t)__builtin_amdgcn_readfirstlane((int)r_hi.w) << 32);
                const uint32_t rflags = (uint32_t)__builtin_amdgcn_readfirstlane((int)r_lo.z);
                VF_PH(16)
                VF_PH(17)
#ifdef VF_PHASE_PROF
                asm volatile("s_waitcnt vmcnt(0)" ::: "memory");
                VF_PH(18)
#endif
                sXY[wave][lane] = xa;
                if (lane < (uint32_t)(kNV - 64)) sXY[wave][64u + lane] = xb;
#ifdef VF_PHASE_PROF
                asm volatile("s_waitcnt lgkmcnt(0)" ::: "memory");
                VF_PH(19)
#endif
                if (!COMPLETE && (rflags & kRecGeneric)) { if (lane == 0) s_redo = 1u; }
                const uint32_t n_even = (uint32_t)__popcll(alive_e), n_alive = n_even + (uint32_t)__popcll(alive_o);
                {
                    const uint32_t pe = __builtin_amdgcn_mbcnt_hi((uint32_t)(alive_e >> 32), __builtin_amdgcn_mbcnt_lo((uint32_t)alive_e, 0u));
                    const uint32_t po = __builtin_amdgcn_mbcnt_hi((uint32_t)(alive_o >> 32), __builtin_amdgcn_mbcnt_lo((uint32_t)alive_o, 0u));
                    if ((alive_e >> lane) & 1ull) sS[wave][pe] = 2u * lane;
                    if ((alive_o >> lane) & 1ull) sS[wave][n_even + po] = 2u * lane + 1u;
                }
                __builtin_amdgcn_wave_barrier();
                VF_PH(2)
                if constexpr (COMPLETE) if (rflags & kRecGeneric) {
                    const ulonglong2 g = V.gen[bidx];
                    const uint32_t lj = lane >> 3, li = lane & 7u;
                    const uint32_t prim = 2u * ((j0 + lj) * P.nm1 + (i0 + li));
                    GVert gv[3];
                    if ((g.x >> lane) & 1ull) { load_prim(P, V.hblk, prim, gv[0], gv[1], gv[2]); raster_generic(gv, P.hw, P.hh, P.W, P.H, T.vis, T.px_lo, T.px_hi, T.py_lo, T.py_hi, prim + 1u); }
                    if ((g.y >> lane) & 1ull) { load_prim(P, V.hblk, prim + 1u, gv[0], gv[1], gv[2]); raster_generic(gv, P.hw, P.hh, P.W, P.H, T.vis, T.px_lo, T.px_hi, T.py_lo, T.py_hi, prim + 2u); }
                }
                uint32_t nsurv = 0;
                bool any_wide = false;
                uint32_t n_cls = n_alive;
                if constexpr (!GROUPS) n_cls = min(n_alive, 64u);
// ... 552 lines not shown
```

Measured before the change: 25750.

## Precompute per-tile candidate block lists when geometry is reused across frames

Adds a k_tile_lists kernel that, when plan geometry is reused, builds a compact per-tile list of candidate blocks (packed pixel boxes and ids) on a side stream. The tile raster kernel then reads these lists instead of rescanning block rows and testing every candidate in each frame. The intent is to cut the per-tile setup and candidate-testing work on static-camera frames. The cost is extra device memory, event dependencies and a more complex path, with a fallback when capacity is exceeded or the lists are stale.

```diff
diff --git a/include/vf_hip.h b/include/vf_hip.h
--- a/include/vf_hip.h
+++ b/include/vf_hip.h
@@ -131,7 +131,11 @@
 #define VF_PLAN_DILATE       8u
 #define VF_PLAN_QUEUED_AHEAD 16u
 #define VF_PLAN_GEOMETRY_REUSED 32u
+#define VF_PLAN_TILE_LISTS   64u
 int vf_terrain_debug_plan_mode(const vf_terrain *t, uint32_t *mode);
+typedef struct vf_tile_list_info { uint32_t built, used, tiles_listed, tiles_fallback, entries, capacity, units_asked, reserved; } vf_tile_list_info;
+int vf_terrain_debug_tile_lists(vf_terrain *t, vf_tile_list_info *out);
+int vf_terrain_debug_set_tile_list_capacity(vf_terrain *t, uint32_t units);
 int vf_terrain_debug_phase_cycles(vf_terrain *t, uint64_t *dst, uint32_t n);
 
 int vf_grid_generate(vf_ctx *ctx, uint32_t nx, uint32_t nz, float dx, float dy,
diff --git a/vulkan_forge_amd/cabi.py b/vulkan_forge_amd/cabi.py
--- a/vulkan_forge_amd/cabi.py
+++ b/vulkan_forge_amd/cabi.py
@@ -12,6 +12,7 @@
 VF_DRAPE_SIZE_MAX, VF_DRAPE_NEAREST, VF_DRAPE_LINEAR = 16384, 0, 1
 VF_DRAPE_MIP_BIAS_MAX, VF_DRAPE_MIP_LEVELS_MAX = 16.0, 15
 VF_PLAN_FIRST, VF_PLAN_FRESH, VF_PLAN_MOTION_MAP, VF_PLAN_DILATE, VF_PLAN_QUEUED_AHEAD = 1, 2, 4, 8, 16
+VF_PLAN_TILE_LISTS = 64
 VF_PLAN_GEOMETRY_REUSED = 32
 
 SYMBOLS = [
@@ -21,7 +22,7 @@
     "vf_terrain_local_tiles", "vf_terrain_read_tiles", "vf_tile_layout", "vf_terrain_tile_times", "vf_balance_stripes", "vf_tile_layout_register_map", "vf_terrain_set_output_device",
     "vf_terrain_rgba_device", "vf_terrain_render", "vf_terrain_render_batch", "vf_terrain_render_batch_host", "vf_terrain_sync",
     "vf_terrain_add_points", "vf_terrain_add_lines", "vf_terrain_add_polygons", "vf_terrain_set_layer_occlusion", "vf_terrain_add_contours", "vf_terrain_height_bounds", "vf_terrain_layer_primitive_count", "vf_terrain_clear_overlays", "vf_terrain_read_rgba", "vf_terrain_read_png_scanlines", "vf_terrain_read_visibility",
-    "vf_terrain_enable_timing", "vf_terrain_timings", "vf_terrain_frame_times", "vf_terrain_debug_item_stats", "vf_terrain_debug_band_masks", "vf_terrain_debug_set_plan_feedback", "vf_terrain_debug_plan_mode", "vf_terrain_debug_phase_cycles", "vf_grid_generate", "vf_grid_generate_device", "vf_triangle_render",
+    "vf_terrain_enable_timing", "vf_terrain_timings", "vf_terrain_frame_times", "vf_terrain_debug_item_stats", "vf_terrain_debug_band_masks", "vf_terrain_debug_set_plan_feedback", "vf_terrain_debug_plan_mode", "vf_terrain_debug_tile_lists", "vf_terrain_debug_set_tile_list_capacity", "vf_terrain_debug_phase_cycles", "vf_grid_generate", "vf_grid_generate_device", "vf_triangle_render",
     "vf_stitch_bands_device", "vf_stitch_tiles_device",
     "vf_dist_available", "vf_dist_version", "vf_dist_unique_id", "vf_dist_comm_init", "vf_dist_comm_destroy", "vf_dist_gather_tiles", "vf_dist_gather_bands", "vf_dist_exchange_bands",
     "vf_terrain_debug_fragment_stage", "vf_host_alloc", "vf_host_free",
@@ -117,6 +118,8 @@
     "vf_terrain_debug_band_masks": (_i, [_vp, _vp, _vp, _vp, _u32, C.POINTER(_u32)]),
     "vf_terrain_debug_set_plan_feedback": (_i, [_vp, _vp, _vp, _vp, _u32]),
     "vf_terrain_debug_plan_mode": (_i, [_vp, C.POINTER(_u32)]),
+    "vf_terrain_debug_tile_lists": (_i, [_vp, _vp]),
+    "vf_terrain_debug_set_tile_list_capacity": (_i, [_vp, _u32]),
     "vf_terrain_debug_phase_cycles": (_i, [_vp, _vp, _u32]),
     "vf_terrain_tile_times": (_i, [_vp, _vp, _u32, C.POINTER(_u32)]),
     "vf_balance_stripes": (_i, [_vp, _u32, _u32, _vp]),
@@ -705,7 +708,18 @@
     def plan_mode(self, geometry=False):
         m = _u32()
         self._check(self.lib.vf_terrain_debug_plan_mode(self.t, C.byref(m)))
-        return m.value if geometry else m.value & ~VF_PLAN_GEOMETRY_REUSED
+        return m.value if geometry else m.value & ~(VF_PLAN_GEOMETRY_REUSED | VF_PLAN_TILE_LISTS)
+
+    def tile_lists(self):
+        w = (_u32 * 8)()
+        self._check(self.lib.vf_terrain_debug_tile_lists(self.t, C.addressof(w)))
+        names = ("built", "used", "tiles_listed", "tiles_fallback", "entries", "capacity", "units_asked")
+        d = dict(zip(names, (int(v) for v in w)))
+        d["built"], d["used"] = bool(d["built"]), bool(d["used"])
+        return d
+
+    def set_tile_list_capacity(self, units=0xFFFFFFFF):
+        self._check(self.lib.vf_terrain_debug_set_tile_list_capacity(self.t, units))
 
     def geometry_reused(self):
         return bool(self.plan_mode(geometry=True) & VF_PLAN_GEOMETRY_REUSED)
diff --git a/vulkan_forge_amd/csrc/vf_hip.hip b/vulkan_forge_amd/csrc/vf_hip.hip
--- a/vulkan_forge_amd/csrc/vf_hip.hip
+++ b/vulkan_forge_amd/csrc/vf_hip.hip
@@ -185,6 +185,7 @@
     bool motion_starts = false;
     bool sampled = true;
     uint32_t *rc_lo = nullptr, *rc_hi = nullptr, *seg_count = nullptr;
+    bool lists = false;
 };
 
 template <typename T> struct DevBuf {
@@ -437,7 +438,16 @@
         float u_used[32] = {};
         bool have_u_used = false;
         uint64_t geom_stamp = 0, height_stamp = 0;
+        uint4 *tl_ent = nullptr, *tl_hdr = nullptr;
+        uint32_t *tl_ctl = nullptr;
+        uint32_t tl_units = 0, tl_cap = 0;
+        uint64_t list_stamp = 0;
+        hipEvent_t listed = nullptr;
     } ps[kPlanStates];
+    struct ListJob { bool pending = false; uint32_t set = 0; uint64_t geom = 0; FrameParams P; } tl_job;
+    bool tl_off = false;
+    uint32_t tl_cap_debug = 0xFFFFFFFFu;
+    bool tl_failed = false;
     PlanCursor cursor;
     uint32_t last_set = 0;
     uint32_t last_plan_mode = 0;
@@ -716,6 +726,7 @@
     hipError_t err = C.commit(&S.slab, zero_on);
     if (err != hipSuccess) { S.slab = nullptr; return err; }
     S.geom_stamp = S.height_stamp = 0;
+    S.list_stamp = 0;
     S.work_sorted = S.work + (all_tiles + kSplitBudget + 16);
     if (err == hipSuccess) err = hipEventCreateWithFlags(&S.planned, hipEventDisableTiming);
     if (err == hipSuccess) err = hipEventCreateWithFlags(&S.drawn, hipEventDisableTiming);
@@ -786,6 +797,7 @@
     if (n > 8192) return fail(VF_ERR_INVALID, "grid must be <= 8192");
     VF_HIP_TRY(hipSetDevice(ctx->device));
     vf_terrain *t = new (std::nothrow) vf_terrain;
+    if (t) { const char *e = std::getenv("VF_NO_TILE_LISTS"); t->tl_off = e && *e && std::strcmp(e, "0") != 0; }
     if (!t) return fail(VF_ERR_NOMEM, "out of host memory");
     t->ctx = ctx; t->W = width; t->H = height; t->n = n;
     t->nb = (n - 1 + kBlockCells - 1) / kBlockCells;
@@ -856,6 +868,9 @@
         if (S.drawn) (void)hipEventDestroy(S.drawn);
         if (S.boxed) (void)hipEventDestroy(S.boxed);
         if (S.set_up) (void)hipEventDestroy(S.set_up);
+        if (S.listed) (void)hipEventDestroy(S.listed);
+        if (S.tl_ent) (void)hipFree(S.tl_ent);
+        if (S.tl_hdr) (void)hipFree(S.tl_hdr);
         for (auto &e : S.pev) if (e) (void)hipEventDestroy(e);
     }
     pinned_free(t->h_stage);
@@ -991,7 +1006,7 @@
         VF_HIP_TRY(hipMemset(S.background, 0, (size_t)t->ntx * t->nty * sizeof(uint32_t)));
         S.have_u_used = false;
     }
-    for (auto &S : t->ps) S.geom_stamp = S.height_stamp = 0;
+    for (auto &S : t->ps) { S.geom_stamp = S.height_stamp = 0; S.list_stamp = 0; }
     return VF_OK;
 }
 
@@ -1286,7 +1301,56 @@
 #endif
 static bool fast_shading(const FrameInputs &in) { return in.precision == VF_PRECISION_FAST && in.shade_mode == VF_SHADE_REFERENCE; }
 
-static int plan_frame(vf_terrain *t, hipStream_t s, FramePlan &K, bool streaming = false)
+constexpr size_t kTileListMaxUnits = (size_t)4 << 20;
+static bool lists_valid(const vf_terrain *t, const vf_terrain::PlanState &S)
+{
+    return S.list_stamp != 0 && S.list_stamp == S.geom_stamp && S.geom_stamp == t->geom_gen && S.height_stamp == t->height_gen;
+}
+static hipError_t queue_tile_lists(vf_terrain *t, vf_terrain::PlanState &S, const FrameParams &P, hipStream_t on)
+{
+    const uint32_t ntiles = t->local_tiles;
+    if (t->tl_off || t->tl_failed || !ntiles || !S.slab || S.geom_stamp == 0) return hipSuccess;
+    if (!S.tl_ent) {
+        const size_t all_tiles = (size_t)t->ntx * t->nty;
+        const size_t units = std::min<size_t>(kTileListMaxUnits, 2 * (size_t)t->nblocks + 512 * (size_t)ntiles);
+        hipError_t e = hipMalloc((void **)&S.tl_ent, units * sizeof(uint4));
+        if (e == hipSuccess) e = hipMalloc((void **)&S.tl_hdr, (all_tiles + 2) * sizeof(uint4));
+        if (e == hipSuccess && !S.listed) e = hipEventCreateWithFlags(&S.listed, hipEventDisableTiming);
+        if (e != hipSuccess) {
+            if (S.tl_ent) (void)hipFree(S.tl_ent);
+            if (S.tl_hdr) (void)hipFree(S.tl_hdr);
+            S.tl_ent = S.tl_hdr = nullptr;
+            t->tl_failed = true;
+            (void)hipGetLastError();
+            return hipSuccess;
+        }
+        S.tl_ctl = reinterpret_cast<uint32_t *>(S.tl_hdr + all_tiles);
+        S.tl_units = (uint32_t)units;
+    }
+    const size_t rc_n = (size_t)t->nb * t->ntx;
+    hipError_t e = hipStreamWaitEvent(on, S.set_up, 0);
+    if (e == hipSuccess) e = hipStreamWaitEvent(on, S.drawn, 0);
+    if (e == hipSuccess) e = hipMemsetAsync(S.tl_ctl, 0, 8 * sizeof(uint32_t), on);
+    if (e != hipSuccess) return e;
+    S.tl_cap = std::min(S.tl_units, t->tl_cap_debug);
+    hipLaunchKernelGGL(k_tile_lists, dim3(ntiles), dim3(256), 0, on, P, S.row_ranges, S.recs, S.cap_seg, S.cap_rad, S.rc, S.rc + rc_n,
+                       S.tl_ent, S.tl_hdr, S.tl_ctl, S.tl_cap);
+    e = hipGetLastError();
+    if (e == hipSuccess) e = hipEventRecord(S.listed, on);
+    if (e == hipSuccess) S.list_stamp = S.geom_stamp;
+    return e;
+}
+static void flush_tile_lists(vf_terrain *t, hipStream_t s)
+{
+    if (!t->tl_job.pending) return;
+    t->tl_job.pending = false;
+    vf_terrain::PlanState &S = t->ps[t->tl_job.set];
+    if (S.geom_stamp == 0 || S.geom_stamp != t->tl_job.geom || S.geom_stamp != t->geom_gen || S.height_stamp != t->height_gen || t->bounds_dirty) return;
+    if (lists_valid(t, S)) return;
+    if (queue_tile_lists(t, S, t->tl_job.P, s) != hipSuccess) (void)hipGetLastError();
+}
+
+static int plan_frame(vf_terrain *t, hipStream_t s, FramePlan &K, bool streaming = false, bool ahead = false)
 {
     FrameParams &P = K.P;
     PlanCursor &C = t->cursor;
@@ -1342,7 +1406,7 @@
         VF_HIP_TRY(hipEventRecord(t->cached, side));
         t->cached_on = side;
         t->bounds_dirty = false;
-        for (auto &X : t->ps) X.geom_stamp = X.height_stamp = 0;
+        for (auto &X : t->ps) { X.geom_stamp = X.height_stamp = 0; X.list_stamp = 0; }
     }
     if (t->cached_on && t->cached_on != side) {
         VF_HIP_TRY(hipStreamWaitEvent(side, t->cached, 0));
@@ -1360,6 +1424,8 @@
         hipLaunchKernelGGL(k_plan_begin, dim3(1), dim3(512), 0, side, quantum_from, t->ntx * t->nty, quantum, S.work_count);
     } else {
         S.geom_stamp = S.height_stamp = 0;
+        S.list_stamp = 0;
+        if (S.listed) VF_HIP_TRY(hipStreamWaitEvent(side, S.listed, 0));
         hipLaunchKernelGGL(k_block_boxes, dim3(t->nb + 1), dim3(t->nb > 256 ? 512 : 256), 0, side, P, t->d_bounds, S.ranges, S.row_ranges, S.cap_seg, S.cap_rad, rc_lo, rc_hi,
                            quantum_from, t->ntx * t->nty, quantum, S.work_count, S.recs, S.seg_list, seg_count);
         VF_HIP_TRY(hipEventRecord(S.boxed, side));
@@ -1370,6 +1436,8 @@
         VF_HIP_TRY(hipGetLastError());
         S.geom_stamp = t->geom_gen; S.height_stamp = t->height_gen;
     }
+    K.lists = reuse && ntiles && !t->tl_off && lists_valid(t, S);
+    if (reuse && ntiles && !K.lists && !solo && (ahead || streaming)) VF_HIP_TRY(queue_tile_lists(t, S, P, side2));
     if (timed) VF_HIP_TRY(hipEventRecord(ev[1], side));
     if (ntiles) {
         if (fresh) {
@@ -1390,7 +1458,7 @@
     if (timed) VF_HIP_TRY(hipEventRecord(ev[2], side));
     VF_HIP_TRY(hipEventRecord(S.planned, side));
     K.mode = (first ? VF_PLAN_FIRST : 0u) | (fresh ? VF_PLAN_FRESH : 0u) | (M.on ? VF_PLAN_MOTION_MAP : 0u) | (dilate ? VF_PLAN_DILATE : 0u) |
-             (reuse ? VF_PLAN_GEOMETRY_REUSED : 0u);
+             (reuse ? VF_PLAN_GEOMETRY_REUSED : 0u) | (K.lists ? VF_PLAN_TILE_LISTS : 0u);
     K.set = set; K.ntiles = ntiles; K.motion_starts = motion_starts; K.rc_lo = rc_lo; K.rc_hi = rc_hi; K.seg_count = seg_count;
     return VF_OK;
 }
@@ -1470,6 +1538,8 @@
     const uint32_t nstats = (uint32_t)stats_layout(t).words;
     VF_HIP_TRY(hipStreamWaitEvent(s, S.planned, 0));
     VF_HIP_TRY(hipStreamWaitEvent(s, S.set_up, 0));
+    if (K.lists) VF_HIP_TRY(hipStreamWaitEvent(s, S.listed, 0));
+    const TileLists TL = { K.lists ? S.tl_ent : nullptr, K.lists ? S.tl_hdr : nullptr };
     if (t->last_stream && t->last_stream != s && t->rendered)
         VF_HIP_TRY(hipStreamWaitEvent(s, t->ps[t->last_set].drawn, 0));
     if (timing_now) VF_HIP_TRY(hipEventRecord(ev.begin, s));
@@ -1483,7 +1553,7 @@
         const dim3 per_cu(std::min<uint32_t>((uint32_t)std::max(1, t->ctx->prop.multiProcessorCount) * (1024u / (uint32_t)kTileThreads), ntiles + kSplitBudget)),
                    few(std::min<uint32_t>(64u, ntiles + kSplitBudget)), threads(kTileThreads);
 #define VF_TILE_ARGS P, V, S.row_ranges, S.cap_seg, S.cap_rad, t->d_lut, t->ctx->d_thresh, S.work_sorted, S.work_count, \
-                     rc_lo, rc_hi, t->d_rgba, vis, stats, S.feedback, S.redo, S.band
+                     rc_lo, rc_hi, t->d_rgba, vis, stats, S.feedback, S.redo, S.band, TL
         const bool fast = fast_shading(t->inputs);
 #define VF_TILE_LAUNCH(WV, FS)                                                                                         \
         do {                                                                                                           \
@@ -1535,7 +1605,7 @@
 {
     vf_terrain::PrePlan &R = t->pre;
     R.before = t->cursor;
-    if (plan_frame(t, s, R.K) == VF_OK) { R.valid = true; R.gen = t->inputs_gen; R.geom = t->geom_gen; }
+    if (plan_frame(t, s, R.K, false, true) == VF_OK) { R.valid = true; R.gen = t->inputs_gen; R.geom = t->geom_gen; }
     else {
         t->cursor = R.before;
         (void)hipGetLastError();
@@ -1552,11 +1622,12 @@
 
 static hipError_t finish_readback(vf_terrain *t, hipStream_t s)
 {
-    if (!t->preplan_pending) return hipStreamSynchronize(s);
+    if (!t->preplan_pending && !t->tl_job.pending) return hipStreamSynchronize(s);
     hipError_t e = t->copied ? hipSuccess : hipEventCreateWithFlags(&t->copied, hipEventDisableTiming);
-    if (e != hipSuccess) { t->preplan_pending = false; return hipStreamSynchronize(s); }
+    if (e != hipSuccess) { t->preplan_pending = false; t->tl_job.pending = false; return hipStreamSynchronize(s); }
     e = hipEventRecord(t->copied, s);
     if (e != hipSuccess) return e;
+    flush_tile_lists(t, s);
     flush_preplan(t, s);
     return hipEventSynchronize(t->copied);
 }
@@ -1589,6 +1660,10 @@
     if (rc != VF_OK) return rc;
     t->last_plan_mode = K.mode | (planned ? VF_PLAN_QUEUED_AHEAD : 0u);
     t->last_drawn_geom = t->geom_gen;
+    flush_tile_lists(t, t->side ? t->side2 : s);
+    if (!write_vis && (K.mode & VF_PLAN_GEOMETRY_REUSED) && !K.lists && !t->tl_off && !t->tl_failed && K.ntiles && !lists_valid(t, t->ps[K.set])) {
+        t->tl_job.pending = true; t->tl_job.set = K.set; t->tl_job.geom = t->ps[K.set].geom_stamp; t->tl_job.P = K.P;
+    }
     if (again && (idle_at_entry || t->side) && !write_vis && !t->bounds_dirty && !t->cursor.camera_moving && !t->cursor.was_moving && t->cursor.frames_since_reset > vf_terrain::kPlanStates && !(t->timing && t->stats_on)) {
         if (t->side) plan_ahead(t, s);
         else t->preplan_pending = true;
@@ -2124,7 +2199,7 @@
         if (err == hipSuccess) err = hipEventRecord(t->stage_ev[i % kStageSlots], s);
         if (err == hipSuccess) enqueued.store(i + 1, std::memory_order_release);
     }
-    if (err == hipSuccess) flush_preplan(t, s);
+    if (err == hipSuccess) { flush_tile_lists(t, s); flush_preplan(t, s); }
     if (err != hipSuccess) failed.store(1);
     for (auto &th : pool) th.join();
     if (err != hipSuccess) return fail(VF_ERR_HIP, hipGetErrorString(err));
@@ -3362,6 +3437,41 @@
     return VF_OK;
 }
 
+int vf_terrain_debug_tile_lists(vf_terrain *t, vf_tile_list_info *out)
+{
+    if (!t || !out) return fail(VF_ERR_INVALID, "NULL argument");
+    if (!t->rendered) return fail(VF_ERR_INVALID, "nothing rendered yet");
+    VF_HIP_TRY(hipSetDevice(t->ctx->device));
+    std::memset(out, 0, sizeof *out);
+    const vf_terrain::PlanState &S = t->ps[t->last_set];
+    out->used = (t->last_plan_mode & VF_PLAN_TILE_LISTS) ? 1u : 0u;
+    out->built = lists_valid(t, S) ? 1u : 0u;
+    if (!out->built && !out->used) return VF_OK;
+    VF_HIP_TRY(hipEventSynchronize(S.listed));
+    uint32_t ctl[8];
+    VF_HIP_TRY(hipMemcpy(ctl, S.tl_ctl, sizeof ctl, hipMemcpyDeviceToHost));
+    out->tiles_listed = ctl[2]; out->tiles_fallback = ctl[3]; out->entries = ctl[4];
+    out->capacity = S.tl_cap;
+    const unsigned long long asked = (unsigned long long)ctl[0] | ((unsigned long long)ctl[1] << 32);
+    out->units_asked = asked > 0xFFFFFFFFull ? 0xFFFFFFFFu : (uint32_t)asked;
+    return VF_OK;
+}
+
+int vf_terrain_debug_set_tile_list_capacity(vf_terrain *t, uint32_t units)
+{
+    if (!t) return fail(VF_ERR_INVALID, "NULL argument");
+    VF_HIP_TRY(hipSetDevice(t->ctx->device));
+    VF_HIP_TRY(wait_frame(t));
+    VF_HIP_TRY(sync_sides(t));
+    VF_HIP_TRY(drop_preplan(t));
+    VF_HIP_TRY(wait_frame(t));
+    VF_HIP_TRY(sync_sides(t));
+    t->tl_cap_debug = units;
+    t->tl_job.pending = false;
+    for (auto &S : t->ps) S.list_stamp = 0;
+    return VF_OK;
+}
+
 int vf_terrain_debug_phase_cycles(vf_terrain *t, uint64_t *dst, uint32_t n)
 {
     if (!t || !dst) return fail(VF_ERR_INVALID, "NULL argument");
diff --git a/vulkan_forge_amd/csrc/vf_kernels.h b/vulkan_forge_amd/csrc/vf_kernels.h
--- a/vulkan_forge_amd/csrc/vf_kernels.h
+++ b/vulkan_forge_amd/csrc/vf_kernels.h
@@ -1024,6 +1024,94 @@
         const uint32_t ticks = max(s_est / 16u, 1u);
         feedback[blockIdx.x] = ticks;
         feedback[(size_t)P.ntx * P.nty + 1u + (size_t)blockIdx.x * 64u] = ticks;
+    }
+}
+
+__global__ __launch_bounds__(256) void k_tile_lists(FrameParams P, const PixelBox *__restrict__ row_boxes, const BlockRec *__restrict__ recs,
+                                                    const float4 *__restrict__ cap_seg, const float *__restrict__ cap_rad,
+                                                    const uint32_t *__restrict__ rc_lo, const uint32_t *__restrict__ rc_hi,
+                                                    uint4 *__restrict__ ent, uint4 *__restrict__ hdr, uint32_t *__restrict__ ctl, uint32_t capacity)
+{
+    __shared__ uint32_t s_cnt[1024];
+    __shared__ uint32_t s_part[4], s_at, s_hi, s_lo;
+    int32_t px_lo, px_hi, py_lo, py_hi;
+    const TilePlace tp = tile_rect(P, blockIdx.x, px_lo, px_hi, py_lo, py_hi);
+    const uint32_t tid = threadIdx.x, sub = tid & 7u, rsub = tid >> 3, lane = tid & 63u, wv = tid >> 6;
+    for (uint32_t r = tid; r < 1024u; r += 256u) s_cnt[r] = 0u;
+    if (tid == 0) { s_hi = 0u; s_lo = 0xFFFFu; }
+    __syncthreads();
+    auto test = [&](uint32_t r, uint32_t bx, uint4 &e) -> bool {
+        const uint4 rw = *reinterpret_cast<const uint4 *>(recs + r * P.nb + bx);
+        const int32_t x0 = (int16_t)(rw.x & 0xFFFFu), y0 = (int16_t)(rw.x >> 16), x1 = (int16_t)(rw.y & 0xFFFFu), y1 = (int16_t)(rw.y >> 16);
+        if (!(x0 <= x1 && x1 >= px_lo && x0 <= px_hi && y1 >= py_lo && y0 <= py_hi)) return false;
+        if (!capsule_hits_rect(cap_seg[r * P.nb + bx], cap_rad[r * P.nb + bx], px_lo, px_hi, py_lo, py_hi)) return false;
+        e = make_uint4(bx | (r << 10), rw.x, rw.y, 0u);
+        return true;
+    };
+    auto row_range = [&](uint32_t r, uint32_t &lo, uint32_t &hi) -> bool {
+        const PixelBox rr = row_boxes[r];
+        lo = rc_lo[tp.tx * P.nb + r]; hi = rc_hi[tp.tx * P.nb + r];
+        return lo < hi && rr.x0 <= rr.x1 && rr.x1 >= px_lo && rr.x0 <= px_hi && rr.y1 >= py_lo && rr.y0 <= py_hi;
+    };
+    for (uint32_t base = 0; base < P.nb; base += 32u) {
+        const uint32_t r = base + rsub;
+        uint32_t c = 0, lo = 1, hi = 0;
+        if (r < P.nb && row_range(r, lo, hi))
+            for (uint32_t bx = lo + sub; bx < hi; bx += 8u) { uint4 e; c += test(r, bx, e) ? 1u : 0u; }
+        c += __shfl_xor(c, 1); c += __shfl_xor(c, 2); c += __shfl_xor(c, 4);
+        if (sub == 0 && c) { s_cnt[r] = c; atomicMax(&s_hi, r); atomicMin(&s_lo, r); }
+    }
+    __syncthreads();
+    uint32_t mine[4], sum = 0;
+#pragma unroll
+    for (int k = 0; k < 4; ++k) { mine[k] = s_cnt[1023u - (tid * 4u + (uint32_t)k)]; sum += mine[k]; }
+    const uint32_t inc = wave_scan_add(sum);
+    if (lane == 63u) s_part[wv] = inc;
+    __syncthreads();
+    uint32_t before = inc - sum;
+    for (uint32_t w = 0; w < wv; ++w) before += s_part[w];
+    const uint32_t total = s_part[0] + s_part[1] + s_part[2] + s_part[3];
+#pragma unroll
+    for (int k = 0; k < 4; ++k) { s_cnt[1023u - (tid * 4u + (uint32_t)k)] = before; before += mine[k]; }
+    const uint32_t row_hi = s_hi, row_lo = s_lo;
+    const uint32_t span = total ? row_hi - row_lo + 1u : 0u;
+    const uint32_t noff4 = (span + 1u + 3u) / 4u;
+    if (tid == 0) {
+        uint32_t at = 0xFFFFFFFFu;
+        if (total) {
+            const unsigned long long need = (unsigned long long)noff4 + total;
+            const unsigned long long got = atomicAdd(reinterpret_cast<unsigned long long *>(ctl), need);
+            if (got + need <= (unsigned long long)capacity) at = (uint32_t)got;
+            if (at != 0xFFFFFFFFu) { atomicAdd(&ctl[2], 1u); atomicAdd(&ctl[4], total); } else atomicAdd(&ctl[3], 1u);
+            hdr[blockIdx.x] = at != 0xFFFFFFFFu ? make_uint4(at + noff4, total, row_hi | (row_lo << 16), at) : make_uint4(0u, 0xFFFFFFFFu, 0u, 0u);
+        } else {
+            atomicAdd(&ctl[2], 1u);
+            hdr[blockIdx.x] = make_uint4(0u, 0u, 0u, 0u);
+        }
+        s_at = at;
+    }
+    __syncthreads();
+    const uint32_t at = s_at;
+    if (at == 0xFFFFFFFFu) return;
+    uint32_t *const roff = reinterpret_cast<uint32_t *>(ent + at);
+    for (uint32_t j = tid; j <= span; j += 256u) roff[j] = j < span ? s_cnt[row_hi - j] : total;
+    uint4 *const out = ent + at + noff4;
+    for (uint32_t base = 0; base < P.nb; base += 32u) {
+        const uint32_t r = base + rsub;
+        uint32_t lo = 1, hi = 0;
+        const bool on = r < P.nb && row_range(r, lo, hi);
+        const uint32_t trips = on ? (hi - lo + 7u) / 8u : 0u;
+        uint32_t tmax = trips, done = 0;
+        tmax = max(tmax, (uint32_t)__shfl_xor((int)tmax, 8)); tmax = max(tmax, (uint32_t)__shfl_xor((int)tmax, 16)); tmax = max(tmax, (uint32_t)__shfl_xor((int)tmax, 32));
+        for (uint32_t t = 0; t < tmax; ++t) {
+            uint4 e = make_uint4(0u, 0u, 0u, 0u);
+            const uint32_t bx = lo + sub + 8u * t;
+            const bool hit = t < trips && bx < hi && test(r, bx, e);
+            const unsigned long long m = __ballot(hit);
+            const uint32_t grp = (uint32_t)((m >> (lane & ~7u)) & 0xFFull);
+            if (hit) out[s_cnt[r] + done + (uint32_t)__popc(grp & ((1u << sub) - 1u))] = e;
+            done += (uint32_t)__popc(grp);
+        }
     }
 }
 
@@ -1202,6 +1290,7 @@
 #define VF_PH_ARG
 #define VF_PH_PASS
 #endif
+struct TileLists { const uint4 *ent; const uint4 *hdr; };
 namespace tile {
 constexpr int kWaves = kTileThreads / 64;
 constexpr int kNV = kBlockVerts * kBlockVerts;
@@ -1399,6 +1488,66 @@
 }
 
 template <bool GROUPS>
+__device__ __forceinline__ void take_listed_rows(const FrameParams &P, const Lds &L, const TileCtx &T, const uint4 *__restrict__ ent,
+                                                 const uint32_t *__restrict__ roff, const float4 *__restrict__ cap_seg, const float *__restrict__ cap_rad,
+                                                 bool strip, uint32_t row_hi, uint32_t done, uint32_t span_all,
+                                                 uint32_t tid, uint32_t lane, uint32_t wave, uint32_t &nsteps, uint32_t &nlist VF_PH_ARG)
+{
+    static_assert(kMaxSteps == 128 && kChunk == 64u * 64u, "two lanes' worth of offset words and one; one ballot per lane in the scan");
+    static_assert(sizeof(unsigned long long) * 64 + sizeof(uint32_t) * kChunk <= kOverlayBytes, "ballots + block words live in the overlay");
+    const uint32_t span = min((uint32_t)kMaxSteps, span_all - done);
+    const uint32_t *const o = roff + done;
+    const uint32_t v0 = lane <= span ? o[lane] : 0u, v1 = 64u + lane <= span ? o[64u + lane] : 0u;
+    const uint32_t v2 = span == 128u ? o[128] : 0u;
+    const uint32_t e_first = (uint32_t)__builtin_amdgcn_readfirstlane((int)v0);
+    const unsigned long long fa = __ballot(lane >= 1u && lane <= span && v0 - e_first <= kChunk), fb = __ballot(64u + lane <= span && v1 - e_first <= kChunk);
+    nsteps = (uint32_t)__builtin_amdgcn_readfirstlane((int)((uint32_t)__popcll(fa) + (uint32_t)__popcll(fb) + (span == 128u && v2 - e_first <= kChunk ? 1u : 0u)));
+    uint32_t e_end = (uint32_t)__builtin_amdgcn_readfirstlane((int)v2);
+    if (nsteps < 64u) e_end = (uint32_t)__builtin_amdgcn_readlane((int)v0, (int)nsteps);
+    else if (nsteps < 128u) e_end = (uint32_t)__builtin_amdgcn_readlane((int)v1, (int)(nsteps - 64u));
+    const uint32_t n_ent = e_end - e_first, ntrips = (n_ent + 63u) / 64u;
+    const uint32_t row_top = row_hi - done;
+    asm volatile("" : "+v"(tid));
+    if (tid < nsteps) { L.pending[tid] = 0u; L.firstid[tid] = 2u * ((row_top - tid) * kBlockCells * P.nm1) + 1u; }
+    unsigned long long *const hitm = &L.hit[0][0];
+    uint32_t *const stage = reinterpret_cast<uint32_t *>(hitm + 64);
+    const uint4 *const src = ent + e_first;
+    for (uint32_t t = wave; t < ntrips; t += kWaves) {
+        const uint32_t idx = t * 64u + lane;
+        bool hit = false;
+        if (idx < n_ent) {
+            const uint4 e = src[idx];
+            stage[idx] = e.x;
+            const PixelBox box = PixelBox{ (int16_t)(e.y & 0xFFFFu), (int16_t)(e.y >> 16), (int16_t)(e.z & 0xFFFFu), (int16_t)(e.z >> 16) };
+            float4 seg = make_float4(0.f, 0.f, 0.f, 0.f);
+            float rad = INFINITY;
+            if (strip && box.x1 >= T.px_lo && box.x0 <= T.px_hi) {
+                const uint32_t bidx = ((e.x >> 10) & 0x3FFu) * P.nb + (e.x & 0x3FFu);
+                seg = cap_seg[bidx]; rad = cap_rad[bidx];
+            }
+            hit = block_is_candidate<GROUPS>(box, seg, rad, T);
+        }
+        const unsigned long long m = __ballot(hit);
+        if (lane == 0) hitm[t] = m;
+    }
+    VF_PH(9)
+    __syncthreads();
+    VF_PH(10)
+    const uint32_t c = lane < ntrips ? (uint32_t)__popcll(hitm[lane]) : 0u;
+    const uint32_t inc = wave_scan_add(c);
+    nlist = (uint32_t)__builtin_amdgcn_readlane((int)inc, 63);
+    for (uint32_t t = wave; t < ntrips; t += kWaves) {
+        const unsigned long long m = hitm[t];
+        const uint32_t pos = (uint32_t)__builtin_amdgcn_readlane((int)inc, (int)t) - (uint32_t)__popcll(m);
+        if ((m >> lane) & 1ull) {
+            const uint32_t e = stage[t * 64u + lane], step = row_top - ((e >> 10) & 0x3FFu);
+            L.list[pos + (uint32_t)__popcll(m & ((1ull << lane) - 1ull))] = (e & 0xFFFFFu) | (step << 20);
+            atomicAdd(&L.pending[step], 1u);
+        }
+    }
+}
+
+template <bool GROUPS>
 __device__ __forceinline__ uint32_t publish_chunk_masks(const Lds &L, uint32_t nsteps, uint32_t lane, uint32_t wave)
 {
     {
@@ -1455,7 +1604,7 @@
                                                        const uint32_t *__restrict__ rc_lo, const uint32_t *__restrict__ rc_hi,
                                                        uint32_t *__restrict__ rgba, uint32_t *__restrict__ vis_out, uint32_t *stats,
                                                        uint32_t *__restrict__ last_blocks, uint32_t *__restrict__ redo,
-                                                       const ulonglong2 *__restrict__ band)
+                                                       const ulonglong2 *__restrict__ band, TileLists TL)
 {
     using namespace tile;
     uint32_t *const redo_count = work_count + 3;
@@ -1477,6 +1626,7 @@
     __shared__ __attribute__((aligned(16))) float s_lut[kLutFloats];
     __shared__ float s_thr[256];
     __shared__ uint32_t s_per[65];
+    __shared__ uint32_t s_tl[4];
     WaveLds &s_wave = *reinterpret_cast<WaveLds *>(s_overlay);
     int2 (&sXY)[kWaves][kNV] = s_wave.xy;
     uint32_t (&sS)[kWaves][kBlockPrims] = s_wave.surv;
@@ -1528,23 +1678,38 @@
     for (int k = tid; k < kTileH * 2; k += kTileThreads) s_rowfin[k] = 0u;
     if (tid < kTileW / 4 * 2) { s_colfin4[tid] = 0u; s_rowfin4[tid] = 0u; }
     if (tid < 16) s_rows[tid] = 0ull;
-    if (tid == 0) { s_done = 0; s_blocks = 0; s_redo = 0; }
+    if (tid == 0) {
+        s_done = 0; s_blocks = 0; s_redo = 0;
+        uint4 th = make_uint4(0u, 0xFFFFFFFFu, 0u, 0u);
+        if (TL.hdr) th = TL.hdr[tile];
+        s_tl[0] = th.x; s_tl[1] = th.y; s_tl[2] = th.z; s_tl[3] = th.w;
+    }
     __syncthreads();
     VF_PH(13)
-    const uint32_t nrows_total = list_block_rows(P, L, T, row_boxes, rc_lo, rc_hi, tcol, tid, lane, wave VF_PH_PASS);
+    const bool listed = lds_peek(&s_tl[1]) != 0xFFFFFFFFu;
+    uint32_t nrows_total;
+    if (listed) { const uint32_t n = lds_peek(&s_tl[1]), rows = lds_peek(&s_tl[2]); nrows_total = n ? (rows & 0xFFFFu) - (rows >> 16) + 1u : 0u; }
+    else nrows_total = list_block_rows(P, L, T, row_boxes, rc_lo, rc_hi, tcol, tid, lane, wave VF_PH_PASS);
     VF_PH(8)
     uint32_t dbg_loop = 0;
     const uint32_t hit_words = (P.nb + 63u) / 64u;
     for (uint32_t cursor = 0; cursor < nrows_total;) {
+        if (tid == 0) { s_next = 0; s_lock = 0; s_frontier = 0; s_published = 0; }
+        uint32_t nsteps, nlist;
+        if (lds_peek(&s_tl[1]) != 0xFFFFFFFFu) {
+            const uint32_t e0 = (uint32_t)__builtin_amdgcn_readfirstlane((int)lds_peek(&s_tl[0])), o0 = (uint32_t)__builtin_amdgcn_readfirstlane((int)lds_peek(&s_tl[3]));
+            const uint32_t row_hi = (uint32_t)__builtin_amdgcn_readfirstlane((int)lds_peek(&s_tl[2])) & 0xFFFFu;
+            take_listed_rows<GROUPS>(P, L, T, TL.ent + e0, reinterpret_cast<const uint32_t *>(TL.ent + o0), cap_seg, cap_rad, ((item >> 24) & 7u) != 0u, row_hi, cursor, nrows_total,
+                                     tid, lane, wave, nsteps, nlist VF_PH_PASS);
+        } else {
         const uint32_t nrowsteps = min((uint32_t)kMaxSteps, nrows_total - cursor);
-        if (tid == 0) { s_next = 0; s_lock = 0; s_frontier = 0; s_published = 0; }
         if (!GROUPS) test_candidates_pairs<GROUPS>(P, V, L, T, cap_seg, cap_rad, cursor, nrowsteps, lane, wave);
         else test_candidates_rows<GROUPS>(P, V, L, T, cap_seg, cap_rad, cursor, nrowsteps, hit_words, lane, wave);
         VF_PH(9)
         __syncthreads();
         VF_PH(10)
-        uint32_t nsteps, nlist;
         fill_work_list(L, cursor, nrowsteps, lane, wave, nsteps, nlist);
+        }
         cursor += nsteps;
         VF_PH(11)
         __syncthreads();
```

Result: faster. 27230, median of 6 (+5.8%).
